# castacks/mvs_gi

Measured on AMD Instinct MI355X. Metric: stereo frames/sec/GPU (G16V, 3-cam, D=16) + inv-dist L1 vs reference, higher is better.
Workload: dtype f16x3 (split-fp16 MFMA operands: 11 + 11 significant bits, f32 accumulate/activations)

## Files before the change

### __graft_entry__.py

```python
import os
import subprocess
import sys

ROOT = os.path.dirname(os.path.abspath(__file__))
CSRC = os.path.join(ROOT, "mvs_gi_amd", "csrc")
LIB = os.path.join(ROOT, "mvs_gi_amd", "libmvsgi_hip.so")
SOURCES = ["api.cpp", "sweep.hip", "conv3d.hip", "conv3d_f16.hip", "conv3d_rs.hip", "conv3d_wino.hip", "conv3d_wino_up2.hip", "conv3d_s2rs.hip", "conv3d_up2poly.hip", "conv3d_headsplit.hip", "conv2d.hip", "resblock2d_rs.hip", "resize.hip", "softargmin.hip", "layout.hip", "grids.hip", "deform_conv2d.hip", "instnorm.hip"]


SRCHASH = LIB + ".srchash"


def _deps() -> list:
    return sorted([os.path.join(CSRC, s) for s in SOURCES] +
                  [os.path.join(CSRC, h) for h in os.listdir(CSRC) if h.endswith((".hpp", ".inc"))] +
                  [os.path.join(ROOT, "include", "mvsgi.h")])


def _source_hash(defs=()) -> str:
    import hashlib
    h = hashlib.sha256()
    for d in _deps():
        h.update(os.path.basename(d).encode() + b"\0")
        h.update(open(d, "rb").read())
    h.update(repr((sorted(defs), sorted(EXTRA_FLAGS.items()))).encode())
    return h.hexdigest()


def _needs_rebuild() -> bool:
    if not os.path.isfile(LIB) or not os.path.isfile(SRCHASH):
        return True
    return open(SRCHASH).read().strip() != _source_hash()


EXTRA_FLAGS = {
    "conv3d_rs.hip": ["-fno-slp-vectorize"],
    "conv3d_wino.hip": ["-fno-slp-vectorize"],
    "conv3d_wino_up2.hip": ["-fno-slp-vectorize"],
}


def _compile_objects(defs=(), tag="") -> list:
    from concurrent.futures import ThreadPoolExecutor
    import hashlib
    hipcc = os.environ.get("HIPCC", "/opt/rocm/bin/hipcc")
    if defs:
        tag += "_" + hashlib.md5(repr(sorted(defs)).encode()).hexdigest()[:8]
    objdir = os.path.join(ROOT, "build", "obj" + tag)
    os.makedirs(objdir, exist_ok=True)
    hdrs = [os.path.join(CSRC, h) for h in os.listdir(CSRC) if h.endswith((".hpp", ".inc"))] + \
           [os.path.join(ROOT, "include", "mvsgi.h")]
    hdr_t = max(os.path.getmtime(h) for h in hdrs)

    def one(src):
        obj = os.path.join(objdir, src + ".o")
        sp = os.path.join(CSRC, src)
        if os.path.isfile(obj) and os.path.getmtime(obj) > max(os.path.getmtime(sp), hdr_t):
            return obj
        cmd = [hipcc, "--offload-arch=gfx950", "-O3", "-std=c++17", "-fPIC", "-c", sp, "-o", obj] + list(defs) + \
            EXTRA_FLAGS.get(src, [])
        print("[build]", " ".join(cmd), flush=True)
        subprocess.run(cmd, check=True)
        return obj
    with ThreadPoolExecutor(max_workers=min(8, len(SOURCES))) as ex:
        return list(ex.map(one, SOURCES))


def _link(objs, out) -> None:
    hipcc = os.environ.get("HIPCC", "/opt/rocm/bin/hipcc")
    tmp = out + f".tmp{os.getpid()}"
    try:
        subprocess.run([hipcc, "--offload-arch=gfx950", "-fPIC", "-shared", "-o", tmp] + objs, check=True)
        os.replace(tmp, out)
    finally:
        if os.path.exists(tmp):
            os.remove(tmp)


def build(force: bool = False) -> None:
    if ROOT not in sys.path:
        sys.path.insert(0, ROOT)
    if force or _needs_rebuild():
        if force:
            import shutil
            shutil.rmtree(os.path.join(ROOT, "build", "obj"), ignore_errors=True)
        h = _source_hash()
        _link(_compile_objects(), LIB)
        with open(SRCHASH + f".tmp{os.getpid()}", "w") as f:
            f.write(h + "\n")
        os.replace(SRCHASH + f".tmp{os.getpid()}", SRCHASH)
    import mvs_gi_amd
    from mvs_gi_amd import _lib
    lib = _lib.load()
    assert lib.mvsgi_abi_version() == _lib.ABI_VERSION
    print(f"[build] {LIB} ok (ABI {lib.mvsgi_abi_version()})", flush=True)


def build_stamps(ablate: int = 0) -> str:
    out = os.path.join(ROOT, "mvs_gi_amd", f"libmvsgi_hip_stamps{ablate or ''}.so")
    _link(_compile_objects(["-DMVSGI_STAMPS", "-DMVSGI_RS_STAMPS", f"-DMVSGI_ABL={ablate}", f"-DMVSGI_RS_ABL={ablate}"],
                           tag=f"_stamps{ablate or ''}"), out)
    return out


def build_variant(defs, tag: str) -> str:
    out = os.path.join(ROOT, "mvs_gi_amd", f"libmvsgi_hip_{tag}.so")
    _link(_compile_objects(list(defs), tag="_" + tag), out)
    return out


def smoke() -> None:
    if ROOT not in sys.path:
        sys.path.insert(0, ROOT)
    import numpy as np
    import torch
    build()
    from mvs_gi_amd import hip_ops as H, synth
    from mvs_gi_amd.configs import CONFIGS, DIST_8L
    from mvs_gi_amd.pipeline import HotPath
    from oracle import mvsgi_oracle as O

    assert torch.cuda.is_available(), "smoke() needs a GPU"
    cfg = CONFIGS["G16V"].scaled(feat_hw=(16, 64), mask_hw=(64, 256), cv_hw=(8, 32), dist_cands=DIST_8L)
    inp = synth.make_inputs(cfg, seed=11, batch=1)
    w = synth.make_weights(cfg, seed=11)
    t = O.to_torch(inp)
    ref = O.hot_path(t["feats"], t["grids"], t["grid_masks"], t["masks"], O.to_torch(w), cfg.builder,
                     cfg.dist_cands, cfg.bf, cfg.interp_scale_factor, cfg.pre_interp)
    default_mode = H.get_conv_mode()
    try:
        bars = {"bf16x3": 1e-3, "f16x3": 1e-4, "f32": 1e-4}
        for mode in dict.fromkeys((default_mode, "f16x3", "bf16x3", "f32")):
            bar = bars[mode]
            H.set_conv_mode(mode)
            hp = HotPath(cfg, w, inp, device="cuda:0")
            inv, _ = hp(torch.from_numpy(inp["feats"]).to("cuda:0"))
            torch.cuda.synchronize()
            err = float((inv.cpu() - ref).abs().max() / ref.abs().max())
            print(f"[smoke] mode {mode}: inv_dist {tuple(inv.shape)} max-rel error vs oracle {err:.3e} (bar {bar:g})", flush=True)
            assert np.isfinite(err) and err < bar, (mode, err)
    finally:
        H.set_conv_mode(default_mode)


if __name__ == "__main__":
    build(force="--force" in sys.argv)
    if "--smoke" in sys.argv:
        smoke()
```

### include/mvsgi.h

```cpp
#ifndef MVSGI_H
#define MVSGI_H

#include <stddef.h>
#include <stdint.h>

#ifdef __cplusplus
extern "C" {
#endif

#define MVSGI_ABI_VERSION 5

typedef void* mvsgi_stream_t;

#define MVSGI_CONV_AUTO   0
#define MVSGI_CONV_DIRECT 1
#define MVSGI_CONV_MFMA   2
#define MVSGI_CONV_BF16X3 3
#define MVSGI_CONV_BF16X3_C16 4
#define MVSGI_CONV_BF16X3_V32 5
#define MVSGI_CONV_BF16X3_D32 6

#define MVSGI_CONV_F16 0x100

#define MVSGI_SPLIT_F16 1

int         mvsgi_abi_version(void);
const char* mvsgi_last_error(void);

#define MVSGI_SAT_SWEEP 1u
#define MVSGI_SAT_SPLIT 2u
#define MVSGI_SAT_WINO  4u
int mvsgi_saturation_flags(int clear, unsigned* flags);
int mvsgi_saturation_words(unsigned* words8);

int mvsgi_sweep_std_f32(const float* feats, const float* grids, const void* grid_masks,
                        int grid_mask_is_f32, const float* masks, float* vol,
                        int B, int N, int C, int Hi, int Wi, int Hm, int Wm,
                        int D, int Ho, int Wo, mvsgi_stream_t stream);

int mvsgi_sweep_cat_f32(const float* feats, const float* grids, float* vol,
                        int B, int N, int C, int Hi, int Wi,
                        int D, int Ho, int Wo, mvsgi_stream_t stream);

int mvsgi_sweep_std_nhwc_f32(const float* feats, const float* grids, const void* grid_masks,
                             int grid_mask_is_f32, const float* masks, float* vol,
                             int B, int N, int C, int Hi, int Wi, int Hm, int Wm,
                             int D, int Ho, int Wo, mvsgi_stream_t stream);
int mvsgi_sweep_cat_nhwc_f32(const float* feats, const float* grids, float* vol,
                             int B, int N, int C, int Hi, int Wi,
                             int D, int Ho, int Wo, mvsgi_stream_t stream);

int mvsgi_sweep_validity_u8(const float* grids, const void* grid_masks, int grid_mask_is_f32,
                            const float* masks, unsigned char* vmask,
                            int B, int N, int Hm, int Wm, int D, int Ho, int Wo, mvsgi_stream_t stream);
int mvsgi_sweep_std_nhwc_valid_f32(const float* feats, const float* grids, const unsigned char* vmask,
                                   float* vol, int B, int N, int C, int Hi, int Wi,
                                   int D, int Ho, int Wo, mvsgi_stream_t stream);
int mvsgi_sweep_std_nhwc_valid_rig_f32(const float* feats, const float* grids, const unsigned char* vmask,
                                       float* vol, int B, int N, int C, int Hi, int Wi, int D, int Ho, int Wo,
                                       mvsgi_stream_t stream);

size_t mvsgi_conv3d_packed_weight_floats(int Cout, int Cin);
int mvsgi_conv3d_pack_weights_f32(const float* w_oidhw, float* w_packed, int Cout, int Cin,
                                  mvsgi_stream_t stream);
size_t mvsgi_conv3d_packed_weight_bytes_bf16x3(int Cout, int Cin);
int mvsgi_conv3d_pack_weights_bf16x3(const float* w_oidhw, void* w_packed, int Cout, int Cin,
                                     mvsgi_stream_t stream);
int mvsgi_conv3d_pack_weights_split(const float* w_oidhw, void* w_packed, int Cout, int Cin, int layout, mvsgi_stream_t stream);
int mvsgi_conv3d_f32(const float* x, const float* w_oidhw, const float* w_packed,
                     const float* scale, const float* shift, const float* res, float* y,
                     int B, int Cin, int Din, int Hin, int Win, int Cout,
                     int stride, float neg_slope, int impl, mvsgi_stream_t stream);
const char* mvsgi_conv3d_variant_f32(int B, int Cin, int Din, int Hin, int Win, int Cout,
                                     int stride, int impl);

int mvsgi_conv3d_up2_f32(const float* x, const void* w_packed, int w_layout ,
                         const float* scale, const float* shift, const float* res, float* y,
                         int B, int Cin, int Dl, int Hl, int Wl, int Cout, float neg_slope, mvsgi_stream_t stream);
const char* mvsgi_conv3d_up2_variant_f32(int B, int Cin, int Dl, int Hl, int Wl, int Cout, int w_layout);
int mvsgi_conv3d_v32_applies(int B, int Cin, int Din, int Hin, int Win, int Cout, int stride);
int mvsgi_conv3d_d32_applies(int B, int Cin, int Din, int Hin, int Win, int Cout, int stride);
int mvsgi_conv3d_up2_d32_applies(int B, int Cin, int Dl, int Hl, int Wl, int Cout);
size_t mvsgi_conv3d_packed_weight_bytes_bf16x3_v32(int Cout, int Cin);
int mvsgi_conv3d_pack_weights_bf16x3_v32(const float* w_oidhw, void* w_packed, int Cout, int Cin, mvsgi_stream_t stream);
size_t mvsgi_conv3d_packed_weight_bytes_bf16x3_c16(int Cin);
int mvsgi_conv3d_pack_weights_bf16x3_c16(const float* w_oidhw, void* w_packed, int Cin, mvsgi_stream_t stream);

size_t mvsgi_conv2d_packed_weight_floats(int Cout, int Cin);
int mvsgi_conv2d_pack_weights_f32(const float* w_oihw, float* w_packed, int Cout, int Cin,
                                  mvsgi_stream_t stream);
size_t mvsgi_conv2d_stem_packed_weight_bytes(void);
int mvsgi_conv2d_stem_pack_weights(const float* w_oihw, void* w_packed, mvsgi_stream_t stream);
size_t mvsgi_conv2d_packed_weight_bytes_bf16x3(int Cout, int Cin);
int mvsgi_conv2d_pack_weights_bf16x3(const float* w_oihw, void* w_packed, int Cout, int Cin,
                                     mvsgi_stream_t stream);
int mvsgi_conv2d_f32(const float* x, const float* w_oihw, const void* w_packed,
                     const float* scale, const float* shift, const float* res, float* y,
                     int B, int Cin, int Hin, int Win, int Cout, int ksize, int stride,
                     float neg_slope, int impl, int in_nchw, mvsgi_stream_t stream);
const char* mvsgi_conv2d_variant_f32(int Cin, int Cout, int ksize, int stride, int impl, int in_nchw);

int mvsgi_resize_trilinear_f32(const float* x, float* y, int B, int C,
                               int Di, int Hi, int Wi, int Do, int Ho, int Wo,
                               mvsgi_stream_t stream);

int mvsgi_softargmin_f32(const float* costs, const float* inv_idx, float* inv_dist,
                         float* norm_costs, int B, int D, int H, int W, int scale,
                         mvsgi_stream_t stream);

int mvsgi_softargmin_div_f32(const float* costs, const float* inv_idx, float* inv_dist,
                             float* norm_costs, int B, int D, int H, int W, int scale,
                             float post_div, mvsgi_stream_t stream);

#define MVSGI_SA_AUTO  0
#define MVSGI_SA_PIXEL 1
#define MVSGI_SA_BAND  2
int mvsgi_softargmin_scaled_f32(const float* costs, const float* inv_idx, float* inv_dist,
                                float* norm_costs, int B, int D, int H, int W, double scale,
                                int OH, int OW, float post_div, int variant, mvsgi_stream_t stream);

int mvsgi_ncv_to_nvc_f32(const float* x, float* y, int B, int C, long long V, mvsgi_stream_t stream);
int mvsgi_nvc_to_ncv_f32(const float* x, float* y, int B, int C, long long V, mvsgi_stream_t stream);

int mvsgi_resblock2d_f32(const float* x, const void* w_packed1, const float* scale1, const float* shift1,
                         const void* w_packed2, const float* scale2, const float* shift2, float* y,
                         int N, int H, int W, float neg_slope, mvsgi_stream_t stream);

size_t mvsgi_split2d_bytes(int N, int H, int W);
int mvsgi_f32_to_split2d(const float* x, void* y_split, int N, int H, int W, mvsgi_stream_t stream);
int mvsgi_split2d_to_f32(const void* x_split, float* y, int N, int H, int W, mvsgi_stream_t stream);
size_t mvsgi_resblock2d_split_packed_weight_bytes(void);
int mvsgi_resblock2d_split_pack_weights(const float* w_oihw, const float* scale, void* w_packed, mvsgi_stream_t stream);
int mvsgi_resblock2d_split(const void* x_split, const void* w_packed1, const float* shift1,
                           const void* w_packed2, const float* shift2, void* y, int y_is_split,
                           int N, int H, int W, float neg_slope, mvsgi_stream_t stream);
int mvsgi_conv2d_s2_split(const void* x_split, const void* w_packed, const float* shift, void* y_split,
                          int N, int H, int W, float neg_slope, mvsgi_stream_t stream);
int mvsgi_conv2d_f32_out_split2d(const float* x, const float* w_oihw, const void* w_packed,
                                 const float* scale, const float* shift, const float* res, void* y_split,
                                 int B, int Cin, int Hin, int Win, int Cout, int ksize, int stride,
                                 float neg_slope, int impl, int in_nchw, mvsgi_stream_t stream);

int mvsgi_rays_panorama_f32(const float* dist, float* rays, int N, int H, int W,
                            float lat0, float lat1, float lon0, float lon1, mvsgi_stream_t stream);
int mvsgi_transform_points_f32(const float* T , const float* points, float* out,
                               int B, long long M, mvsgi_stream_t stream);
int mvsgi_grid_double_sphere_f32(const float* points, float* grid, unsigned char* mask, int B, long long M,
                                 float xi, float alpha, float fx, float fy, float cx, float cy,
                                 int calib_h, int calib_w, float w2, mvsgi_stream_t stream);
int mvsgi_grid_equirect_f32(const float* points, float* grid, int B, long long M, mvsgi_stream_t stream);

int mvsgi_deform_conv2d_pack_weights_f32(const float* w_oihw, float* w_packed, int Cout, int Cin, int Kh, int Kw,
                                         mvsgi_stream_t stream);
int mvsgi_deform_conv2d_f32(const float* x, const float* offset, int offset_per_image, const float* w_packed,
                            const float* scale, const float* shift, const float* res, float* y,
                            int N, int Cin, int H, int W, int Cout, int Kh, int Kw, int stride_h, int stride_w,
                            int pad_h, int pad_w, int dil_h, int dil_w, float neg_slope, mvsgi_stream_t stream);

int mvsgi_sweep_std_nhwc_valid_split(const float* feats, const float* grids, const unsigned char* vmask,
                                     void* vol_split, int B, int N, int C, int Hi, int Wi, int D, int Ho, int Wo,
                                     int rig_batch, mvsgi_stream_t stream);

int mvsgi_conv3d_f32_out_split(const float* x, const float* w_packed_b3, const float* scale, const float* shift,
                               const float* res, void* y_split, int B, int Cin, int Din, int Hin, int Win, int Cout,
                               int stride, float neg_slope, mvsgi_stream_t stream);
int mvsgi_conv3d_rs16_split(const void* x_split, const void* w_packed_rs, const float* scale, const float* shift, float* y,
                            int B, int D, int H, int W, float neg_slope, mvsgi_stream_t stream);
int mvsgi_conv3d_rs16_split_out_split(const void* x_split, const void* w_packed_rs, const float* scale, const float* shift,
                                      void* y_split, int B, int D, int H, int W, float neg_slope, mvsgi_stream_t stream);
size_t mvsgi_conv3d_s2rs_packed_weight_bytes(void);
int mvsgi_conv3d_s2rs_pack_weights(const float* w_oidhw, const float* scale, void* w_packed, mvsgi_stream_t stream);
int mvsgi_conv3d_s2rs(const void* x_split, const void* w_packed, const float* shift, void* y_split,
                      int B, int D, int H, int W, float neg_slope, mvsgi_stream_t stream);
size_t mvsgi_conv3d_rs_packed_weight_bytes(int Cout, int Cin);
int mvsgi_conv3d_rs_pack_weights(const float* w_oidhw, void* w_packed, int Cout, int Cin, mvsgi_stream_t stream);
size_t mvsgi_act_split_bytes(int B, int C, int D, int H, int W);
int mvsgi_act_f32_to_split(const float* x, void* y_split, int B, int C, int D, int H, int W, mvsgi_stream_t stream);
int mvsgi_act_split_to_f32(const void* x_split, float* y, int B, int C, int D, int H, int W, mvsgi_stream_t stream);
int mvsgi_conv3d_rs_split(const void* x_split, const void* w_packed_rs, const float* scale, const float* shift,
                          const void* res_split, void* y, int y_is_f32, int B, int Cin, int D, int H, int W, int Cout,
                          float neg_slope, mvsgi_stream_t stream);

int mvsgi_conv3d_up2_f32_out_split(const float* x, const void* w_packed, int w_layout, const float* scale, const float* shift,
                                   const float* res, void* y_split, int B, int Cin, int Dl, int Hl, int Wl, int Cout,
                                   float neg_slope, mvsgi_stream_t stream);
int mvsgi_conv3d_up2_poly_split(const void* x_split, const void* plan_dev, const float* scale, const float* shift, void* y_split,
                                int B, int D, int H, int W, float neg_slope, mvsgi_stream_t stream);
size_t mvsgi_conv3d_head_split_packed_weight_bytes(int Cin);
int mvsgi_conv3d_head_split_pack_weights(const float* w_oidhw, void* w_packed, int Cin, mvsgi_stream_t stream);
int mvsgi_conv3d_head_split(const void* x_split, const void* w_packed, float scale, float shift, float* y, int B, int Cin,
                            int D, int H, int W, float neg_slope, mvsgi_stream_t stream);
int mvsgi_conv3d_head_split_pack_weights_f16(const float* w_oidhw, void* w_packed, int Cin, mvsgi_stream_t stream);
int mvsgi_conv3d_head_split_f16(const void* x_split, const void* w_packed, float scale, float shift, float* y, int B, int Cin,
                            int D, int H, int W, float neg_slope, mvsgi_stream_t stream);
size_t mvsgi_conv3d_up2_poly_plan_bytes(int D, int H, int W);
int mvsgi_conv3d_up2_poly_plan(const float* w_oidhw_host, void* plan_host, int D, int H, int W);
int mvsgi_conv3d_up2_poly_f32(const void* x_split, const void* plan_dev, const float* scale, const float* shift, float* y,
                              int B, int D, int H, int W, float neg_slope, mvsgi_stream_t stream);

int mvsgi_act_f32_to_split_fmt(const float* x, void* y_split, int B, int C, int D, int H, int W, int fmt, mvsgi_stream_t stream);
int mvsgi_act_split_to_f32_fmt(const void* x_split, float* y, int B, int C, int D, int H, int W, int fmt, mvsgi_stream_t stream);
int mvsgi_sweep_std_nhwc_valid_split_fmt(const float* feats, const float* grids, const unsigned char* vmask, void* vol_split,
                                         int B, int N, int C, int Hi, int Wi, int D, int Ho, int Wo, int rig_batch, int fmt,
                                         mvsgi_stream_t stream);
int mvsgi_conv3d_f32_out_split_fmt(const float* x, const float* w_packed_b3, const float* scale, const float* shift,
                                   const float* res, void* y_split, int B, int Cin, int Din, int Hin, int Win, int Cout,
                                   int stride, float neg_slope, int fmt, mvsgi_stream_t stream);
int mvsgi_conv3d_rs_pack_weights_fmt(const float* w_oidhw, void* w_packed, int Cout, int Cin, int fmt, mvsgi_stream_t stream);
int mvsgi_conv3d_rs_split_fmt(const void* x_split, const void* w_packed_rs, const float* scale, const float* shift,
                              const void* res_split, void* y, int y_is_f32, int B, int Cin, int D, int H, int W, int Cout,
                              float neg_slope, int fmt, mvsgi_stream_t stream);
int mvsgi_conv3d_rs16_split_fmt(const void* x_split, const void* w_packed_rs, const float* scale, const float* shift, void* y,
                                int y_is_split, int B, int D, int H, int W, float neg_slope, int fmt, mvsgi_stream_t stream);
int mvsgi_conv3d_s2rs_pack_weights_fmt(const float* w_oidhw, const float* scale, void* w_packed, int fmt, mvsgi_stream_t stream);
int mvsgi_conv3d_s2rs_fmt(const void* x_split, const void* w_packed, const float* shift, void* y_split, int B, int D, int H, int W,
                          float neg_slope, float unscale, int fmt, mvsgi_stream_t stream);
int mvsgi_conv3d_s2rs_out_fmt(const void* x_split, const void* w_packed, const float* shift, void* y_split, int B, int D, int H, int W,
                              float neg_slope, float unscale, int fmt, int y_f32p, mvsgi_stream_t stream);
int mvsgi_conv3d_up2_poly_plan_fmt(const float* w_oidhw_host, void* plan_host, int D, int H, int W, int fmt);
int mvsgi_conv3d_up2_poly_fmt(const void* x_split, const void* plan_dev, const float* scale, const float* shift, void* y,
                              int y_is_split, int B, int D, int H, int W, float neg_slope, int fmt, mvsgi_stream_t stream);
int mvsgi_conv3d_up2_poly_wino_pays(int B, int D, int H, int W);

size_t mvsgi_conv3d_wino32_packed_weight_bytes(void);
int mvsgi_conv3d_wino32_applies(int Cin, int Cout, int D, int H, int W, int stride, float neg_slope);
int mvsgi_conv3d_wino32_pack_weights(const float* w_oidhw, void* w_packed, float* unscale, mvsgi_stream_t stream);
int mvsgi_conv3d_wino32_f16(const void* x_split, const void* w_packed, const float* scale, const float* shift, const void* res_split,
                            void* y, int y_is_f32, int act_f32p, int B, int D, int H, int W, float neg_slope, mvsgi_stream_t stream);

size_t mvsgi_instance_norm_ws_bytes(int B, int S, int C);
int mvsgi_instance_norm_f32(const float* x, const float* res, const float* gamma, const float* beta, float* y, float* ws,
                            int B, int S, int C, float eps, float neg_slope, mvsgi_stream_t stream);

#ifdef __cplusplus
}
#endif
#endif
```

### mvs_gi_amd/_lib.py

```python
from __future__ import annotations

import ctypes
import os
from ctypes import c_char_p, c_double, c_float, c_int, c_longlong, c_size_t, c_void_p

_HERE = os.path.dirname(os.path.abspath(__file__))
LIB_PATH = os.environ.get("MVSGI_LIB", os.path.join(_HERE, "libmvsgi_hip.so"))

ABI_VERSION = 5


class MvsgiLibraryMissing(RuntimeError):
    pass


_P = c_void_p
SIGNATURES = {
    "mvsgi_abi_version": (c_int, []),
    "mvsgi_last_error": (c_char_p, []),
    "mvsgi_saturation_flags": (c_int, [c_int, _P]),
    "mvsgi_saturation_words": (c_int, [_P]),
    "mvsgi_sweep_std_f32": (c_int, [_P, _P, _P, c_int, _P, _P] + [c_int] * 10 + [_P]),
    "mvsgi_sweep_cat_f32": (c_int, [_P, _P, _P] + [c_int] * 8 + [_P]),
    "mvsgi_sweep_std_nhwc_f32": (c_int, [_P, _P, _P, c_int, _P, _P] + [c_int] * 10 + [_P]),
    "mvsgi_sweep_cat_nhwc_f32": (c_int, [_P, _P, _P] + [c_int] * 8 + [_P]),
    "mvsgi_sweep_validity_u8": (c_int, [_P, _P, c_int, _P, _P] + [c_int] * 7 + [_P]),
    "mvsgi_sweep_std_nhwc_valid_f32": (c_int, [_P, _P, _P, _P] + [c_int] * 8 + [_P]),
    "mvsgi_sweep_std_nhwc_valid_split": (c_int, [_P, _P, _P, _P] + [c_int] * 9 + [_P]),
    "mvsgi_sweep_std_nhwc_valid_rig_f32": (c_int, [_P, _P, _P, _P] + [c_int] * 8 + [_P]),
    "mvsgi_conv3d_packed_weight_floats": (c_size_t, [c_int, c_int]),
    "mvsgi_conv3d_pack_weights_f32": (c_int, [_P, _P, c_int, c_int, _P]),
    "mvsgi_conv3d_packed_weight_bytes_bf16x3": (c_size_t, [c_int, c_int]),
    "mvsgi_conv3d_pack_weights_bf16x3": (c_int, [_P, _P, c_int, c_int, _P]),
    "mvsgi_conv3d_pack_weights_split": (c_int, [_P, _P, c_int, c_int, c_int, _P]),
    "mvsgi_conv3d_f32": (c_int, [_P] * 7 + [c_int] * 7 + [c_float, c_int, _P]),
    "mvsgi_conv3d_variant_f32": (c_char_p, [c_int] * 8),
    "mvsgi_conv3d_up2_f32": (c_int, [_P, _P, c_int] + [_P] * 4 + [c_int] * 6 + [c_float, _P]),
    "mvsgi_conv3d_up2_variant_f32": (c_char_p, [c_int] * 7),
    "mvsgi_conv3d_v32_applies": (c_int, [c_int] * 7),
    "mvsgi_conv3d_d32_applies": (c_int, [c_int] * 7),
    "mvsgi_conv3d_up2_d32_applies": (c_int, [c_int] * 6),
    "mvsgi_conv3d_packed_weight_bytes_bf16x3_v32": (c_size_t, [c_int, c_int]),
    "mvsgi_conv3d_pack_weights_bf16x3_v32": (c_int, [_P, _P, c_int, c_int, _P]),
    "mvsgi_conv3d_packed_weight_bytes_bf16x3_c16": (c_size_t, [c_int]),
    "mvsgi_conv3d_pack_weights_bf16x3_c16": (c_int, [_P, _P, c_int, _P]),
    "mvsgi_conv2d_stem_packed_weight_bytes": (c_size_t, []),
    "mvsgi_conv2d_stem_pack_weights": (c_int, [_P, _P, _P]),
    "mvsgi_conv2d_packed_weight_floats": (c_size_t, [c_int, c_int]),
    "mvsgi_conv2d_pack_weights_f32": (c_int, [_P, _P, c_int, c_int, _P]),
    "mvsgi_conv2d_packed_weight_bytes_bf16x3": (c_size_t, [c_int, c_int]),
    "mvsgi_conv2d_pack_weights_bf16x3": (c_int, [_P, _P, c_int, c_int, _P]),
    "mvsgi_conv2d_f32": (c_int, [_P] * 7 + [c_int] * 7 + [c_float, c_int, c_int, _P]),
    "mvsgi_conv2d_variant_f32": (c_char_p, [c_int] * 6),
    "mvsgi_resblock2d_f32": (c_int, [_P] * 8 + [c_int] * 3 + [c_float, _P]),
    "mvsgi_split2d_bytes": (c_size_t, [c_int] * 3),
    "mvsgi_f32_to_split2d": (c_int, [_P, _P] + [c_int] * 3 + [_P]),
    "mvsgi_split2d_to_f32": (c_int, [_P, _P] + [c_int] * 3 + [_P]),
    "mvsgi_resblock2d_split_packed_weight_bytes": (c_size_t, []),
    "mvsgi_resblock2d_split_pack_weights": (c_int, [_P, _P, _P, _P]),
    "mvsgi_resblock2d_split": (c_int, [_P] * 6 + [c_int] * 4 + [c_float, _P]),
    "mvsgi_conv2d_s2_split": (c_int, [_P] * 4 + [c_int] * 3 + [c_float, _P]),
    "mvsgi_conv2d_f32_out_split2d": (c_int, [_P] * 7 + [c_int] * 7 + [c_float, c_int, c_int, _P]),
    "mvsgi_resize_trilinear_f32": (c_int, [_P, _P] + [c_int] * 8 + [_P]),
    "mvsgi_softargmin_f32": (c_int, [_P, _P, _P, _P] + [c_int] * 5 + [_P]),
    "mvsgi_softargmin_div_f32": (c_int, [_P, _P, _P, _P] + [c_int] * 5 + [c_float, _P]),
    "mvsgi_softargmin_scaled_f32": (c_int, [_P, _P, _P, _P] + [c_int] * 4 + [c_double, c_int, c_int, c_float, c_int, _P]),
    "mvsgi_rays_panorama_f32": (c_int, [_P, _P, c_int, c_int, c_int] + [c_float] * 4 + [_P]),
    "mvsgi_transform_points_f32": (c_int, [_P, _P, _P, c_int, c_longlong, _P]),
    "mvsgi_grid_double_sphere_f32": (c_int, [_P, _P, _P, c_int, c_longlong] + [c_float] * 6 + [c_int, c_int, c_float, _P]),
    "mvsgi_grid_equirect_f32": (c_int, [_P, _P, c_int, c_longlong, _P]),
    "mvsgi_deform_conv2d_pack_weights_f32": (c_int, [_P, _P] + [c_int] * 4 + [_P]),
    "mvsgi_deform_conv2d_f32": (c_int, [_P, _P, c_int] + [_P] * 5 + [c_int] * 13 + [c_float, _P]),
    "mvsgi_act_split_bytes": (c_size_t, [c_int] * 5),
    "mvsgi_act_f32_to_split": (c_int, [_P, _P] + [c_int] * 5 + [_P]),
    "mvsgi_act_split_to_f32": (c_int, [_P, _P] + [c_int] * 5 + [_P]),
    "mvsgi_conv3d_f32_out_split": (c_int, [_P] * 6 + [c_int] * 7 + [c_float, _P]),
    "mvsgi_conv3d_rs16_split": (c_int, [_P] * 5 + [c_int] * 4 + [c_float, _P]),
    "mvsgi_conv3d_rs16_split_out_split": (c_int, [_P] * 5 + [c_int] * 4 + [c_float, _P]),
    "mvsgi_conv3d_s2rs_packed_weight_bytes": (c_size_t, []),
    "mvsgi_conv3d_s2rs_pack_weights": (c_int, [_P, _P, _P, _P]),
    "mvsgi_conv3d_s2rs": (c_int, [_P] * 4 + [c_int] * 4 + [c_float, _P]),
    "mvsgi_conv3d_rs_packed_weight_bytes": (c_size_t, [c_int, c_int]),
    "mvsgi_conv3d_rs_pack_weights": (c_int, [_P, _P, c_int, c_int, _P]),
    "mvsgi_conv3d_rs_split": (c_int, [_P] * 6 + [c_int] * 7 + [c_float, _P]),
    "mvsgi_conv3d_up2_f32_out_split": (c_int, [_P, _P, c_int] + [_P] * 4 + [c_int] * 6 + [c_float, _P]),
    "mvsgi_conv3d_up2_poly_split": (c_int, [_P] * 5 + [c_int] * 4 + [c_float, _P]),
    "mvsgi_conv3d_head_split_packed_weight_bytes": (c_size_t, [c_int]),
    "mvsgi_conv3d_head_split_pack_weights": (c_int, [_P, _P, c_int, _P]),
    "mvsgi_conv3d_head_split": (c_int, [_P, _P, c_float, c_float, _P] + [c_int] * 5 + [c_float, _P]),
    "mvsgi_conv3d_head_split_pack_weights_f16": (c_int, [_P, _P, c_int, _P]),
    "mvsgi_conv3d_head_split_f16": (c_int, [_P, _P, c_float, c_float, _P] + [c_int] * 5 + [c_float, _P]),
    "mvsgi_conv3d_up2_poly_plan_bytes": (c_size_t, [c_int] * 3),
    "mvsgi_conv3d_up2_poly_plan": (c_int, [_P, _P] + [c_int] * 3),
    "mvsgi_conv3d_up2_poly_f32": (c_int, [_P] * 5 + [c_int] * 4 + [c_float, _P]),
    "mvsgi_act_f32_to_split_fmt": (c_int, [_P, _P] + [c_int] * 6 + [_P]),
    "mvsgi_act_split_to_f32_fmt": (c_int, [_P, _P] + [c_int] * 6 + [_P]),
    "mvsgi_sweep_std_nhwc_valid_split_fmt": (c_int, [_P, _P, _P, _P] + [c_int] * 10 + [_P]),
    "mvsgi_conv3d_f32_out_split_fmt": (c_int, [_P] * 6 + [c_int] * 7 + [c_float, c_int, _P]),
    "mvsgi_conv3d_rs_pack_weights_fmt": (c_int, [_P, _P, c_int, c_int, c_int, _P]),
    "mvsgi_conv3d_rs_split_fmt": (c_int, [_P] * 6 + [c_int] * 7 + [c_float, c_int, _P]),
    "mvsgi_conv3d_rs16_split_fmt": (c_int, [_P] * 5 + [c_int] * 5 + [c_float, c_int, _P]),
    "mvsgi_conv3d_s2rs_pack_weights_fmt": (c_int, [_P, _P, _P, c_int, _P]),
    "mvsgi_conv3d_s2rs_fmt": (c_int, [_P] * 4 + [c_int] * 4 + [c_float, c_float, c_int, _P]),
    "mvsgi_conv3d_s2rs_out_fmt": (c_int, [_P] * 4 + [c_int] * 4 + [c_float, c_float, c_int, c_int, _P]),
    "mvsgi_conv3d_up2_poly_plan_fmt": (c_int, [_P, _P] + [c_int] * 4),
    "mvsgi_conv3d_wino32_packed_weight_bytes": (c_size_t, []),
    "mvsgi_conv3d_wino32_applies": (c_int, [c_int] * 6 + [c_float]),
    "mvsgi_conv3d_wino32_pack_weights": (c_int, [_P] * 4),
    "mvsgi_conv3d_wino32_f16": (c_int, [_P] * 6 + [c_int] * 6 + [c_float, _P]),
    "mvsgi_conv3d_up2_poly_fmt": (c_int, [_P] * 5 + [c_int] * 5 + [c_float, c_int, _P]),
    "mvsgi_conv3d_up2_poly_wino_pays": (c_int, [c_int] * 4),
    "mvsgi_ncv_to_nvc_f32": (c_int, [_P, _P, c_int, c_int, c_longlong, _P]),
    "mvsgi_nvc_to_ncv_f32": (c_int, [_P, _P, c_int, c_int, c_longlong, _P]),
    "mvsgi_instance_norm_ws_bytes": (c_size_t, [c_int] * 3),
    "mvsgi_instance_norm_f32": (c_int, [_P] * 6 + [c_int] * 3 + [c_float, c_float, _P]),
}

_lib = None


def load() -> ctypes.CDLL:
    global _lib
    if _lib is not None:
        return _lib
    if not os.path.isfile(LIB_PATH):
        raise MvsgiLibraryMissing(
            f"{LIB_PATH} not found: build the HIP library first (__graft_entry__.build()). "
            "mvs_gi_amd has no CPU fallback.")
    import torch
    lib = ctypes.CDLL(LIB_PATH)
    try:
        lib.mvsgi_abi_version.restype = c_int
        lib.mvsgi_abi_version.argtypes = []
        got = lib.mvsgi_abi_version()
    except AttributeError as e:
        raise MvsgiLibraryMissing(f"{LIB_PATH}: not a libmvsgi_hip ({e}); rebuild it (__graft_entry__.build())") from None
    if got != ABI_VERSION:
        raise MvsgiLibraryMissing(f"{LIB_PATH}: ABI version {got}, expected {ABI_VERSION}; rebuild it (__graft_entry__.build())")
    for name, (res, args) in SIGNATURES.items():
        try:
            fn = getattr(lib, name)
        except AttributeError:
            raise MvsgiLibraryMissing(f"{LIB_PATH}: symbol {name} missing although the ABI version matches; rebuild it "
                                      "(__graft_entry__.build())") from None
        fn.restype = res
        fn.argtypes = args
    lib.mvsgi_saturation_flags(0, None)
    _lib = lib
    return lib


def check(status: int, what: str) -> None:
    if status != 0:
        msg = load().mvsgi_last_error()
        raise RuntimeError(f"{what}: {msg.decode() if msg else 'unknown error'}")
```

### mvs_gi_amd/csrc/sweep.hip

```cpp
#include "common.hpp"

namespace {

#include "split_fmt.hpp"

struct Bilin {
    int o00, o01, o10, o11;
    float w00, w01, w10, w11;
};

#ifndef MVSGI_SWEEP_SKIP_CAM
#define MVSGI_SWEEP_SKIP_CAM 1
#endif
__device__ __forceinline__ Bilin bilin_setup(float gx, float gy, int W, int H) {
#pragma clang fp contract(off)
    Bilin t;
    const float x = ((gx + 1.0f) * (float)W - 1.0f) / 2.0f;
    const float y = ((gy + 1.0f) * (float)H - 1.0f) / 2.0f;
    const float xf = floorf(x), yf = floorf(y);
    const float x1f = xf + 1.0f, y1f = yf + 1.0f;
    t.w00 = (x1f - x) * (y1f - y);
    t.w01 = (x1f - x) * (y - yf);
    t.w10 = (x - xf) * (y1f - y);
    t.w11 = (x - xf) * (y - yf);
    const int x0 = (int)fminf(fmaxf(xf, -2.0f), (float)W + 1.0f);
    const int y0 = (int)fminf(fmaxf(yf, -2.0f), (float)H + 1.0f);
    const int x1 = x0 + 1, y1 = y0 + 1;
    const bool vx0 = (x0 >= 0) & (x0 < W), vx1 = (x1 >= 0) & (x1 < W);
    const bool vy0 = (y0 >= 0) & (y0 < H), vy1 = (y1 >= 0) & (y1 < H);
    t.o00 = (vx0 & vy0) ? y0 * W + x0 : -1;
    t.o01 = (vx0 & vy1) ? y1 * W + x0 : -1;
    t.o10 = (vx1 & vy0) ? y0 * W + x1 : -1;
    t.o11 = (vx1 & vy1) ? y1 * W + x1 : -1;
    return t;
}

__device__ __forceinline__ Bilin bilin_setup_bytes(float gx, float gy, int W, int H, int C4, int rowB) {
#pragma clang fp contract(off)
    Bilin t;
    const float x = ((gx + 1.0f) * (float)W - 1.0f) / 2.0f;
    const float y = ((gy + 1.0f) * (float)H - 1.0f) / 2.0f;
    const float xf = floorf(x), yf = floorf(y);
    const float x1f = xf + 1.0f, y1f = yf + 1.0f;
    t.w00 = (x1f - x) * (y1f - y);
    t.w01 = (x1f - x) * (y - yf);
    t.w10 = (x - xf) * (y1f - y);
    t.w11 = (x - xf) * (y - yf);
    const int x0 = (int)fminf(fmaxf(xf, -2.0f), (float)W + 1.0f);
    const int y0 = (int)fminf(fmaxf(yf, -2.0f), (float)H + 1.0f);
    const bool vx0 = (unsigned)x0 < (unsigned)W, vx1 = (unsigned)(x0 + 1) < (unsigned)W;
    const bool vy0 = (unsigned)y0 < (unsigned)H, vy1 = (unsigned)(y0 + 1) < (unsigned)H;
    const int base = __mul24(y0, rowB) + __mul24(x0, C4);
    constexpr int kOutside = (int)0x80000000;
    t.o00 = (vx0 & vy0) ? base : kOutside;
    t.o01 = (vx0 & vy1) ? base + rowB : kOutside;
    t.o10 = (vx1 & vy0) ? base + C4 : kOutside;
    t.o11 = (vx1 & vy1) ? base + rowB + C4 : kOutside;
    return t;
}

__device__ __forceinline__ float bilin_fetch(const float* __restrict__ plane, const Bilin& t) {
#pragma clang fp contract(off)
    const float i00 = t.o00 >= 0 ? plane[t.o00] : 0.0f;
    const float i01 = t.o01 >= 0 ? plane[t.o01] : 0.0f;
    const float i10 = t.o10 >= 0 ? plane[t.o10] : 0.0f;
    const float i11 = t.o11 >= 0 ? plane[t.o11] : 0.0f;
    return ((i00 * t.w00 + i01 * t.w01) + i10 * t.w10) + i11 * t.w11;
}

typedef float f32x4_t __attribute__((ext_vector_type(4)));

__device__ __forceinline__ float div_small(float x, float d, float inv) {
    const float ax = fabsf(x);
    const float q = x * inv;
    const float r = __builtin_fmaf(-d, q, x);
    float res = __builtin_fmaf(r, inv, q);
    if (ax == 0.0f) res = x;
    const bool rare = ax != 0.0f && !(ax >= 1e-30f && ax <= 1e30f);
    if (__builtin_amdgcn_ballot_w64(rare) != 0) {
        if (rare) res = x / d;
    }
    return res;
}

struct SweepDims {
    int B, N, C, Hi, Wi, Hm, Wm, D, Ho, Wo;
};

template <int NCAM, int CC>
__global__ __launch_bounds__(256) void sweep_std_kernel(const float* __restrict__ feats,
                                                        const float* __restrict__ grids,
                                                        const unsigned char* __restrict__ gm_u8,
                                                        const float* __restrict__ gm_f32,
                                                        const float* __restrict__ masks,
                                                        float* __restrict__ vol, SweepDims s) {
#pragma clang fp contract(off)
    const long long total = (long long)s.B * s.D * s.Ho * s.Wo;
    const long long idx = (long long)blockIdx.x * 256 + threadIdx.x;
    if (idx >= total) return;
    const int wo = (int)(idx % s.Wo);
    const int ho = (int)((idx / s.Wo) % s.Ho);
    const int d = (int)((idx / ((long long)s.Wo * s.Ho)) % s.D);
    const int b = (int)(idx / ((long long)s.Wo * s.Ho * s.D));

    Bilin ft[NCAM];
    float vf[NCAM];
    float n = 0.0f;
    const long long HWi = (long long)s.Hi * s.Wi;
    const long long HWm = (long long)s.Hm * s.Wm;
#pragma unroll
    for (int cam = 0; cam < NCAM; ++cam) {
        const long long g = ((((long long)(b * NCAM + cam) * s.D + d) * s.Ho + ho) * s.Wo + wo);
        const float2 gxy = *reinterpret_cast<const float2*>(grids + g * 2);
        ft[cam] = bilin_setup(gxy.x, gxy.y, s.Wi, s.Hi);
        const Bilin mt = bilin_setup(gxy.x, gxy.y, s.Wm, s.Hm);
        const float sm = bilin_fetch(masks + (long long)(b * NCAM + cam) * HWm, mt);
        const bool gmv = gm_f32 ? (gm_f32[g] != 0.0f) : (gm_u8[g] != 0);
        const bool valid = (sm > 0.0f) && gmv;
        vf[cam] = valid ? 1.0f : 0.0f;
        n = n + vf[cam];
    }
    const bool ok = n > 1.0f;
    const float cnt = ok ? n : 1.0f;

    float* out = vol + idx * s.C;
    for (int c = 0; c < s.C; c += CC) {
        float sv[NCAM][CC];
#pragma unroll
        for (int cam = 0; cam < NCAM; ++cam) {
            const float* plane = feats + ((long long)(b * NCAM + cam) * s.C + c) * HWi;
#pragma unroll
            for (int k = 0; k < CC; ++k) sv[cam][k] = bilin_fetch(plane + k * HWi, ft[cam]);
        }
        float r[CC];
#pragma unroll
        for (int k = 0; k < CC; ++k) {
            float sum = 0.0f;
#pragma unroll
            for (int cam = 0; cam < NCAM; ++cam) sum = sum + sv[cam][k] * vf[cam];
            const float avg = sum / cnt;
            float var = 0.0f;
#pragma unroll
            for (int cam = 0; cam < NCAM; ++cam) {
                const float t = vf[cam] != 0.0f ? sv[cam][k] : avg;
                const float df = t - avg;
                var = var + df * df;
            }
            var = var / cnt;
            r[k] = ok ? var : 0.0f;
        }
        if (CC == 4) {
            *reinterpret_cast<float4*>(out + c) = make_float4(r[0], r[1], r[2], r[3]);
        } else {
#pragma unroll
            for (int k = 0; k < CC; ++k) out[c + k] = r[k];
        }
    }
}

template <int CC>
__global__ __launch_bounds__(256) void sweep_cat_kernel(const float* __restrict__ feats,
                                                        const float* __restrict__ grids,
                                                        float* __restrict__ vol, SweepDims s) {
#pragma clang fp contract(off)
    const long long total = (long long)s.B * s.D * s.Ho * s.N * s.Wo;
    const long long idx = (long long)blockIdx.x * 256 + threadIdx.x;
    if (idx >= total) return;
    const int wo = (int)(idx % s.Wo);
    const int cam = (int)((idx / s.Wo) % s.N);
    const int ho = (int)((idx / ((long long)s.Wo * s.N)) % s.Ho);
    const int d = (int)((idx / ((long long)s.Wo * s.N * s.Ho)) % s.D);
    const int b = (int)(idx / ((long long)s.Wo * s.N * s.Ho * s.D));
    const long long g = ((((long long)(b * s.N + cam) * s.D + d) * s.Ho + ho) * s.Wo + wo);
    const float2 gxy = *reinterpret_cast<const float2*>(grids + g * 2);
    const Bilin ft = bilin_setup(gxy.x, gxy.y, s.Wi, s.Hi);
    const long long HWi = (long long)s.Hi * s.Wi;
    const long long vox = (((long long)b * s.D + d) * s.Ho + ho) * s.Wo + wo;
    float* out = vol + vox * ((long long)s.N * s.C) + (long long)cam * s.C;
    const float* base = feats + ((long long)(b * s.N + cam) * s.C) * HWi;
    for (int c = 0; c < s.C; c += CC) {
        float r[CC];
#pragma unroll
        for (int k = 0; k < CC; ++k) r[k] = bilin_fetch(base + (long long)(c + k) * HWi, ft);
        if (CC == 4) {
            *reinterpret_cast<float4*>(out + c) = make_float4(r[0], r[1], r[2], r[3]);
        } else {
#pragma unroll
            for (int k = 0; k < CC; ++k) out[c + k] = r[k];
        }
    }
}

__device__ __forceinline__ f32x4_t ld4(const float* p) { return *reinterpret_cast<const f32x4_t*>(p); }

__device__ __forceinline__ f32x4_t bilin_fetch4(const float* __restrict__ img, int C, const Bilin& t) {
#pragma clang fp contract(off)
    const f32x4_t z = {0.f, 0.f, 0.f, 0.f};
    const f32x4_t i00 = t.o00 >= 0 ? ld4(img + t.o00 * C) : z;
    const f32x4_t i01 = t.o01 >= 0 ? ld4(img + t.o01 * C) : z;
    const f32x4_t i10 = t.o10 >= 0 ? ld4(img + t.o10 * C) : z;
    const f32x4_t i11 = t.o11 >= 0 ? ld4(img + t.o11 * C) : z;
    return ((i00 * t.w00 + i01 * t.w01) + i10 * t.w10) + i11 * t.w11;
}

__device__ __forceinline__ f32x4_t bilin_fetch4_buf(__amdgpu_buffer_rsrc_t img, int c, int C, const Bilin& t) {
#pragma clang fp contract(off)
    const f32x4_t i00 = __builtin_bit_cast(f32x4_t, __builtin_amdgcn_raw_buffer_load_b128(img, (t.o00 * C + c) * 4, 0, 0));
    const f32x4_t i01 = __builtin_bit_cast(f32x4_t, __builtin_amdgcn_raw_buffer_load_b128(img, (t.o01 * C + c) * 4, 0, 0));
    const f32x4_t i10 = __builtin_bit_cast(f32x4_t, __builtin_amdgcn_raw_buffer_load_b128(img, (t.o10 * C + c) * 4, 0, 0));
    const f32x4_t i11 = __builtin_bit_cast(f32x4_t, __builtin_amdgcn_raw_buffer_load_b128(img, (t.o11 * C + c) * 4, 0, 0));
    return ((i00 * t.w00 + i01 * t.w01) + i10 * t.w10) + i11 * t.w11;
}

__device__ __forceinline__ float bilin_fetch_buf(__amdgpu_buffer_rsrc_t plane, const Bilin& t) {
#pragma clang fp contract(off)
    const float i00 = __builtin_bit_cast(float, __builtin_amdgcn_raw_buffer_load_b32(plane, t.o00 * 4, 0, 0));
    const float i01 = __builtin_bit_cast(float, __builtin_amdgcn_raw_buffer_load_b32(plane, t.o01 * 4, 0, 0));
    const float i10 = __builtin_bit_cast(float, __builtin_amdgcn_raw_buffer_load_b32(plane, t.o10 * 4, 0, 0));
    const float i11 = __builtin_bit_cast(float, __builtin_amdgcn_raw_buffer_load_b32(plane, t.o11 * 4, 0, 0));
    return ((i00 * t.w00 + i01 * t.w01) + i10 * t.w10) + i11 * t.w11;
}

__device__ __forceinline__ int sweep_xcd_remap(int bid, int n) {
    const int q = n >> 3, r = n & 7, x = bid & 7, i = bid >> 3;
    return (x < r ? x * (q + 1) : r * (q + 1) + (x - r) * q) + i;
}

template <int NCAM>
__global__ __launch_bounds__(256) void sweep_std_nhwc_kernel(const float* __restrict__ feats,
                                                             const float* __restrict__ grids,
                                                             const unsigned char* __restrict__ gm_u8,
                                                             const float* __restrict__ gm_f32,
                                                             const float* __restrict__ masks,
                                                             float* __restrict__ vol, SweepDims s) {
#pragma clang fp contract(off)
    static_assert(NCAM <= 4, "one camera per lane of a quad");
    const int q = threadIdx.x & 3;
    const int WT = (s.Wo + 63) >> 6;
    int L = sweep_xcd_remap((int)blockIdx.x, (int)gridDim.x);
    const int wt = L % WT;
    L /= WT;
    const int d = L % s.D;
    L /= s.D;
    const int ho = L % s.Ho;
    const int b = L / s.Ho;
    int wo = wt * 64 + (threadIdx.x >> 2);
    const bool live = wo < s.Wo;
    if (!live) wo = s.Wo - 1;
    const int HWm = s.Hm * s.Wm, HWi = s.Hi * s.Wi;

    Bilin mine = {};
    float myvalid = 0.f;
    if (q < NCAM) {
        const long long grow = (((long long)(b * NCAM + q) * s.D + d) * s.Ho + ho) * s.Wo;
        const float2 gxy = *reinterpret_cast<const float2*>(grids + (grow + wo) * 2);
        mine = bilin_setup(gxy.x, gxy.y, s.Wi, s.Hi);
        const Bilin mt = bilin_setup(gxy.x, gxy.y, s.Wm, s.Hm);
        const float sm = bilin_fetch(masks + (long long)(b * NCAM + q) * HWm, mt);
        const bool gmv = gm_f32 ? (gm_f32[grow + wo] != 0.0f) : (gm_u8[grow + wo] != 0);
        myvalid = ((sm > 0.0f) && gmv) ? 1.0f : 0.0f;
    }
    const int lane = threadIdx.x & 63, qbase = lane & ~3;
    __amdgpu_buffer_rsrc_t img[NCAM];
#pragma unroll
    for (int cam = 0; cam < NCAM; ++cam)
        img[cam] = __builtin_amdgcn_make_buffer_rsrc(
            const_cast<float*>(feats + (long long)(b * NCAM + cam) * HWi * s.C), 0, HWi * s.C * 4, 0x00020000);
    Bilin ft[NCAM];
    float vf[NCAM];
    float n = 0.0f;
#pragma unroll
    for (int cam = 0; cam < NCAM; ++cam) {
        const int src = qbase + cam;
        ft[cam].o00 = __shfl(mine.o00, src);
        ft[cam].o01 = __shfl(mine.o01, src);
        ft[cam].o10 = __shfl(mine.o10, src);
        ft[cam].o11 = __shfl(mine.o11, src);
        ft[cam].w00 = __shfl(mine.w00, src);
        ft[cam].w01 = __shfl(mine.w01, src);
        ft[cam].w10 = __shfl(mine.w10, src);
        ft[cam].w11 = __shfl(mine.w11, src);
        vf[cam] = __shfl(myvalid, src);
        n = n + vf[cam];
    }
    const bool ok = n > 1.0f;
    const float cnt = ok ? n : 1.0f;
    const float inv = 1.0f / cnt;
    float* out = vol + ((((long long)b * s.D + d) * s.Ho + ho) * s.Wo + wo) * s.C;
    for (int c = q * 4; c < s.C; c += 16) {
        f32x4_t sv[NCAM];
#pragma unroll
        for (int cam = 0; cam < NCAM; ++cam) sv[cam] = bilin_fetch4_buf(img[cam], c, s.C, ft[cam]);
        f32x4_t r;
#pragma unroll
        for (int k = 0; k < 4; ++k) {
            float sum = 0.0f;
#pragma unroll
            for (int cam = 0; cam < NCAM; ++cam) sum = sum + sv[cam][k] * vf[cam];
            const float avg = div_small(sum, cnt, inv);
            float var = 0.0f;
#pragma unroll
            for (int cam = 0; cam < NCAM; ++cam) {
                const float t = vf[cam] != 0.0f ? sv[cam][k] : avg;
                const float df = t - avg;
                var = var + df * df;
            }
            var = div_small(var, cnt, inv);
            r[k] = ok ? var : 0.0f;
        }
        if (live) *reinterpret_cast<f32x4_t*>(out + c) = r;
    }
}

__global__ __launch_bounds__(256) void sweep_validity_kernel(const float* __restrict__ grids,
                                                             const unsigned char* __restrict__ gm_u8,
                                                             const float* __restrict__ gm_f32,
                                                             const float* __restrict__ masks,
                                                             unsigned char* __restrict__ vmask, SweepDims s) {
#pragma clang fp contract(off)
    const long long HW = (long long)s.Ho * s.Wo;
    const long long total = (long long)s.B * s.D * HW;
    const long long idx = (long long)blockIdx.x * 256 + threadIdx.x;
    if (idx >= total) return;
    const long long pix = idx % HW;
    const int d = (int)((idx / HW) % s.D);
    const int b = (int)(idx / (HW * s.D));
    const long long HWm = (long long)s.Hm * s.Wm;
    unsigned bits = 0;
    for (int cam = 0; cam < s.N; ++cam) {
        const long long g = ((long long)(b * s.N + cam) * s.D + d) * HW + pix;
        const float2 gxy = *reinterpret_cast<const float2*>(grids + g * 2);
        const Bilin mt = bilin_setup(gxy.x, gxy.y, s.Wm, s.Hm);
        const float sm = bilin_fetch(masks + (long long)(b * s.N + cam) * HWm, mt);
        const bool gmv = gm_f32 ? (gm_f32[g] != 0.0f) : (gm_u8[g] != 0);
        bits |= ((sm > 0.0f) && gmv) ? (1u << cam) : 0u;
    }
    vmask[idx] = (unsigned char)bits;
}

template <int CAM>
__device__ __forceinline__ int quad_bcast_i(int v) {
    return __builtin_amdgcn_mov_dpp(v, CAM * 0x55, 0xf, 0xf, true);
}
template <int CAM>
__device__ __forceinline__ float quad_bcast_f(float v) {
    return __builtin_bit_cast(float, quad_bcast_i<CAM>(__builtin_bit_cast(int, v)));
}
template <int CAM>
__device__ __forceinline__ Bilin quad_bcast(const Bilin& m) {
    Bilin t;
    t.o00 = quad_bcast_i<CAM>(m.o00);
    t.o01 = quad_bcast_i<CAM>(m.o01);
    t.o10 = quad_bcast_i<CAM>(m.o10);
    t.o11 = quad_bcast_i<CAM>(m.o11);
    t.w00 = quad_bcast_f<CAM>(m.w00);
    t.w01 = quad_bcast_f<CAM>(m.w01);
    t.w10 = quad_bcast_f<CAM>(m.w10);
    t.w11 = quad_bcast_f<CAM>(m.w11);
    return t;
}

#ifndef MVSGI_SWEEP_NT
#define MVSGI_SWEEP_NT 0
#endif
#ifndef MVSGI_SWEEP_WAVES
#define MVSGI_SWEEP_WAVES 5
#endif
template <int NCAM, bool C16, bool F16 = false>
__global__ __launch_bounds__(256, MVSGI_SWEEP_WAVES) void sweep_std_nhwc_v_kernel(const float* __restrict__ feats,
                                                               const float* __restrict__ grids,
                                                               const unsigned char* __restrict__ vmask,
                                                               float* __restrict__ vol, SweepDims s, int dchunk,
                                                               int nd, int rig_shared, unsigned char* __restrict__ vol_split,
                                                               unsigned* __restrict__ sat) {
#pragma clang fp contract(off)
    static_assert(NCAM <= 4, "one camera per lane of a quad");
    float satm = 0.f;
    const int q = threadIdx.x & 3;
    const int WT = (s.Wo + 63) >> 6;
    int L = sweep_xcd_remap((int)blockIdx.x, (int)gridDim.x);
    const int wt = L % WT;
    L /= WT;
    const int dc = L % nd;
    L /= nd;
    const int ho = L % s.Ho;
    const int b = L / s.Ho;
    int wo = wt * 64 + (threadIdx.x >> 2);
    const bool live = wo < s.Wo;
    if (!live) wo = s.Wo - 1;
    const int d0 = dc * dchunk;
    const int d1 = d0 + dchunk < s.D ? d0 + dchunk : s.D;
    const int HWi = s.Hi * s.Wi;
    const long long HW = (long long)s.Ho * s.Wo;

    __amdgpu_buffer_rsrc_t img[NCAM];
#pragma unroll
    for (int cam = 0; cam < NCAM; ++cam)
        img[cam] = __builtin_amdgcn_make_buffer_rsrc(
            const_cast<float*>(feats + (long long)(b * NCAM + cam) * HWi * s.C), 0, HWi * s.C * 4, 0x00020000);
    const int mycam = q < NCAM ? q : NCAM - 1;
    const int br = rig_shared ? 0 : b;
    const float2* gp = reinterpret_cast<const float2*>(grids) + ((long long)(br * NCAM + mycam) * s.D + d0) * HW +
                       (long long)ho * s.Wo + wo;
    const unsigned char* vp = vmask + ((long long)br * s.D + d0) * HW + (long long)ho * s.Wo + wo;
    float* out = vol + ((((long long)b * s.D + d0) * s.Ho + ho) * s.Wo + wo) * s.C;
    const long long vstep = HW * s.C;
    unsigned char* outs = vol_split ? vol_split + ((((long long)b * (s.D + 2) + d0 + 1) * (s.Ho + 2) + ho + 1) * (s.Wo + 2) + wo + 1) * 64 +
                                          ((q & 1) * 2 + (q >> 1)) * 16
                                    : nullptr;
    const long long sstep = (long long)(s.Ho + 2) * (s.Wo + 2) * 64;
    const int C4 = C16 ? 64 : s.C * 4, rowB = s.Wi * C4;
    auto candidate = [&](const float2 gxy, const unsigned vm, float* __restrict__ o, unsigned char* __restrict__ os) {
        typedef float f32x2_t __attribute__((ext_vector_type(2)));
        const Bilin mine = bilin_setup_bytes(gxy.x, gxy.y, s.Wi, s.Hi, C4, rowB);
        Bilin ft[NCAM];
        ft[0] = quad_bcast<0>(mine);
        if (NCAM > 1) ft[NCAM > 1 ? 1 : 0] = quad_bcast<1>(mine);
        if (NCAM > 2) ft[NCAM > 2 ? 2 : 0] = quad_bcast<2>(mine);
        if (NCAM > 3) ft[NCAM > 3 ? 3 : 0] = quad_bcast<3>(mine);
        bool val[NCAM];
        f32x2_t VF[NCAM];
        float n = 0.0f;
#pragma unroll
        for (int cam = 0; cam < NCAM; ++cam) {
            val[cam] = ((vm >> cam) & 1u) != 0;
            const float vf = val[cam] ? 1.0f : 0.0f;
            VF[cam] = f32x2_t{vf, vf};
            n = n + vf;
        }
        const bool ok = n > 1.0f;
        const float cnt = ok ? n : 1.0f;
#ifndef MVSGI_SWEEP_GATHER_ALL
#pragma unroll
        for (int cam = 0; cam < NCAM; ++cam) {
            const bool need = val[cam] & ok;
            ft[cam].o00 = need ? ft[cam].o00 : (int)0x80000000;
            ft[cam].o01 = need ? ft[cam].o01 : (int)0x80000000;
            ft[cam].o10 = need ? ft[cam].o10 : (int)0x80000000;
            ft[cam].o11 = need ? ft[cam].o11 : (int)0x80000000;
        }
#endif
        const float inv = cnt == 2.0f ? 0.5f : cnt == 3.0f ? 0x1.555556p-2f : cnt == 4.0f ? 0.25f : 1.0f;
        const f32x2_t INV = {inv, inv}, NCNT = {-cnt, -cnt};
#pragma unroll 1
        for (int cb = q * 16; cb < (C16 ? 64 : C4); cb += 64) {
            f32x4_t tx[NCAM][4];
#ifdef MVSGI_SWEEP_ABL_NOGATHER
#pragma unroll
            for (int cam = 0; cam < NCAM; ++cam) { ft[cam].o00 &= 64; ft[cam].o01 &= 64; ft[cam].o10 &= 64; ft[cam].o11 &= 64; }
#endif
#pragma unroll
            for (int cam = 0; cam < NCAM; ++cam) {
#if MVSGI_SWEEP_SKIP_CAM
                if (__builtin_amdgcn_ballot_w64(val[cam] & ok) == 0) {
                    tx[cam][0] = tx[cam][1] = tx[cam][2] = tx[cam][3] = f32x4_t{0.f, 0.f, 0.f, 0.f};
                    continue;
                }
#endif
                tx[cam][0] = __builtin_bit_cast(f32x4_t, __builtin_amdgcn_raw_buffer_load_b128(img[cam], ft[cam].o00 + cb, 0, 0));
                tx[cam][1] = __builtin_bit_cast(f32x4_t, __builtin_amdgcn_raw_buffer_load_b128(img[cam], ft[cam].o01 + cb, 0, 0));
                tx[cam][2] = __builtin_bit_cast(f32x4_t, __builtin_amdgcn_raw_buffer_load_b128(img[cam], ft[cam].o10 + cb, 0, 0));
                tx[cam][3] = __builtin_bit_cast(f32x4_t, __builtin_amdgcn_raw_buffer_load_b128(img[cam], ft[cam].o11 + cb, 0, 0));
            }
            f32x2_t sv[NCAM][2];
#pragma unroll
            for (int cam = 0; cam < NCAM; ++cam) {
                const f32x2_t W00 = {ft[cam].w00, ft[cam].w00}, W01 = {ft[cam].w01, ft[cam].w01};
                const f32x2_t W10 = {ft[cam].w10, ft[cam].w10}, W11 = {ft[cam].w11, ft[cam].w11};
#pragma unroll
                for (int p = 0; p < 2; ++p) {
                    const f32x2_t i00 = {tx[cam][0][2 * p], tx[cam][0][2 * p + 1]}, i01 = {tx[cam][1][2 * p], tx[cam][1][2 * p + 1]};
                    const f32x2_t i10 = {tx[cam][2][2 * p], tx[cam][2][2 * p + 1]}, i11 = {tx[cam][3][2 * p], tx[cam][3][2 * p + 1]};
                    sv[cam][p] = ((i00 * W00 + i01 * W01) + i10 * W10) + i11 * W11;
                }
            }
            f32x2_t sum[2], var[2];
            f32x4_t r;
            float big = 0.0f;
#pragma unroll
            for (int p = 0; p < 2; ++p) {
                sum[p] = sv[0][p] * VF[0];
#pragma unroll
                for (int cam = 1; cam < NCAM; ++cam) sum[p] = sum[p] + sv[cam][p] * VF[cam];
                const f32x2_t qa = sum[p] * INV;
                const f32x2_t avg = __builtin_elementwise_fma(__builtin_elementwise_fma(NCNT, qa, sum[p]), INV, qa);
#pragma unroll
                for (int cam = 0; cam < NCAM; ++cam) {
                    const f32x2_t t = {val[cam] ? sv[cam][p].x : avg.x, val[cam] ? sv[cam][p].y : avg.y};
                    const f32x2_t df = t - avg;
                    var[p] = cam == 0 ? df * df : var[p] + df * df;
                }
                const f32x2_t qv = var[p] * INV;
                const f32x2_t v = __builtin_elementwise_fma(__builtin_elementwise_fma(NCNT, qv, var[p]), INV, qv);
                r[2 * p] = ok ? v.x : 0.0f;
                r[2 * p + 1] = ok ? v.y : 0.0f;
                big = __builtin_fmaxf(__builtin_fmaxf(big, __builtin_fmaxf(__builtin_fabsf(sum[p].x), __builtin_fabsf(sum[p].y))),
                                      __builtin_fmaxf(var[p].x, var[p].y));
            }
            if (__builtin_amdgcn_ballot_w64(big > 1e30f) != 0) {
                float dv = cnt;
                asm volatile("; exact-division path" : "+v"(dv));
#pragma unroll
                for (int k = 0; k < 4; ++k) {
                    const float sm = sum[k >> 1][k & 1];
                    const float avg = sm / dv;
                    float vr = 0.0f;
#pragma unroll
                    for (int cam = 0; cam < NCAM; ++cam) {
                        const float t = val[cam] ? sv[cam][k >> 1][k & 1] : avg;
                        const float df = t - avg;
                        vr = vr + df * df;
                    }
                    vr = vr / dv;
                    r[k] = ok ? vr : 0.0f;
                }
            }
            if (os) {
                unsigned hi[2], lo[2];
#pragma unroll
                for (int p = 0; p < 2; ++p) {
                    if constexpr (F16) {
                        const float a_ = sf_clamp<true>(r[2 * p]), b_ = sf_clamp<true>(r[2 * p + 1]);
                        satm = sf_sat_acc(satm, a_, b_);
                        const unsigned hb = sf_cvt_pk<true>(a_, b_);
                        hi[p] = hb;
                        lo[p] = sf_cvt_pk<true>(a_ - sf_widen_lo<true>(hb), b_ - sf_widen_hi<true>(hb));
                    } else {
                        typedef __bf16 b2_t __attribute__((ext_vector_type(2)));
                        const f32x2_t v = {r[2 * p], r[2 * p + 1]};
                        const unsigned hb = __builtin_bit_cast(unsigned, __builtin_convertvector(v, b2_t));
                        const f32x2_t hf = {__builtin_bit_cast(float, hb << 16), __builtin_bit_cast(float, hb & 0xffff0000u)};
                        hi[p] = hb;
                        lo[p] = __builtin_bit_cast(unsigned, __builtin_convertvector(v - hf, b2_t));
                    }
                }
                const bool odd = (q & 1) != 0;
                const unsigned r0 = (unsigned)__builtin_amdgcn_mov_dpp((int)(odd ? hi[0] : lo[0]), 0xB1, 0xf, 0xf, true);
                const unsigned r1 = (unsigned)__builtin_amdgcn_mov_dpp((int)(odd ? hi[1] : lo[1]), 0xB1, 0xf, 0xf, true);
                const uint4 piece = odd ? make_uint4(r0, r1, lo[0], lo[1]) : make_uint4(hi[0], hi[1], r0, r1);
#ifdef MVSGI_SWEEP_ABL_NOSTORE
                if (live && hi[0] == 0x12345678u) {
#else
                if (live) {
#endif
#if MVSGI_SWEEP_NT
                    {
                        typedef unsigned nt_u32x4 __attribute__((ext_vector_type(4)));
                        __builtin_nontemporal_store(nt_u32x4{piece.x, piece.y, piece.z, piece.w}, reinterpret_cast<nt_u32x4*>(os));
                    }
#else
                    *reinterpret_cast<uint4*>(os) = piece;
#endif
                }
            } else if (live) *reinterpret_cast<f32x4_t*>(reinterpret_cast<char*>(o) + cb) = r;
        }
    };
    float2 gA = *gp;
    unsigned vA = *vp;
    for (int d = d0; d < d1; d += 2) {
        const bool hasB = d + 1 < d1;
        const long long sB = hasB ? HW : 0;
        const float2 gB = gp[sB];
        const unsigned vB = vp[sB];
        candidate(gA, vA, out, outs);
        const long long sA = d + 2 < d1 ? 2 * HW : sB;
        gA = gp[sA];
        vA = vp[sA];
        if (hasB) candidate(gB, vB, out + vstep, outs ? outs + sstep : nullptr);
        gp += 2 * HW;
        vp += 2 * HW;
        out += 2 * vstep;
        if (outs) outs += 2 * sstep;
    }
    if constexpr (F16) sf_sat_report(sat, kSatSweep, satm, kF16Max);
}

__global__ __launch_bounds__(256) void sweep_cat_nhwc_kernel(const float* __restrict__ feats,
                                                             const float* __restrict__ grids,
                                                             float* __restrict__ vol, SweepDims s) {
#pragma clang fp contract(off)
    const int q = threadIdx.x & 3;
    const int WT = (s.Wo + 63) >> 6;
    int L = sweep_xcd_remap((int)blockIdx.x, (int)gridDim.x);
    const int wt = L % WT;
    L /= WT;
    const int cam = L % s.N;
    L /= s.N;
    const int d = L % s.D;
    L /= s.D;
    const int ho = L % s.Ho;
    const int b = L / s.Ho;
    const int wo = wt * 64 + (threadIdx.x >> 2);
    if (wo >= s.Wo) return;
    const long long grow = (((long long)(b * s.N + cam) * s.D + d) * s.Ho + ho) * s.Wo;
    const float2 gxy = *reinterpret_cast<const float2*>(grids + (grow + wo) * 2);
    const Bilin ft = bilin_setup(gxy.x, gxy.y, s.Wi, s.Hi);
    const int HWi = s.Hi * s.Wi;
    const long long vox = (((long long)b * s.D + d) * s.Ho + ho) * s.Wo + wo;
    float* out = vol + vox * ((long long)s.N * s.C) + (long long)cam * s.C;
    const __amdgpu_buffer_rsrc_t img = __builtin_amdgcn_make_buffer_rsrc(
        const_cast<float*>(feats + (long long)(b * s.N + cam) * HWi * s.C), 0, HWi * s.C * 4, 0x00020000);
    for (int c = q * 4; c < s.C; c += 16)
        *reinterpret_cast<f32x4_t*>(out + c) = bilin_fetch4_buf(img, c, s.C, ft);
}

int check_dims(const SweepDims& s, const char* who) {
    MVSGI_REQUIRE(s.B > 0 && s.N > 0 && s.C > 0 && s.Hi > 0 && s.Wi > 0 && s.D > 0 && s.Ho > 0 && s.Wo > 0,
                  "%s: non-positive dimension", who);
    MVSGI_REQUIRE((long long)s.Hi * s.Wi < (1ll << 31) && (long long)s.Hm * s.Wm < (1ll << 31),
                  "%s: image plane too large for 32-bit texel offsets", who);
    return 0;
}

}

extern "C" int mvsgi_sweep_std_f32(const float* feats, const float* grids, const void* grid_masks,
                                   int grid_mask_is_f32, const float* masks, float* vol, int B, int N,
                                   int C, int Hi, int Wi, int Hm, int Wm, int D, int Ho, int Wo,
                                   mvsgi_stream_t stream) {
    SweepDims s{B, N, C, Hi, Wi, Hm, Wm, D, Ho, Wo};
    if (check_dims(s, "mvsgi_sweep_std_f32")) return 1;
    MVSGI_REQUIRE(Hm > 0 && Wm > 0, "mvsgi_sweep_std_f32: non-positive mask size");
    MVSGI_REQUIRE(feats && grids && grid_masks && masks && vol, "mvsgi_sweep_std_f32: null pointer");
    MVSGI_REQUIRE(N >= 1 && N <= 6, "mvsgi_sweep_std_f32: num_cams %d not in [1, 6]", N);
    const long long total = (long long)B * D * Ho * Wo;
    const dim3 grid((unsigned)mvsgi::cdiv(total, 256)), block(256);
    const unsigned char* g8 = grid_mask_is_f32 ? nullptr : static_cast<const unsigned char*>(grid_masks);
    const float* g32 = grid_mask_is_f32 ? static_cast<const float*>(grid_masks) : nullptr;
    hipStream_t st = mvsgi::as_stream(stream);
#define LAUNCH_STD(NC)                                                                                    \
    case NC:                                                                                              \
        if (C % 4 == 0)                                                                                   \
            hipLaunchKernelGGL((sweep_std_kernel<NC, 4>), grid, block, 0, st, feats, grids, g8, g32, masks, \
                               vol, s);                                                                   \
        else                                                                                              \
            hipLaunchKernelGGL((sweep_std_kernel<NC, 1>), grid, block, 0, st, feats, grids, g8, g32, masks, \
                               vol, s);                                                                   \
        break;
    switch (N) {
        LAUNCH_STD(1)
        LAUNCH_STD(2)
        LAUNCH_STD(3)
        LAUNCH_STD(4)
        LAUNCH_STD(5)
        LAUNCH_STD(6)
    }
#undef LAUNCH_STD
    return mvsgi::check_launch("mvsgi_sweep_std_f32");
}

extern "C" int mvsgi_sweep_cat_f32(const float* feats, const float* grids, float* vol, int B, int N, int C,
                                   int Hi, int Wi, int D, int Ho, int Wo, mvsgi_stream_t stream) {
    SweepDims s{B, N, C, Hi, Wi, 1, 1, D, Ho, Wo};
    if (check_dims(s, "mvsgi_sweep_cat_f32")) return 1;
    MVSGI_REQUIRE(feats && grids && vol, "mvsgi_sweep_cat_f32: null pointer");
    const long long total = (long long)B * D * Ho * N * Wo;
    const dim3 grid((unsigned)mvsgi::cdiv(total, 256)), block(256);
    hipStream_t st = mvsgi::as_stream(stream);
    if (C % 4 == 0)
        hipLaunchKernelGGL((sweep_cat_kernel<4>), grid, block, 0, st, feats, grids, vol, s);
    else
        hipLaunchKernelGGL((sweep_cat_kernel<1>), grid, block, 0, st, feats, grids, vol, s);
    return mvsgi::check_launch("mvsgi_sweep_cat_f32");
}

extern "C" int mvsgi_sweep_std_nhwc_f32(const float* feats, const float* grids, const void* grid_masks,
                                        int grid_mask_is_f32, const float* masks, float* vol, int B, int N,
                                        int C, int Hi, int Wi, int Hm, int Wm, int D, int Ho, int Wo,
                                        mvsgi_stream_t stream) {
    SweepDims s{B, N, C, Hi, Wi, Hm, Wm, D, Ho, Wo};
    if (check_dims(s, "mvsgi_sweep_std_nhwc_f32")) return 1;
    MVSGI_REQUIRE(Hm > 0 && Wm > 0, "mvsgi_sweep_std_nhwc_f32: non-positive mask size");
    MVSGI_REQUIRE(feats && grids && grid_masks && masks && vol, "mvsgi_sweep_std_nhwc_f32: null pointer");
    MVSGI_REQUIRE(N >= 1 && N <= 4, "mvsgi_sweep_std_nhwc_f32: num_cams %d not in [1, 4]", N);
    MVSGI_REQUIRE(C % 4 == 0, "mvsgi_sweep_std_nhwc_f32: C=%d must be a multiple of 4", C);
    const long long nblk = mvsgi::cdiv(Wo, 64) * Ho * D * B;
    MVSGI_REQUIRE((long long)Hi * Wi * C < (1ll << 31) && nblk < (1ll << 31),
                  "mvsgi_sweep_std_nhwc_f32: dimensions exceed the launch geometry");
    const dim3 grid((unsigned)nblk), block(256);
    const unsigned char* g8 = grid_mask_is_f32 ? nullptr : static_cast<const unsigned char*>(grid_masks);
    const float* g32 = grid_mask_is_f32 ? static_cast<const float*>(grid_masks) : nullptr;
    hipStream_t st = mvsgi::as_stream(stream);
    switch (N) {
        case 1: hipLaunchKernelGGL((sweep_std_nhwc_kernel<1>), grid, block, 0, st, feats, grids, g8, g32, masks, vol, s); break;
        case 2: hipLaunchKernelGGL((sweep_std_nhwc_kernel<2>), grid, block, 0, st, feats, grids, g8, g32, masks, vol, s); break;
        case 3: hipLaunchKernelGGL((sweep_std_nhwc_kernel<3>), grid, block, 0, st, feats, grids, g8, g32, masks, vol, s); break;
        case 4: hipLaunchKernelGGL((sweep_std_nhwc_kernel<4>), grid, block, 0, st, feats, grids, g8, g32, masks, vol, s); break;
    }
    return mvsgi::check_launch("mvsgi_sweep_std_nhwc_f32");
}

extern "C" int mvsgi_sweep_cat_nhwc_f32(const float* feats, const float* grids, float* vol, int B, int N, int C,
                                        int Hi, int Wi, int D, int Ho, int Wo, mvsgi_stream_t stream) {
    SweepDims s{B, N, C, Hi, Wi, 1, 1, D, Ho, Wo};
    if (check_dims(s, "mvsgi_sweep_cat_nhwc_f32")) return 1;
    MVSGI_REQUIRE(feats && grids && vol, "mvsgi_sweep_cat_nhwc_f32: null pointer");
    MVSGI_REQUIRE(C % 4 == 0, "mvsgi_sweep_cat_nhwc_f32: C=%d must be a multiple of 4", C);
    const long long nblk = mvsgi::cdiv(Wo, 64) * N * Ho * D * B;
    MVSGI_REQUIRE((long long)Hi * Wi * C < (1ll << 31) && nblk < (1ll << 31),
                  "mvsgi_sweep_cat_nhwc_f32: dimensions exceed the launch geometry");
    hipLaunchKernelGGL(sweep_cat_nhwc_kernel, dim3((unsigned)nblk), dim3(256), 0, mvsgi::as_stream(stream), feats,
                       grids, vol, s);
    return mvsgi::check_launch("mvsgi_sweep_cat_nhwc_f32");
}

extern "C" int mvsgi_sweep_validity_u8(const float* grids, const void* grid_masks, int grid_mask_is_f32,
                                       const float* masks, unsigned char* vmask, int B, int N, int Hm, int Wm, int D,
                                       int Ho, int Wo, mvsgi_stream_t stream) {
    SweepDims s{B, N, 1, 1, 1, Hm, Wm, D, Ho, Wo};
    if (check_dims(s, "mvsgi_sweep_validity_u8")) return 1;
    MVSGI_REQUIRE(Hm > 0 && Wm > 0, "mvsgi_sweep_validity_u8: non-positive mask size");
    MVSGI_REQUIRE(grids && grid_masks && masks && vmask, "mvsgi_sweep_validity_u8: null pointer");
    MVSGI_REQUIRE(N >= 1 && N <= 8, "mvsgi_sweep_validity_u8: num_cams %d not in [1, 8]", N);
    const long long total = (long long)B * D * Ho * Wo;
    MVSGI_REQUIRE(mvsgi::cdiv(total, 256) < (1ll << 31), "mvsgi_sweep_validity_u8: too many voxels");
    const unsigned char* g8 = grid_mask_is_f32 ? nullptr : static_cast<const unsigned char*>(grid_masks);
    const float* g32 = grid_mask_is_f32 ? static_cast<const float*>(grid_masks) : nullptr;
    hipLaunchKernelGGL(sweep_validity_kernel, dim3((unsigned)mvsgi::cdiv(total, 256)), dim3(256), 0,
                       mvsgi::as_stream(stream), grids, g8, g32, masks, vmask, s);
    return mvsgi::check_launch("mvsgi_sweep_validity_u8");
}

namespace {
int sweep_std_nhwc_valid_impl(const float* feats, const float* grids, const unsigned char* vmask, float* vol, int B, int N, int C,
                              int Hi, int Wi, int D, int Ho, int Wo, int rig_shared, mvsgi_stream_t stream,
                              unsigned char* vol_split = nullptr, int fmt = 0) {
    MVSGI_REQUIRE(fmt == 0 || (fmt == MVSGI_SPLIT_F16 && vol_split), "mvsgi_sweep_std_nhwc_valid_split: fmt %d not in {0, MVSGI_SPLIT_F16}", fmt);
    SweepDims s{B, N, C, Hi, Wi, 1, 1, D, Ho, Wo};
    if (check_dims(s, "mvsgi_sweep_std_nhwc_valid_f32")) return 1;
    MVSGI_REQUIRE(feats && grids && vmask && (vol || vol_split), "mvsgi_sweep_std_nhwc_valid_f32: null pointer");
    MVSGI_REQUIRE(!vol_split || C == 16, "mvsgi_sweep_std_nhwc_valid_split: the split-padded output needs C == 16 (got %d)", C);
    MVSGI_REQUIRE(N >= 1 && N <= 4, "mvsgi_sweep_std_nhwc_valid_f32: num_cams %d not in [1, 4]", N);
    MVSGI_REQUIRE(C % 4 == 0, "mvsgi_sweep_std_nhwc_valid_f32: C=%d must be a multiple of 4", C);
    const long long rows = mvsgi::cdiv(Wo, 64) * Ho * B;
    long long nd = rows >= 8192 ? 2 : mvsgi::cdiv(8192, rows);
    if (nd > D) nd = D;
    const int dchunk = (int)mvsgi::cdiv(D, nd);
    nd = mvsgi::cdiv(D, dchunk);
    const long long nblk = rows * nd;
    MVSGI_REQUIRE((long long)Hi * Wi * C < (1ll << 29) && (long long)Wi * C * 4 < (1ll << 23) && nblk < (1ll << 31),
                  "mvsgi_sweep_std_nhwc_valid_f32: dimensions exceed the launch geometry (image bytes < 2^31, row bytes < 2^23)");
    hipStream_t st = mvsgi::as_stream(stream);
    MVSGI_SAT_WORDS(sat);
    const dim3 grid((unsigned)nblk), block(256);
    if (fmt) {
        switch (N) {
            case 1: hipLaunchKernelGGL((sweep_std_nhwc_v_kernel<1, true, true>), grid, block, 0, st, feats, grids, vmask, vol, s, dchunk, (int)nd, rig_shared, vol_split, sat); break;
            case 2: hipLaunchKernelGGL((sweep_std_nhwc_v_kernel<2, true, true>), grid, block, 0, st, feats, grids, vmask, vol, s, dchunk, (int)nd, rig_shared, vol_split, sat); break;
            case 3: hipLaunchKernelGGL((sweep_std_nhwc_v_kernel<3, true, true>), grid, block, 0, st, feats, grids, vmask, vol, s, dchunk, (int)nd, rig_shared, vol_split, sat); break;
            case 4: hipLaunchKernelGGL((sweep_std_nhwc_v_kernel<4, true, true>), grid, block, 0, st, feats, grids, vmask, vol, s, dchunk, (int)nd, rig_shared, vol_split, sat); break;
        }
        return mvsgi::check_launch("mvsgi_sweep_std_nhwc_valid_split");
    }
    switch (N) {
        case 1: if (C == 16) hipLaunchKernelGGL((sweep_std_nhwc_v_kernel<1, true>), grid, block, 0, st, feats, grids, vmask, vol, s, dchunk, (int)nd, rig_shared, vol_split, sat);
                else hipLaunchKernelGGL((sweep_std_nhwc_v_kernel<1, false>), grid, block, 0, st, feats, grids, vmask, vol, s, dchunk, (int)nd, rig_shared, vol_split, sat);
                break;
        case 2: if (C == 16) hipLaunchKernelGGL((sweep_std_nhwc_v_kernel<2, true>), grid, block, 0, st, feats, grids, vmask, vol, s, dchunk, (int)nd, rig_shared, vol_split, sat);
                else hipLaunchKernelGGL((sweep_std_nhwc_v_kernel<2, false>), grid, block, 0, st, feats, grids, vmask, vol, s, dchunk, (int)nd, rig_shared, vol_split, sat);
                break;
        case 3: if (C == 16) hipLaunchKernelGGL((sweep_std_nhwc_v_kernel<3, true>), grid, block, 0, st, feats, grids, vmask, vol, s, dchunk, (int)nd, rig_shared, vol_split, sat);
                else hipLaunchKernelGGL((sweep_std_nhwc_v_kernel<3, false>), grid, block, 0, st, feats, grids, vmask, vol, s, dchunk, (int)nd, rig_shared, vol_split, sat);
                break;
        case 4: if (C == 16) hipLaunchKernelGGL((sweep_std_nhwc_v_kernel<4, true>), grid, block, 0, st, feats, grids, vmask, vol, s, dchunk, (int)nd, rig_shared, vol_split, sat);
                else hipLaunchKernelGGL((sweep_std_nhwc_v_kernel<4, false>), grid, block, 0, st, feats, grids, vmask, vol, s, dchunk, (int)nd, rig_shared, vol_split, sat);
                break;
    }
    return mvsgi::check_launch("mvsgi_sweep_std_nhwc_valid_f32");
}
}

extern "C" int mvsgi_sweep_std_nhwc_valid_f32(const float* feats, const float* grids, const unsigned char* vmask,
                                              float* vol, int B, int N, int C, int Hi, int Wi, int D, int Ho, int Wo,
                                              mvsgi_stream_t stream) {
    return sweep_std_nhwc_valid_impl(feats, grids, vmask, vol, B, N, C, Hi, Wi, D, Ho, Wo, 0, stream);
}

extern "C" int mvsgi_sweep_std_nhwc_valid_split(const float* feats, const float* grids, const unsigned char* vmask,
                                                void* vol_split, int B, int N, int C, int Hi, int Wi, int D, int Ho, int Wo,
                                                int rig_batch, mvsgi_stream_t stream) {
    MVSGI_REQUIRE(rig_batch == 1 || rig_batch == B, "mvsgi_sweep_std_nhwc_valid_split: rig_batch %d not in {1, B}", rig_batch);
    return sweep_std_nhwc_valid_impl(feats, grids, vmask, nullptr, B, N, C, Hi, Wi, D, Ho, Wo, rig_batch == 1 && B > 1 ? 1 : 0, stream,
                                     static_cast<unsigned char*>(vol_split));
}
extern "C" int mvsgi_sweep_std_nhwc_valid_split_fmt(const float* feats, const float* grids, const unsigned char* vmask,
                                                    void* vol_split, int B, int N, int C, int Hi, int Wi, int D, int Ho, int Wo,
                                                    int rig_batch, int fmt, mvsgi_stream_t stream) {
    MVSGI_REQUIRE(rig_batch == 1 || rig_batch == B, "mvsgi_sweep_std_nhwc_valid_split: rig_batch %d not in {1, B}", rig_batch);
    return sweep_std_nhwc_valid_impl(feats, grids, vmask, nullptr, B, N, C, Hi, Wi, D, Ho, Wo, rig_batch == 1 && B > 1 ? 1 : 0, stream,
                                     static_cast<unsigned char*>(vol_split), fmt);
}

extern "C" int mvsgi_sweep_std_nhwc_valid_rig_f32(const float* feats, const float* grids, const unsigned char* vmask,
                                                  float* vol, int B, int N, int C, int Hi, int Wi, int D, int Ho, int Wo,
                                                  mvsgi_stream_t stream) {
    return sweep_std_nhwc_valid_impl(feats, grids, vmask, vol, B, N, C, Hi, Wi, D, Ho, Wo, 1, stream);
}
```

### mvs_gi_amd/dropin/cost_volume_builder.py

```python
from __future__ import annotations

from torch import nn, Tensor

import os
import weakref

import torch

from .. import hip_ops as H
from . import common_modules as cm
from .common_modules import NORM3D_TYPE, RELU_TYPE


_RIG_VALIDITY = weakref.WeakKeyDictionary()
_RIG_CACHE_ENV = os.environ.get("MVSGI_RIG_CACHE", "1") != "0"


class _SweepBase(nn.Module):
    cache_rig_constants = True
    __getstate__ = cm.module_getstate

    def __init__(self, num_cams: int, feat_chs: int, post_k_sz: int, norm_type: str = "batch",
                 relu_type: str = "leaky"):
        super().__init__()
        self.num_cams = num_cams
        self.feat_chs = feat_chs
        self.norm_type = NORM3D_TYPE[norm_type]
        self.relu_type = RELU_TYPE[relu_type]
        self.grid_sample_mode = "bilinear"
        self.post_vol = cm.BaseConvBlk3d(in_chs=feat_chs, out_chs=feat_chs, kernel_size=post_k_sz,
                                         activation=self.relu_type(), norm_layer=self.norm_type(feat_chs))


def _rig_hit(entry, tensors) -> bool:
    return entry is not None and all(a is b for a, b in zip(entry[0], tensors)) \
        and entry[1] == tuple(t._version for t in tensors)


def _rig_cache_usable(owner, feats, grids) -> bool:
    return owner is not None and getattr(owner, "cache_rig_constants", True) and _RIG_CACHE_ENV \
        and H.nhwc_sweep_ok(feats) and grids.is_cuda


def _owned_split_buffer(owner, attr: str, key: tuple, make):
    bufs = owner.__dict__.setdefault(attr, {})
    if key not in bufs:
        bufs[key] = make()
    return bufs[key]


def std_sweep_ndhwc(feats, grids, grid_masks, masks, owner=None, split_out: bool = False, buf_frames: int = 0):
    use_cache = _rig_cache_usable(owner, feats, grids)
    if not use_cache:
        return None if split_out else H.sweep_std(feats, grids, grid_masks, masks)
    tensors = (grids, grid_masks, masks)
    cached = _RIG_VALIDITY.get(owner)
    if not _rig_hit(cached, tensors):
        if all(t.dim() > 0 and t.shape[0] > 1 and t.stride(0) == 0 for t in tensors):
            g1, gm1, m1 = (t[:1].contiguous() for t in tensors)
        else:
            g1, gm1, m1 = grids, grid_masks, masks
        cached = (tensors, tuple(t._version for t in tensors), H.sweep_validity(g1, gm1, m1), g1 if g1 is not grids else None)
        _RIG_VALIDITY[owner] = cached
    if torch.cuda.is_current_stream_capturing():
        pins = owner.__dict__.setdefault("_mvsgi_graph_pins", [])
        if not any(p is cached for p in pins):
            pins.append(cached)
    g_use = cached[3] if cached[3] is not None else grids
    if split_out:
        B, D, Ho, Wo = feats.shape[0], grids.shape[2], grids.shape[3], grids.shape[4]
        nb = max(B, int(buf_frames))
        full = _owned_split_buffer(owner, "_mvsgi_rs_vol", (nb, D, Ho, Wo, feats.device),
                                   lambda: H.SplitAct(nb, D, Ho, Wo, 16, feats.device))
        out = full if nb == B else H.SplitAct(B, D, Ho, Wo, 16, feats.device, buf=full.buf[:B])
        return H.sweep_std_valid_split(feats, g_use, cached[2], out=out, fmt=H.mode_fmt())
    return H.sweep_std_valid(feats, g_use, cached[2])


def cat_sweep_ndhwc(feats, grids) -> Tensor:
    return H.sweep_cat(feats, grids)


_USE_RS = True
_FRONT_CHUNK = int(os.environ.get("MVSGI_FRONT_CHUNK", "16"))


def _std_front(self, feats: Tensor, grids: Tensor, grid_masks: Tensor, masks: Tensor, hand_over_split: bool):
    L = cm.lower_conv_block(self.post_vol)
    if not (_USE_RS and H.split_mode() and L.cin == 16 and L.cout == 16 and L.stride == 1 and L.inorm is None
            and 0.0 <= L.neg_slope <= 1.0 and feats.dim() == 5 and feats.shape[2] == 16 and grids.dim() == 6):
        return None
    B, D, Ho, Wo = feats.shape[0], grids.shape[2], grids.shape[3], grids.shape[4]
    if not _rig_cache_usable(self, feats, grids):
        return None
    wp_rs, sc_rs = L._rs(H.mode_fmt())
    xs = None
    if hand_over_split:
        xs = _owned_split_buffer(self, "_mvsgi_rs_x0", (B, D, Ho, Wo, feats.device), lambda: H.SplitAct(B, D, Ho, Wo, 16, feats.device))
    k = _FRONT_CHUNK
    shared = all(t.dim() > 0 and t.shape[0] > 1 and t.stride(0) == 0 for t in (grids, grid_masks, masks))
    if k > 0 and B > k and shared:
        y = None if hand_over_split else torch.empty((B, D, Ho, Wo, 16), device=feats.device, dtype=torch.float32)
        for i in range(0, B, k):
            j = min(i + k, B)
            vs = std_sweep_ndhwc(feats[i:j], grids, grid_masks, masks, owner=self, split_out=True, buf_frames=k)
            if hand_over_split:
                H.conv3d_rs16(vs, wp_rs, sc_rs, L.shift, neg_slope=L.neg_slope,
                              out_split=H.SplitAct(j - i, D, Ho, Wo, 16, feats.device, buf=xs.buf[i:j]))
            else:
                H.conv3d_rs16(vs, wp_rs, sc_rs, L.shift, neg_slope=L.neg_slope, out=y[i:j])
        if hand_over_split:
            xs.fmt = H.mode_fmt()
        return xs if hand_over_split else y
    vs = std_sweep_ndhwc(feats, grids, grid_masks, masks, owner=self, split_out=True)
    if hand_over_split:
        return H.conv3d_rs16(vs, wp_rs, sc_rs, L.shift, neg_slope=L.neg_slope, out_split=xs)
    return H.conv3d_rs16(vs, wp_rs, sc_rs, L.shift, neg_slope=L.neg_slope)


def std_forward(self, feats: Tensor, grids: Tensor, grid_masks: Tensor, masks: Tensor) -> Tensor:
    y = _std_front(self, feats, grids, grid_masks, masks, False)
    if y is not None:
        return cm._to_ncdhw_view(y)
    L = cm.lower_conv_block(self.post_vol)
    vol_raw = std_sweep_ndhwc(feats, grids, grid_masks, masks, owner=self)
    return cm._to_ncdhw_view(L.run(vol_raw))


def std_forward_split(self, feats: Tensor, grids: Tensor, grid_masks: Tensor, masks: Tensor):
    return _std_front(self, feats, grids, grid_masks, masks, True)


def cat_forward(self, feats: Tensor, grids: Tensor, grid_masks: Tensor, masks: Tensor) -> Tensor:
    vol_raw = cat_sweep_ndhwc(feats, grids)
    return cm._to_ncdhw_view(cm.lower_conv_block(self.post_vol).run(vol_raw))


class SphericalSweepStdMasked(_SweepBase):
    def sweep(self, feats: Tensor, grids: Tensor, grid_masks: Tensor, masks: Tensor) -> Tensor:
        return cm._to_ncdhw_view(std_sweep_ndhwc(feats, grids, grid_masks, masks, owner=self))

    forward = std_forward
    forward_split = std_forward_split


class SphericalSweep(_SweepBase):
    def sweep(self, feats: Tensor, grids: Tensor, masks: Tensor = None) -> Tensor:
        return cm._to_ncdhw_view(cat_sweep_ndhwc(feats, grids))

    forward = cat_forward
```

### mvs_gi_amd/hip_ops.py

```python
from __future__ import annotations

from typing import Optional

import torch

from . import _lib

import math
import os

CONV_AUTO, CONV_DIRECT, CONV_MFMA, CONV_BF16X3, CONV_BF16X3_C16, CONV_BF16X3_V32, CONV_BF16X3_D32 = 0, 1, 2, 3, 4, 5, 6
SPLIT_F16 = 1
CONV_F16 = 0x100

CONV_MODES = ("f32", "bf16x3", "f16x3")
_CONV_MODE = os.environ.get("MVSGI_CONV_MODE", "f16x3")
if _CONV_MODE not in CONV_MODES:
    raise ValueError(f"MVSGI_CONV_MODE={_CONV_MODE!r} not in {CONV_MODES}")




def set_conv_mode(mode: str) -> None:
    global _CONV_MODE
    if mode not in CONV_MODES:
        raise ValueError(f"conv mode {mode!r} not in {CONV_MODES}")
    _CONV_MODE = mode


def get_conv_mode() -> str:
    return _CONV_MODE


SAT_SWEEP, SAT_SPLIT, SAT_WINO = 1, 2, 4
_SAT_TEXT = {SAT_SWEEP: "the sweep's cost volume reached +-65504 (un-normalised features?)",
             SAT_SPLIT: "an activation written or staged in fp16 pieces reached +-65504",
             SAT_WINO: "an activation of the Winograd-form level reached its +-16376 range (or a transformed sum +-65504)"}
RANGE_CHECKS = ("raise", "warn", "off")
_RANGE_CHECK = os.environ.get("MVSGI_RANGE_CHECK", "raise")
if _RANGE_CHECK not in RANGE_CHECKS:
    raise ValueError(f"MVSGI_RANGE_CHECK={_RANGE_CHECK!r} not in {RANGE_CHECKS}")
_RANGE_WARNED = set()
_RANGE_SEEN = 0


class MvsgiRangeError(RuntimeError):
    """The fp16 split left its range: results since the last check are saturated, not the reference's."""


def set_range_check(policy: str) -> None:
    global _RANGE_CHECK
    if policy not in RANGE_CHECKS:
        raise ValueError(f"range check policy {policy!r} not in {RANGE_CHECKS}")
    _RANGE_CHECK = policy


def get_range_check() -> str:
    return _RANGE_CHECK


def saturation_flags(clear: bool = False) -> int:
    import ctypes
    out = ctypes.c_uint(0)
    if _lib.load().mvsgi_saturation_flags(1 if clear else 0, ctypes.byref(out)) != 0:
        return 0
    return int(out.value)


def saturation_words():
    import ctypes
    out = (ctypes.c_uint * 8)()
    if _lib.load().mvsgi_saturation_words(out) != 0:
        return [0] * 8
    return [int(v) for v in out]


def range_flags_seen() -> int:
    return _RANGE_SEEN


def check_range(where: str = "", sync_device=None) -> int:
    if _RANGE_CHECK == "off":
        return 0
    if sync_device is not None:
        torch.cuda.synchronize(sync_device)
    f = saturation_flags(clear=False)
    if not f:
        return 0
    words = saturation_words()
    saturation_flags(clear=True)
    global _RANGE_SEEN
    _RANGE_SEEN |= f
    what = "; ".join(t for b, t in _SAT_TEXT.items() if f & b)
    msg = (f"mvs_gi_amd{' (' + where + ')' if where else ''}: the fp16 split (MVSGI_CONV_MODE=f16x3, the default) left its range (flags 0x{f:x}, words {words[:4]}) -- {what}. "
           "Results computed since the last check are saturated, not the reference's fp32 results "
           "(dsta_mvs/model/common/common_modules.py:105-115 has no clamp). Re-run with MVSGI_CONV_MODE=bf16x3 "
           "(hip_ops.set_conv_mode('bf16x3'): fp32's range, ~8x the rounding error) or 'f32'; HotPath.precision_check(frames) measures "
           "which arithmetic a checkpoint needs. MVSGI_RANGE_CHECK=warn|off relaxes this check.")
    if _RANGE_CHECK == "raise":
        raise MvsgiRangeError(msg)
    if f not in _RANGE_WARNED:
        _RANGE_WARNED.add(f)
        import warnings
        warnings.warn(msg, RuntimeWarning, stacklevel=2)
    return f


def split_mode() -> bool:
    return _CONV_MODE in ("bf16x3", "f16x3")


def mode_fmt() -> str:
    return "f16" if _CONV_MODE == "f16x3" else "bf16"


def _fmt_code(fmt: str) -> int:
    if fmt not in ("bf16", "f16"):
        raise ValueError(f"split format {fmt!r} not in ('bf16', 'f16')")
    return SPLIT_F16 if fmt == "f16" else 0


def _pow2_unscale(amax: torch.Tensor):
    k = torch.where(amax > 0, torch.floor(torch.log2(1024.0 / amax.clamp_min(1e-37))), torch.zeros_like(amax)).clamp(-100.0, 100.0)
    return torch.exp2(k), torch.exp2(-k)


def _stream_ptr(t: torch.Tensor) -> int:
    return torch.cuda.current_stream(t.device).cuda_stream


def _dev(t: torch.Tensor, name: str, dtype=torch.float32) -> torch.Tensor:
    if not isinstance(t, torch.Tensor):
        raise TypeError(f"{name}: expected a torch.Tensor, got {type(t)}")
    if not t.is_cuda:
        raise RuntimeError(f"{name}: mvs_gi_amd runs on the GPU only (tensor is on {t.device}); "
                           "there is no CPU fallback")
    if t.dtype != dtype:
        raise TypeError(f"{name}: expected {dtype}, got {t.dtype}")
    if not t.is_contiguous():
        t = t.contiguous()
    if t.data_ptr() % 16:
        t = t.clone()
    return t


def _ptr(t: Optional[torch.Tensor]) -> Optional[int]:
    return None if t is None else t.data_ptr()


def _feats_nhwc(feats):
    if feats.dim() != 5:
        raise AssertionError(f"feats must be [B, N, C, Hi, Wi], got {tuple(feats.shape)}")
    v = feats.permute(0, 1, 3, 4, 2)
    if v.is_contiguous() and v.data_ptr() % 16 == 0 and v.is_cuda and v.dtype == torch.float32:
        return v
    lib = _lib.load()
    f = _dev(feats, "feats")
    B, N, C, Hi, Wi = f.shape
    y = torch.empty((B, N, Hi, Wi, C), device=f.device, dtype=torch.float32)
    _lib.check(lib.mvsgi_ncv_to_nvc_f32(f.data_ptr(), y.data_ptr(), B * N, C, Hi * Wi, _stream_ptr(f)),
               "mvsgi_ncv_to_nvc_f32")
    return y


def nhwc_sweep_ok(feats) -> bool:
    return feats.dim() == 5 and feats.shape[2] % 4 == 0 and feats.shape[1] <= 4


def sweep_validity(grids, grid_masks, masks) -> torch.Tensor:
    lib = _lib.load()
    grids = _dev(grids, "grids")
    masks = _dev(masks, "masks")
    gm, gm_f32 = _gm_arg(grid_masks)
    B, N, D, Ho, Wo, two = grids.shape
    if two != 2 or N > 8:
        raise AssertionError(f"grids must be [B, N<=8, D, Ho, Wo, 2], got {tuple(grids.shape)}")
    if tuple(gm.shape[:5]) != (B, N, D, Ho, Wo) or gm.numel() != B * N * D * Ho * Wo:
        raise AssertionError(f"grid_masks {tuple(gm.shape)} do not match grids {tuple(grids.shape)}")
    if masks.shape[0] != B or masks.shape[1] != N or masks.numel() != B * N * masks.shape[-2] * masks.shape[-1]:
        raise AssertionError(f"masks {tuple(masks.shape)} do not match grids {tuple(grids.shape)}")
    Hm, Wm = masks.shape[-2:]
    vmask = torch.empty((B, D, Ho, Wo), device=grids.device, dtype=torch.uint8)
    _lib.check(lib.mvsgi_sweep_validity_u8(grids.data_ptr(), gm.data_ptr(), gm_f32, masks.data_ptr(), vmask.data_ptr(),
                                           B, N, Hm, Wm, D, Ho, Wo, _stream_ptr(grids)), "mvsgi_sweep_validity_u8")
    return vmask


def sweep_std_valid(feats, grids, vmask) -> torch.Tensor:
    lib = _lib.load()
    if not nhwc_sweep_ok(feats):
        raise AssertionError(f"sweep_std_valid needs C % 4 == 0 and N <= 4, got feats {tuple(feats.shape)}")
    B, N, C, Hi, Wi = feats.shape
    f = _feats_nhwc(feats)
    grids = _dev(grids, "grids")
    vmask = _dev(vmask, "vmask", torch.uint8)
    Bg, Ng, D, Ho, Wo, two = grids.shape
    if (Ng, two) != (N, 2) or Bg not in (1, B):
        raise AssertionError(f"grids {tuple(grids.shape)} do not match feats {tuple(feats.shape)}")
    if tuple(vmask.shape) != (Bg, D, Ho, Wo):
        raise AssertionError(f"vmask {tuple(vmask.shape)} does not match grids {tuple(grids.shape)}")
    vol = torch.empty((B, D, Ho, Wo, C), device=f.device, dtype=torch.float32)
    fn = lib.mvsgi_sweep_std_nhwc_valid_rig_f32 if (Bg == 1 and B > 1) else lib.mvsgi_sweep_std_nhwc_valid_f32
    _lib.check(fn(f.data_ptr(), grids.data_ptr(), vmask.data_ptr(), vol.data_ptr(), B, N, C, Hi, Wi, D, Ho, Wo, _stream_ptr(f)),
               "mvsgi_sweep_std_nhwc_valid_f32")
    return vol


def sweep_std_valid_split(feats, grids, vmask, out: "SplitAct", fmt: str = "bf16") -> "SplitAct":
    lib = _lib.load()
    B, N, C, Hi, Wi = feats.shape
    f = _feats_nhwc(feats)
    grids = _dev(grids, "grids")
    vmask = _dev(vmask, "vmask", torch.uint8)
    Bg, Ng, D, Ho, Wo, two = grids.shape
    if (Ng, two) != (N, 2) or Bg not in (1, B) or tuple(vmask.shape) != (Bg, D, Ho, Wo) or C != 16:
        raise AssertionError(f"grids {tuple(grids.shape)} / vmask {tuple(vmask.shape)} do not match feats {tuple(feats.shape)}")
    if out.shape != (B, D, Ho, Wo, C):
        raise AssertionError(f"split output {out.shape} does not match {(B, D, Ho, Wo, C)}")
    _lib.check(lib.mvsgi_sweep_std_nhwc_valid_split_fmt(f.data_ptr(), grids.data_ptr(), vmask.data_ptr(), out.buf.data_ptr(), B, N, C, Hi,
                                                        Wi, D, Ho, Wo, Bg, _fmt_code(fmt), _stream_ptr(f)), "mvsgi_sweep_std_nhwc_valid_split")
    out.fmt = fmt
    return out


def sweep_std(feats, grids, grid_masks, masks, layout: str = "auto") -> torch.Tensor:
    lib = _lib.load()
    if layout == "auto" and nhwc_sweep_ok(feats):
        return _sweep_std_nhwc(feats, grids, grid_masks, masks)
    feats = _dev(feats, "feats")
    grids = _dev(grids, "grids")
    masks = _dev(masks, "masks")
    if grid_masks.dtype == torch.bool:
        gm = _dev(grid_masks, "grid_masks", torch.bool)
        gm_f32 = 0
    elif grid_masks.dtype == torch.uint8:
        gm = _dev(grid_masks, "grid_masks", torch.uint8)
        gm_f32 = 0
    else:
        gm = _dev(grid_masks.to(torch.float32) if grid_masks.dtype != torch.float32 else grid_masks, "grid_masks")
        gm_f32 = 1
    B, N, C, Hi, Wi = feats.shape
    Bg, Ng, D, Ho, Wo, two = grids.shape
    if (Bg, Ng, two) != (B, N, 2):
        raise AssertionError(f"grids {tuple(grids.shape)} do not match feats {tuple(feats.shape)}")
    if tuple(gm.shape[:5]) != (B, N, D, Ho, Wo) or gm.numel() != B * N * D * Ho * Wo:
        raise AssertionError(f"grid_masks {tuple(gm.shape)} do not match grids {tuple(grids.shape)}")
    if masks.shape[0] != B or masks.shape[1] != N or masks.numel() != B * N * masks.shape[-2] * masks.shape[-1]:
        raise AssertionError(f"masks {tuple(masks.shape)} do not match feats {tuple(feats.shape)}")
    Hm, Wm = masks.shape[-2:]
    vol = torch.empty((B, D, Ho, Wo, C), device=feats.device, dtype=torch.float32)
    _lib.check(lib.mvsgi_sweep_std_f32(feats.data_ptr(), grids.data_ptr(), gm.data_ptr(), gm_f32, masks.data_ptr(),
                                       vol.data_ptr(), B, N, C, Hi, Wi, Hm, Wm, D, Ho, Wo, _stream_ptr(feats)),
               "mvsgi_sweep_std_f32")
    return vol


def _gm_arg(grid_masks):
    if grid_masks.dtype == torch.bool:
        return _dev(grid_masks, "grid_masks", torch.bool), 0
    if grid_masks.dtype == torch.uint8:
        return _dev(grid_masks, "grid_masks", torch.uint8), 0
    return _dev(grid_masks.to(torch.float32) if grid_masks.dtype != torch.float32 else grid_masks, "grid_masks"), 1


def _sweep_std_nhwc(feats, grids, grid_masks, masks) -> torch.Tensor:
    lib = _lib.load()
    B, N, C, Hi, Wi = feats.shape
    f = _feats_nhwc(feats)
    grids = _dev(grids, "grids")
    masks = _dev(masks, "masks")
    gm, gm_f32 = _gm_arg(grid_masks)
    Bg, Ng, D, Ho, Wo, two = grids.shape
    if (Bg, Ng, two) != (B, N, 2):
        raise AssertionError(f"grids {tuple(grids.shape)} do not match feats {tuple(feats.shape)}")
    if tuple(gm.shape[:5]) != (B, N, D, Ho, Wo) or gm.numel() != B * N * D * Ho * Wo:
        raise AssertionError(f"grid_masks {tuple(gm.shape)} do not match grids {tuple(grids.shape)}")
    if masks.shape[0] != B or masks.shape[1] != N or masks.numel() != B * N * masks.shape[-2] * masks.shape[-1]:
        raise AssertionError(f"masks {tuple(masks.shape)} do not match feats {tuple(feats.shape)}")
    Hm, Wm = masks.shape[-2:]
    vol = torch.empty((B, D, Ho, Wo, C), device=f.device, dtype=torch.float32)
    _lib.check(lib.mvsgi_sweep_std_nhwc_f32(f.data_ptr(), grids.data_ptr(), gm.data_ptr(), gm_f32, masks.data_ptr(),
                                            vol.data_ptr(), B, N, C, Hi, Wi, Hm, Wm, D, Ho, Wo, _stream_ptr(f)),
               "mvsgi_sweep_std_nhwc_f32")
    return vol


def sweep_cat(feats, grids, layout: str = "auto") -> torch.Tensor:
    lib = _lib.load()
    if layout == "auto" and feats.dim() == 5 and feats.shape[2] % 4 == 0:
        B, N, C, Hi, Wi = feats.shape
        f = _feats_nhwc(feats)
        grids = _dev(grids, "grids")
        Bg, Ng, D, Ho, Wo, two = grids.shape
        if (Bg, Ng, two) != (B, N, 2):
            raise AssertionError(f"grids {tuple(grids.shape)} do not match feats {tuple(feats.shape)}")
        vol = torch.empty((B, D, Ho, Wo, N * C), device=f.device, dtype=torch.float32)
        _lib.check(lib.mvsgi_sweep_cat_nhwc_f32(f.data_ptr(), grids.data_ptr(), vol.data_ptr(), B, N, C, Hi, Wi, D,
                                                Ho, Wo, _stream_ptr(f)), "mvsgi_sweep_cat_nhwc_f32")
        return vol
    feats = _dev(feats, "feats")
    grids = _dev(grids, "grids")
    B, N, C, Hi, Wi = feats.shape
    Bg, Ng, D, Ho, Wo, two = grids.shape
    if (Bg, Ng, two) != (B, N, 2):
        raise AssertionError(f"grids {tuple(grids.shape)} do not match feats {tuple(feats.shape)}")
    vol = torch.empty((B, D, Ho, Wo, N * C), device=feats.device, dtype=torch.float32)
    _lib.check(lib.mvsgi_sweep_cat_f32(feats.data_ptr(), grids.data_ptr(), vol.data_ptr(), B, N, C, Hi, Wi, D, Ho, Wo,
                                       _stream_ptr(feats)), "mvsgi_sweep_cat_f32")
    return vol


def pack_conv_weights(w_oidhw: torch.Tensor) -> Optional[torch.Tensor]:
    lib = _lib.load()
    w = _dev(w_oidhw, "conv weight")
    Cout, Cin = w.shape[:2]
    if tuple(w.shape[2:]) != (3, 3, 3):
        raise NotImplementedError(f"only 3x3x3 kernels are supported, got {tuple(w.shape[2:])}")
    if Cin % 16 or not (Cout % 16 == 0 or Cout == 1):
        return None
    wp = torch.empty(lib.mvsgi_conv3d_packed_weight_floats(Cout, Cin), device=w.device, dtype=torch.float32)
    _lib.check(lib.mvsgi_conv3d_pack_weights_f32(w.data_ptr(), wp.data_ptr(), Cout, Cin, _stream_ptr(w)),
               "mvsgi_conv3d_pack_weights_f32")
    return wp


def pack_conv_weights_bf16x3(w_oidhw: torch.Tensor) -> Optional[torch.Tensor]:
    lib = _lib.load()
    w = _dev(w_oidhw, "conv weight")
    Cout, Cin = w.shape[:2]
    if tuple(w.shape[2:]) != (3, 3, 3) or Cin % 16 or Cout % 16:
        return None
    wp = torch.empty(lib.mvsgi_conv3d_packed_weight_bytes_bf16x3(Cout, Cin), device=w.device, dtype=torch.uint8)
    _lib.check(lib.mvsgi_conv3d_pack_weights_bf16x3(w.data_ptr(), wp.data_ptr(), Cout, Cin, _stream_ptr(w)),
               "mvsgi_conv3d_pack_weights_bf16x3")
    return wp


def pack_conv_weights_f16x3(w_oidhw: torch.Tensor, layout: int = CONV_BF16X3):
    lib = _lib.load()
    w = _dev(w_oidhw, "conv weight")
    Cout, Cin = w.shape[:2]
    if tuple(w.shape[2:]) != (3, 3, 3) or Cin % 16 or Cout % 16 or (layout == CONV_BF16X3_C16 and Cout != 16) or \
            (layout == CONV_BF16X3_V32 and Cout % 32) or (layout == CONV_BF16X3_D32 and Cin % 32):
        return None
    amax = w.abs().amax(dim=(1, 2, 3, 4))
    k = torch.where(amax > 0, torch.floor(torch.log2(1024.0 / amax.clamp_min(1e-37))), torch.zeros_like(amax)).clamp(-100.0, 100.0)
    ws = (w * torch.exp2(k).view(-1, 1, 1, 1, 1)).contiguous()
    n = {CONV_BF16X3: lambda: lib.mvsgi_conv3d_packed_weight_bytes_bf16x3(Cout, Cin),
         CONV_BF16X3_C16: lambda: lib.mvsgi_conv3d_packed_weight_bytes_bf16x3_c16(Cin),
         CONV_BF16X3_D32: lambda: lib.mvsgi_conv3d_packed_weight_bytes_bf16x3(Cout, Cin),
         CONV_BF16X3_V32: lambda: lib.mvsgi_conv3d_packed_weight_bytes_bf16x3_v32(Cout, Cin)}[layout]()
    wp = torch.empty(n, device=w.device, dtype=torch.uint8)
    _lib.check(lib.mvsgi_conv3d_pack_weights_split(ws.data_ptr(), wp.data_ptr(), Cout, Cin, layout | CONV_F16, _stream_ptr(w)),
               "mvsgi_conv3d_pack_weights_split")
    return wp, torch.exp2(-k).contiguous()


def conv3d_d32_applies(B, Cin, Din, Hin, Win, Cout, stride=1) -> bool:
    return bool(_lib.load().mvsgi_conv3d_d32_applies(B, Cin, Din, Hin, Win, Cout, stride))


def conv3d_up2_d32_applies(B, Cin, Dl, Hl, Wl, Cout) -> bool:
    return bool(_lib.load().mvsgi_conv3d_up2_d32_applies(B, Cin, Dl, Hl, Wl, Cout))


def pack_conv_weights_bf16x3_d32(w_oidhw: torch.Tensor) -> Optional[torch.Tensor]:
    lib = _lib.load()
    w = _dev(w_oidhw, "conv weight")
    Cout, Cin = w.shape[:2]
    if tuple(w.shape[2:]) != (3, 3, 3) or Cin % 32 or Cout % 16:
        return None
    wp = torch.empty(lib.mvsgi_conv3d_packed_weight_bytes_bf16x3(Cout, Cin), device=w.device, dtype=torch.uint8)
    _lib.check(lib.mvsgi_conv3d_pack_weights_split(w.data_ptr(), wp.data_ptr(), Cout, Cin, CONV_BF16X3_D32, _stream_ptr(w)),
               "mvsgi_conv3d_pack_weights_split")
    return wp


def conv3d_v32_applies(B, Cin, Din, Hin, Win, Cout, stride=1) -> bool:
    return bool(_lib.load().mvsgi_conv3d_v32_applies(B, Cin, Din, Hin, Win, Cout, stride))


def pack_conv_weights_bf16x3_v32(w_oidhw: torch.Tensor) -> Optional[torch.Tensor]:
    lib = _lib.load()
    w = _dev(w_oidhw, "conv weight")
    Cout, Cin = w.shape[:2]
    if tuple(w.shape[2:]) != (3, 3, 3) or Cin % 16 or Cout % 32:
        return None
    wp = torch.empty(lib.mvsgi_conv3d_packed_weight_bytes_bf16x3_v32(Cout, Cin), device=w.device, dtype=torch.uint8)
    _lib.check(lib.mvsgi_conv3d_pack_weights_bf16x3_v32(w.data_ptr(), wp.data_ptr(), Cout, Cin, _stream_ptr(w)),
               "mvsgi_conv3d_pack_weights_bf16x3_v32")
    return wp


def pack_conv_weights_bf16x3_c16(w_oidhw: torch.Tensor) -> Optional[torch.Tensor]:
    lib = _lib.load()
    w = _dev(w_oidhw, "conv weight")
    Cout, Cin = w.shape[:2]
    if tuple(w.shape[2:]) != (3, 3, 3) or Cin % 16 or Cout != 16:
        return None
    wp = torch.empty(lib.mvsgi_conv3d_packed_weight_bytes_bf16x3_c16(Cin), device=w.device, dtype=torch.uint8)
    _lib.check(lib.mvsgi_conv3d_pack_weights_bf16x3_c16(w.data_ptr(), wp.data_ptr(), Cin, _stream_ptr(w)),
               "mvsgi_conv3d_pack_weights_bf16x3_c16")
    return wp


def conv3d(x, w_oidhw, w_packed, scale, shift, res=None, stride=1, neg_slope=0.01, impl=CONV_AUTO, out=None):
    lib = _lib.load()
    x = _dev(x, "x")
    B, Din, Hin, Win, Cin = x.shape
    Cout = scale.numel()
    Do, Ho, Wo = (Din - 1) // stride + 1, (Hin - 1) // stride + 1, (Win - 1) // stride + 1
    if res is not None:
        res = _dev(res, "res")
        if tuple(res.shape) != (B, Do, Ho, Wo, Cout):
            raise AssertionError(f"residual {tuple(res.shape)} does not match output {(B, Do, Ho, Wo, Cout)}")
    y = out if out is not None else torch.empty((B, Do, Ho, Wo, Cout), device=x.device, dtype=torch.float32)
    _lib.check(lib.mvsgi_conv3d_f32(x.data_ptr(), _ptr(w_oidhw), _ptr(w_packed), scale.data_ptr(), shift.data_ptr(),
                                    _ptr(res), y.data_ptr(), B, Cin, Din, Hin, Win, Cout, stride, float(neg_slope),
                                    impl, _stream_ptr(x)), "mvsgi_conv3d_f32")
    return y


def conv3d_up2(x, w_packed_b3, scale, shift, res=None, neg_slope=0.01, out=None, w_layout=CONV_BF16X3):
    lib = _lib.load()
    x = _dev(x, "x")
    B, Dl, Hl, Wl, Cin = x.shape
    Cout = scale.numel()
    shp = (B, 2 * Dl, 2 * Hl, 2 * Wl, Cout)
    if res is not None:
        res = _dev(res, "res")
        if tuple(res.shape) != shp:
            raise AssertionError(f"residual {tuple(res.shape)} does not match output {shp}")
    y = out if out is not None else torch.empty(shp, device=x.device, dtype=torch.float32)
    _lib.check(lib.mvsgi_conv3d_up2_f32(x.data_ptr(), _ptr(w_packed_b3), w_layout, scale.data_ptr(), shift.data_ptr(), _ptr(res),
                                        y.data_ptr(), B, Cin, Dl, Hl, Wl, Cout, float(neg_slope), _stream_ptr(x)),
               "mvsgi_conv3d_up2_f32")
    return y


def conv3d_up2_out_split(x, w_packed_b3, scale, shift, out: "SplitAct", res=None, neg_slope=0.01, w_layout=CONV_BF16X3) -> "SplitAct":
    lib = _lib.load()
    x = _dev(x, "x")
    B, Dl, Hl, Wl, Cin = x.shape
    Cout = scale.numel()
    if out.shape != (B, 2 * Dl, 2 * Hl, 2 * Wl, Cout):
        raise AssertionError(f"split output {out.shape} does not match {(B, 2 * Dl, 2 * Hl, 2 * Wl, Cout)}")
    if res is not None:
        res = _dev(res, "res")
        if tuple(res.shape) != out.shape:
            raise AssertionError(f"residual {tuple(res.shape)} does not match output {out.shape}")
    _lib.check(lib.mvsgi_conv3d_up2_f32_out_split(x.data_ptr(), _ptr(w_packed_b3), w_layout, scale.data_ptr(), shift.data_ptr(), _ptr(res),
                                                  out.buf.data_ptr(), B, Cin, Dl, Hl, Wl, Cout, float(neg_slope), _stream_ptr(x)),
               "mvsgi_conv3d_up2_f32_out_split")
    out.fmt = "f16" if w_layout & CONV_F16 else "bf16"
    return out


def conv3d_up2_poly_applies(cin: int, cout: int, neg_slope: float) -> bool:
    return cin == 32 and cout == 16 and 0.0 <= neg_slope <= 1.0


def conv3d_up2_poly_plan(w_oidhw: torch.Tensor, D: int, H: int, W: int, fmt: str = "bf16"):
    lib = _lib.load()
    if tuple(w_oidhw.shape) != (16, 32, 3, 3, 3):
        raise AssertionError(f"polyphase plan needs a [16, 32, 3, 3, 3] weight, got {tuple(w_oidhw.shape)}")
    n = lib.mvsgi_conv3d_up2_poly_plan_bytes(D, H, W)
    if not n:
        raise RuntimeError("mvsgi_conv3d_up2_poly_plan_bytes: bad dims")
    wh = w_oidhw.detach().to("cpu", torch.float32).contiguous()
    unscale = None
    if fmt == "f16":
        up, un = _pow2_unscale(wh.abs().amax(dim=(1, 2, 3, 4)))
        wh = (wh * up.view(-1, 1, 1, 1, 1)).contiguous()
        unscale = un.to(w_oidhw.device)
    plan = torch.empty(n, dtype=torch.uint8)
    _lib.check(lib.mvsgi_conv3d_up2_poly_plan_fmt(wh.data_ptr(), plan.data_ptr(), D, H, W, _fmt_code(fmt)), "mvsgi_conv3d_up2_poly_plan")
    plan = plan.to(w_oidhw.device)
    return (plan, unscale) if fmt == "f16" else plan


def conv3d_up2_poly(x: "SplitAct", plan: torch.Tensor, scale, shift, neg_slope=0.01, out=None) -> torch.Tensor:
    lib = _lib.load()
    if x.C != 32 or scale.numel() != 16:
        raise AssertionError("conv3d_up2_poly is the 32 -> 16 kernel")
    shp = (x.B, 2 * x.D, 2 * x.H, 2 * x.W, 16)
    y = out if out is not None else torch.empty(shp, device=x.buf.device, dtype=torch.float32)
    if tuple(y.shape) != shp or not y.is_contiguous():
        raise AssertionError(f"output {tuple(y.shape)} does not match {shp}")
    _lib.check(lib.mvsgi_conv3d_up2_poly_fmt(x.buf.data_ptr(), plan.data_ptr(), scale.data_ptr(), shift.data_ptr(), y.data_ptr(), 0,
                                             x.B, x.D, x.H, x.W, float(neg_slope), _fmt_code(x.fmt), _stream_ptr(x.buf)),
               "mvsgi_conv3d_up2_poly_f32")
    return y


POLY_WINO = os.environ.get("MVSGI_POLY_WINO", "1") != "0"


def conv3d_up2_poly_wino_pays(B: int, D: int, Hh: int, W: int) -> bool:
    return POLY_WINO and bool(_lib.load().mvsgi_conv3d_up2_poly_wino_pays(int(B), int(D), int(Hh), int(W)))


def conv3d_up2_poly_split(x: "SplitAct", plan: torch.Tensor, scale, shift, out: "SplitAct", neg_slope=0.01, direct: bool = False,
                          wino: bool = False) -> "SplitAct":
    lib = _lib.load()
    if x.C != 32 or scale.numel() != 16 or out.shape != (x.B, 2 * x.D, 2 * x.H, 2 * x.W, 16):
        raise AssertionError(f"conv3d_up2_poly_split: input {x.shape}, output {out.shape}")
    _lib.check(lib.mvsgi_conv3d_up2_poly_fmt(x.buf.data_ptr(), plan.data_ptr(), scale.data_ptr(), shift.data_ptr(), out.buf.data_ptr(),
                                             5 if wino else (3 if (direct or not POLY_WINO) else 1),
                                             x.B, x.D, x.H, x.W, float(neg_slope), _fmt_code(x.fmt), _stream_ptr(x.buf)),
               "mvsgi_conv3d_up2_poly_split")
    out.fmt = x.fmt
    return out


def pack_head_split_weights(w_oidhw: torch.Tensor) -> Optional[torch.Tensor]:
    lib = _lib.load()
    w = _dev(w_oidhw, "conv weight")
    if w.shape[0] != 1 or tuple(w.shape[2:]) != (3, 3, 3) or w.shape[1] % 16:
        return None
    wp = torch.empty(lib.mvsgi_conv3d_head_split_packed_weight_bytes(int(w.shape[1])), device=w.device, dtype=torch.uint8)
    _lib.check(lib.mvsgi_conv3d_head_split_pack_weights(w.data_ptr(), wp.data_ptr(), int(w.shape[1]), _stream_ptr(w)),
               "mvsgi_conv3d_head_split_pack_weights")
    return wp


def pack_head_split_weights_f16(w_oidhw: torch.Tensor):
    lib = _lib.load()
    w = _dev(w_oidhw, "conv weight")
    if w.shape[0] != 1 or tuple(w.shape[2:]) != (3, 3, 3) or w.shape[1] % 16:
        return None
    amax = float(w.abs().max())
    k = 0.0 if amax == 0.0 else float(torch.floor(torch.log2(torch.tensor(1024.0 / amax))))
    ws = (w * (2.0 ** k)).contiguous()
    wp = torch.empty(lib.mvsgi_conv3d_head_split_packed_weight_bytes(int(w.shape[1])), device=w.device, dtype=torch.uint8)
    _lib.check(lib.mvsgi_conv3d_head_split_pack_weights_f16(ws.data_ptr(), wp.data_ptr(), int(w.shape[1]), _stream_ptr(w)),
               "mvsgi_conv3d_head_split_pack_weights_f16")
    return wp, 2.0 ** -k


def conv3d_head_split(x: "SplitAct", w_packed, scale: float, shift: float, neg_slope=1.0, out=None, f16: bool = False) -> torch.Tensor:
    lib = _lib.load()
    if x.fmt != ("f16" if f16 else "bf16"):
        raise AssertionError(f"conv3d_head_split(f16={f16}) on a split-padded buffer holding {x.fmt} pieces")
    y = out if out is not None else torch.empty((x.B, x.D, x.H, x.W, 1), device=x.buf.device, dtype=torch.float32)
    if tuple(y.shape) != (x.B, x.D, x.H, x.W, 1) or not y.is_contiguous():
        raise AssertionError(f"head output {tuple(y.shape)} does not match {(x.B, x.D, x.H, x.W, 1)}")
    fn = lib.mvsgi_conv3d_head_split_f16 if f16 else lib.mvsgi_conv3d_head_split
    _lib.check(fn(x.buf.data_ptr(), w_packed.data_ptr(), float(scale), float(shift), y.data_ptr(), x.B, x.C,
                  x.D, x.H, x.W, float(neg_slope), _stream_ptr(x.buf)), "mvsgi_conv3d_head_split")
    return y


def conv3d_up2_variant(B, Cin, Dl, Hl, Wl, Cout, w_layout=CONV_BF16X3) -> str:
    lib = _lib.load()
    name = lib.mvsgi_conv3d_up2_variant_f32(B, Cin, Dl, Hl, Wl, Cout, w_layout)
    if name is None:
        raise RuntimeError("mvsgi_conv3d_up2_variant_f32: " + lib.mvsgi_last_error().decode())
    return name.decode()


def conv3d_variant(B, Cin, Din, Hin, Win, Cout, stride=1, impl=CONV_AUTO) -> str:
    lib = _lib.load()
    name = lib.mvsgi_conv3d_variant_f32(B, Cin, Din, Hin, Win, Cout, stride, impl)
    if name is None:
        raise RuntimeError("mvsgi_conv3d_variant_f32: " + lib.mvsgi_last_error().decode())
    return name.decode()


class SplitAct:
    __slots__ = ("buf", "B", "D", "H", "W", "C", "fmt")

    def __init__(self, B, D, H, W, C, device, buf=None):
        self.B, self.D, self.H, self.W, self.C = int(B), int(D), int(H), int(W), int(C)
        self.fmt = "bf16"
        if buf is None:
            buf = torch.zeros((self.B, self.D + 2, self.H + 2, self.W + 2, self.C), device=device, dtype=torch.int32)
        self.buf = buf

    @property
    def shape(self):
        return (self.B, self.D, self.H, self.W, self.C)

    @property
    def device(self):
        return self.buf.device


def act_to_split(x_ndhwc: torch.Tensor, out: Optional[SplitAct] = None, fmt: str = "bf16") -> SplitAct:
    lib = _lib.load()
    x = _dev(x_ndhwc, "x")
    B, D, Hh, W, C = x.shape
    y = out if out is not None else SplitAct(B, D, Hh, W, C, x.device)
    if y.shape != (B, D, Hh, W, C):
        raise AssertionError(f"split buffer {y.shape} does not match {tuple(x.shape)}")
    _lib.check(lib.mvsgi_act_f32_to_split_fmt(x.data_ptr(), y.buf.data_ptr(), B, C, D, Hh, W, _fmt_code(fmt), _stream_ptr(x)),
               "mvsgi_act_f32_to_split")
    y.fmt = fmt
    return y


def act_from_split(x: SplitAct, out: Optional[torch.Tensor] = None) -> torch.Tensor:
    lib = _lib.load()
    y = out if out is not None else torch.empty(x.shape, device=x.buf.device, dtype=torch.float32)
    _lib.check(lib.mvsgi_act_split_to_f32_fmt(x.buf.data_ptr(), y.data_ptr(), x.B, x.C, x.D, x.H, x.W, _fmt_code(x.fmt), _stream_ptr(x.buf)),
               "mvsgi_act_split_to_f32")
    return y


def pack_conv_weights_rs(w_oidhw: torch.Tensor, fmt: str = "bf16"):
    lib = _lib.load()
    w = _dev(w_oidhw, "conv weight")
    unscale = None
    if fmt == "f16":
        up, unscale = _pow2_unscale(w.abs().amax(dim=(1, 2, 3, 4)))
        w = (w * up.view(-1, 1, 1, 1, 1)).contiguous()
    Cout, Cin = w.shape[:2]
    nbytes = lib.mvsgi_conv3d_rs_packed_weight_bytes(Cout, Cin) if tuple(w.shape[2:]) == (3, 3, 3) else 0
    if not nbytes:
        return None
    wp = torch.empty(nbytes, device=w.device, dtype=torch.uint8)
    _lib.check(lib.mvsgi_conv3d_rs_pack_weights_fmt(w.data_ptr(), wp.data_ptr(), Cout, Cin, _fmt_code(fmt), _stream_ptr(w)),
               "mvsgi_conv3d_rs_pack_weights")
    return (wp, unscale.contiguous()) if fmt == "f16" else wp


def conv3d_rs(x: SplitAct, w_packed_rs, scale, shift, res: Optional[SplitAct] = None, neg_slope=0.01,
              out=None, out_f32: bool = False):
    lib = _lib.load()
    Cout = scale.numel()
    if out_f32:
        y = out if out is not None else torch.empty((x.B, x.D, x.H, x.W, Cout), device=x.buf.device, dtype=torch.float32)
        yp = y.data_ptr()
        if tuple(y.shape) != (x.B, x.D, x.H, x.W, Cout) or not y.is_contiguous():
            raise AssertionError(f"fp32 output {tuple(y.shape)} does not match {(x.B, x.D, x.H, x.W, Cout)}")
    else:
        y = out if out is not None else SplitAct(x.B, x.D, x.H, x.W, Cout, x.buf.device)
        yp = y.buf.data_ptr()
        if y.shape != (x.B, x.D, x.H, x.W, Cout):
            raise AssertionError(f"split output {y.shape} does not match {(x.B, x.D, x.H, x.W, Cout)}")
    if res is not None and (res.shape != (x.B, x.D, x.H, x.W, Cout) or res.fmt != x.fmt):
        raise AssertionError(f"residual {res.shape} ({res.fmt}) does not match the output ({x.fmt})")
    _lib.check(lib.mvsgi_conv3d_rs_split_fmt(x.buf.data_ptr(), w_packed_rs.data_ptr(), scale.data_ptr(), shift.data_ptr(),
                                             None if res is None else res.buf.data_ptr(), yp, int(out_f32), x.B, x.C, x.D, x.H,
                                             x.W, Cout, float(neg_slope), _fmt_code(x.fmt), _stream_ptr(x.buf)), "mvsgi_conv3d_rs_split")
    if not out_f32:
        y.fmt = x.fmt
    return y


def conv3d_wino_applies(cin, cout, D, Hh, W, stride, neg_slope) -> bool:
    return bool(_lib.load().mvsgi_conv3d_wino32_applies(int(cin), int(cout), int(D), int(Hh), int(W), int(stride), float(neg_slope)))


def pack_conv_weights_wino(w_oidhw: torch.Tensor):
    lib = _lib.load()
    w = _dev(w_oidhw, "conv weight")
    if tuple(w.shape) != (32, 32, 3, 3, 3):
        return None
    wp = torch.empty(lib.mvsgi_conv3d_wino32_packed_weight_bytes(), device=w.device, dtype=torch.uint8)
    unscale = torch.empty(32, device=w.device, dtype=torch.float32)
    _lib.check(lib.mvsgi_conv3d_wino32_pack_weights(w.data_ptr(), wp.data_ptr(), unscale.data_ptr(), _stream_ptr(w)),
               "mvsgi_conv3d_wino32_pack_weights")
    return wp, unscale


F32P_MAX = 16376.0


def act_to_f32p(x_ndhwc: torch.Tensor, out: Optional[SplitAct] = None) -> SplitAct:
    x = _dev(x_ndhwc, "x")
    B, D, Hh, W, C = x.shape
    y = out if out is not None else SplitAct(B, D, Hh, W, C, x.device)
    y.buf.view(torch.float32)[:, 1:-1, 1:-1, 1:-1, :] = x.clamp(-F32P_MAX, F32P_MAX)
    y.fmt = "f32p"
    return y


def act_from_f32p(x: SplitAct) -> torch.Tensor:
    if x.fmt != "f32p":
        raise AssertionError(f"buffer holds {x.fmt} records")
    return x.buf.view(torch.float32)[:, 1:-1, 1:-1, 1:-1, :].contiguous()


def conv3d_wino(x: SplitAct, w_packed, scale, shift, res: Optional[SplitAct] = None, neg_slope=0.01, out=None, out_f32: bool = False,
                ):
    lib = _lib.load()
    if x.fmt not in ("f16", "f32p") or x.C != 32:
        raise AssertionError(f"conv3d_wino: needs a 32-channel input in the fp16 split or fp32-padded (got {x.C}, {x.fmt})")
    if out_f32:
        y = out if out is not None else torch.empty(x.shape, device=x.buf.device, dtype=torch.float32)
        if tuple(y.shape) != x.shape or not y.is_contiguous() or y.dtype != torch.float32:
            raise AssertionError(f"fp32 output {tuple(y.shape)} does not match {x.shape}")
        yp = y.data_ptr()
    else:
        y = out if out is not None else SplitAct(x.B, x.D, x.H, x.W, 32, x.buf.device)
        if y.shape != x.shape:
            raise AssertionError(f"split output {y.shape} does not match {x.shape}")
        yp = y.buf.data_ptr()
    if res is not None and (res.shape != x.shape or res.fmt != x.fmt):
        raise AssertionError(f"residual {res.shape} ({res.fmt}) does not match the input ({x.fmt})")
    if w_packed.numel() != lib.mvsgi_conv3d_wino32_packed_weight_bytes():
        raise AssertionError("conv3d_wino: packed weights of the wrong size")
    _lib.check(lib.mvsgi_conv3d_wino32_f16(x.buf.data_ptr(), w_packed.data_ptr(), scale.data_ptr(), shift.data_ptr(),
                                           None if res is None else res.buf.data_ptr(), yp, int(out_f32), int(x.fmt == "f32p"),
                                           x.B, x.D, x.H, x.W, float(neg_slope), _stream_ptr(x.buf)), "mvsgi_conv3d_wino32_f16")
    if not out_f32:
        y.fmt = x.fmt
    return y


def conv3d_out_split(x, w_packed_b3, scale, shift, out: "SplitAct", res=None, stride=1, neg_slope=0.01, fmt: str = "bf16") -> "SplitAct":
    lib = _lib.load()
    x = _dev(x, "x")
    B, Din, Hin, Win, Cin = x.shape
    Cout = scale.numel()
    Do, Ho, Wo = (Din - 1) // stride + 1, (Hin - 1) // stride + 1, (Win - 1) // stride + 1
    if out.shape != (B, Do, Ho, Wo, Cout):
        raise AssertionError(f"split output {out.shape} does not match {(B, Do, Ho, Wo, Cout)}")
    if res is not None:
        res = _dev(res, "res")
    _lib.check(lib.mvsgi_conv3d_f32_out_split_fmt(x.data_ptr(), w_packed_b3.data_ptr(), scale.data_ptr(), shift.data_ptr(), _ptr(res),
                                                  out.buf.data_ptr(), B, Cin, Din, Hin, Win, Cout, stride, float(neg_slope),
                                                  _fmt_code(fmt), _stream_ptr(x)), "mvsgi_conv3d_f32_out_split")
    out.fmt = fmt
    return out


def conv3d_rs16(x: "SplitAct", w_packed_rs, scale, shift, neg_slope=0.01, out=None, out_split: Optional["SplitAct"] = None):
    lib = _lib.load()
    if x.C != 16 or scale.numel() != 16:
        raise AssertionError("conv3d_rs16 is the 16 -> 16 kernel")
    if out_split is not None:
        if out_split.shape != x.shape or out_split.buf.data_ptr() == x.buf.data_ptr():
            raise AssertionError(f"split output {out_split.shape} must match the input {x.shape} and be another buffer")
        _lib.check(lib.mvsgi_conv3d_rs16_split_fmt(x.buf.data_ptr(), w_packed_rs.data_ptr(), scale.data_ptr(), shift.data_ptr(),
                                                   out_split.buf.data_ptr(), 1, x.B, x.D, x.H, x.W, float(neg_slope), _fmt_code(x.fmt),
                                                   _stream_ptr(x.buf)), "mvsgi_conv3d_rs16_split_out_split")
        out_split.fmt = x.fmt
        return out_split
    y = out if out is not None else torch.empty((x.B, x.D, x.H, x.W, 16), device=x.buf.device, dtype=torch.float32)
    _lib.check(lib.mvsgi_conv3d_rs16_split_fmt(x.buf.data_ptr(), w_packed_rs.data_ptr(), scale.data_ptr(), shift.data_ptr(), y.data_ptr(), 0,
                                               x.B, x.D, x.H, x.W, float(neg_slope), _fmt_code(x.fmt), _stream_ptr(x.buf)),
               "mvsgi_conv3d_rs16_split")
    return y


def conv3d_s2rs_applies(cin: int, cout: int, stride: int, neg_slope: float) -> bool:
    return cin == 16 and cout == 32 and stride == 2 and 0.0 <= neg_slope <= 1.0


def pack_conv_weights_s2rs(w_oidhw: torch.Tensor, scale: torch.Tensor, fmt: str = "bf16"):
    lib = _lib.load()
    w = _dev(w_oidhw, "w")
    scale = _dev(scale, "scale")
    if tuple(w.shape) != (32, 16, 3, 3, 3) or scale.numel() != 32:
        raise AssertionError(f"conv3d_s2rs is the 16 -> 32 channel stride-2 layer, got weights {tuple(w.shape)}")
    up = un = None
    if fmt == "f16":
        up_t, un_t = _pow2_unscale((w.abs().amax(dim=(1, 2, 3, 4)) * scale.abs()).max().reshape(1))
        up, un = float(up_t[0]), float(un_t[0])
        scale = (scale * up).contiguous()
    wp = torch.empty(lib.mvsgi_conv3d_s2rs_packed_weight_bytes(), device=w.device, dtype=torch.uint8)
    _lib.check(lib.mvsgi_conv3d_s2rs_pack_weights_fmt(w.data_ptr(), scale.data_ptr(), wp.data_ptr(), _fmt_code(fmt), _stream_ptr(w)),
               "mvsgi_conv3d_s2rs_pack_weights")
    return (wp, up, un) if fmt == "f16" else wp


def conv3d_s2rs(x: "SplitAct", w_packed, shift, out: "SplitAct", neg_slope=0.01, unscale: float = 1.0, out_f32p: bool = False) -> "SplitAct":
    lib = _lib.load()
    Do, Ho, Wo = (x.D - 1) // 2 + 1, (x.H - 1) // 2 + 1, (x.W - 1) // 2 + 1
    if x.C != 16 or out.shape != (x.B, Do, Ho, Wo, 32) or shift.numel() != 32:
        raise AssertionError(f"conv3d_s2rs: input {x.shape} -> output {out.shape}, expected {(x.B, Do, Ho, Wo, 32)}")
    _lib.check(lib.mvsgi_conv3d_s2rs_out_fmt(x.buf.data_ptr(), w_packed.data_ptr(), shift.data_ptr(), out.buf.data_ptr(), x.B, x.D, x.H, x.W,
                                             float(neg_slope), float(unscale), _fmt_code(x.fmt), int(out_f32p), _stream_ptr(x.buf)),
               "mvsgi_conv3d_s2rs")
    out.fmt = "f32p" if out_f32p else x.fmt
    return out


def conv3d_rs_applies(cin: int, cout: int, stride: int, neg_slope: float) -> bool:
    return cin == 32 and cout == 32 and stride == 1 and 0.0 <= neg_slope <= 1.0


def pack_conv2d_weights_bf16x3(w_oihw: torch.Tensor) -> Optional[torch.Tensor]:
    lib = _lib.load()
    w = _dev(w_oihw, "conv weight")
    Cout, Cin = w.shape[:2]
    if tuple(w.shape[2:]) != (3, 3) or Cin % 16 or Cout % 16:
        return None
    wp = torch.empty(lib.mvsgi_conv2d_packed_weight_bytes_bf16x3(Cout, Cin), device=w.device, dtype=torch.uint8)
    _lib.check(lib.mvsgi_conv2d_pack_weights_bf16x3(w.data_ptr(), wp.data_ptr(), Cout, Cin, _stream_ptr(w)),
               "mvsgi_conv2d_pack_weights_bf16x3")
    return wp


def pack_conv2d_stem_weights(w_oihw: torch.Tensor) -> Optional[torch.Tensor]:
    lib = _lib.load()
    w = _dev(w_oihw, "conv weight")
    if tuple(w.shape) != (16, 3, 5, 5):
        return None
    wp = torch.empty(lib.mvsgi_conv2d_stem_packed_weight_bytes(), device=w.device, dtype=torch.uint8)
    _lib.check(lib.mvsgi_conv2d_stem_pack_weights(w.data_ptr(), wp.data_ptr(), _stream_ptr(w)), "mvsgi_conv2d_stem_pack_weights")
    return wp


def pack_conv2d_weights_f32(w_oihw: torch.Tensor) -> Optional[torch.Tensor]:
    lib = _lib.load()
    w = _dev(w_oihw, "conv weight")
    Cout, Cin = w.shape[:2]
    if tuple(w.shape[2:]) != (3, 3) or Cin % 16 or Cout not in (16, 32):
        return None
    wp = torch.empty(lib.mvsgi_conv2d_packed_weight_floats(Cout, Cin), device=w.device, dtype=torch.float32)
    _lib.check(lib.mvsgi_conv2d_pack_weights_f32(w.data_ptr(), wp.data_ptr(), Cout, Cin, _stream_ptr(w)),
               "mvsgi_conv2d_pack_weights_f32")
    return wp


def conv2d(x, w_oihw, w_packed, scale, shift, res=None, stride=1, neg_slope=0.01, impl=CONV_AUTO, in_nchw=False, out_split=None):
    lib = _lib.load()
    layout = int(bool(in_nchw))
    if x.dtype == torch.uint8:
        x = _dev(x, "imgs", torch.uint8)
        B, Hin, Win, Cin = x.shape
        layout = 2
    else:
        x = _dev(x, "x")
        if in_nchw:
            B, Cin, Hin, Win = x.shape
        else:
            B, Hin, Win, Cin = x.shape
    Cout, k = scale.numel(), int(w_oihw.shape[-1])
    pad = k // 2
    Ho, Wo = (Hin + 2 * pad - k) // stride + 1, (Win + 2 * pad - k) // stride + 1
    if res is not None:
        res = _dev(res, "res")
        if tuple(res.shape) != (B, Ho, Wo, Cout):
            raise AssertionError(f"residual {tuple(res.shape)} does not match output {(B, Ho, Wo, Cout)}")
    if out_split is not None:
        _check_split2d(out_split, B, Ho, Wo, x.device)
        _lib.check(lib.mvsgi_conv2d_f32_out_split2d(x.data_ptr(), _ptr(w_oihw), _ptr(w_packed), scale.data_ptr(), shift.data_ptr(),
                                                    _ptr(res), out_split.data_ptr(), B, Cin, Hin, Win, Cout, k, stride,
                                                    float(neg_slope), impl, layout, _stream_ptr(x)), "mvsgi_conv2d_f32_out_split2d")
        return out_split
    y = torch.empty((B, Ho, Wo, Cout), device=x.device, dtype=torch.float32)
    _lib.check(lib.mvsgi_conv2d_f32(x.data_ptr(), _ptr(w_oihw), _ptr(w_packed), scale.data_ptr(), shift.data_ptr(),
                                    _ptr(res), y.data_ptr(), B, Cin, Hin, Win, Cout, k, stride, float(neg_slope), impl,
                                    layout, _stream_ptr(x)), "mvsgi_conv2d_f32")
    return y


def conv2d_variant(Cin, Cout, k=3, stride=1, impl=CONV_AUTO, in_nchw=False) -> str:
    lib = _lib.load()
    name = lib.mvsgi_conv2d_variant_f32(Cin, Cout, k, stride, impl, int(bool(in_nchw)))
    if name is None:
        raise RuntimeError("mvsgi_conv2d_variant_f32: " + lib.mvsgi_last_error().decode())
    return name.decode()


def resize_trilinear(x, size) -> torch.Tensor:
    lib = _lib.load()
    x = _dev(x, "x")
    B, Di, Hi, Wi, C = x.shape
    Do, Ho, Wo = (int(s) for s in size)
    y = torch.empty((B, Do, Ho, Wo, C), device=x.device, dtype=torch.float32)
    _lib.check(lib.mvsgi_resize_trilinear_f32(x.data_ptr(), y.data_ptr(), B, C, Di, Hi, Wi, Do, Ho, Wo,
                                              _stream_ptr(x)), "mvsgi_resize_trilinear_f32")
    return y


def instance_norm(x, res=None, gamma=None, beta=None, eps: float = 1e-5, neg_slope: float = 1.0, out=None) -> torch.Tensor:
    lib = _lib.load()
    x = _dev(x, "x")
    B, C = int(x.shape[0]), int(x.shape[-1])
    S = x.numel() // max(B * C, 1)
    if S < 2:
        raise ValueError(f"Expected more than 1 spatial element when training, got input size "
                         f"{[B, C] + list(x.shape[1:-1])}")
    if res is not None:
        res = _dev(res, "res")
        if tuple(res.shape) != tuple(x.shape):
            raise AssertionError(f"residual {tuple(res.shape)} does not match {tuple(x.shape)}")
    for t, name in ((gamma, "gamma"), (beta, "beta")):
        if t is not None and (t.numel() != C or not t.is_cuda or t.dtype != torch.float32 or not t.is_contiguous()):
            raise AssertionError(f"{name} must be a contiguous fp32 [{C}] device tensor")
    if out is None:
        out = torch.empty_like(x)
    elif out.data_ptr() != x.data_ptr():
        out = _dev(out, "out")
        if tuple(out.shape) != tuple(x.shape) or out.data_ptr() % 16:
            raise AssertionError(f"out {tuple(out.shape)} does not match {tuple(x.shape)}")
    nbytes = lib.mvsgi_instance_norm_ws_bytes(B, S, C)
    ws = torch.empty(max(int(nbytes), 16), device=x.device, dtype=torch.uint8)
    _lib.check(lib.mvsgi_instance_norm_f32(x.data_ptr(), _ptr(res), _ptr(gamma), _ptr(beta), out.data_ptr(), ws.data_ptr(),
                                           B, S, C, float(eps), float(neg_slope), _stream_ptr(x)), "mvsgi_instance_norm_f32")
    return out


SA_AUTO, SA_PIXEL, SA_BAND = 0, 1, 2


def softargmin(costs_bdhw, inv_idx, scale: float, want_norm_costs: bool, post_div: float = 1.0, variant: int = SA_AUTO):
    lib = _lib.load()
    c = _dev(costs_bdhw, "costs")
    inv_idx = _dev(inv_idx.reshape(-1), "inv_dist_idx")
    B, D, H, W = c.shape
    if inv_idx.numel() != D:
        raise AssertionError(f"{D} cost planes but {inv_idx.numel()} distance candidates")
    scale = float(scale)
    if not (math.isfinite(scale) and scale > 0):
        raise ValueError(f"softargmin: scale {scale} is not a finite positive factor")
    OH, OW = math.floor(H * scale), math.floor(W * scale)
    if OH < 1 or OW < 1:
        raise ValueError(f"softargmin: scale {scale} gives an empty {OH} x {OW} output for {H} x {W}")
    inv = torch.empty((B, 1, OH, OW), device=c.device, dtype=torch.float32)
    pr = torch.empty((B, D, OH, OW), device=c.device, dtype=torch.float32) if want_norm_costs else None
    if variant == SA_AUTO and scale in (1.0, 2.0):
        _lib.check(lib.mvsgi_softargmin_div_f32(c.data_ptr(), inv_idx.data_ptr(), inv.data_ptr(), _ptr(pr), B, D, H, W,
                                                int(scale), float(post_div), _stream_ptr(c)), "mvsgi_softargmin_div_f32")
    else:
        _lib.check(lib.mvsgi_softargmin_scaled_f32(c.data_ptr(), inv_idx.data_ptr(), inv.data_ptr(), _ptr(pr), B, D, H, W,
                                                   scale, OH, OW, float(post_div), int(variant), _stream_ptr(c)),
                   "mvsgi_softargmin_scaled_f32")
    return inv, pr


def ncdhw_to_ndhwc(x) -> torch.Tensor:
    lib = _lib.load()
    x = _dev(x, "x")
    B, C, D, H, W = x.shape
    y = torch.empty((B, D, H, W, C), device=x.device, dtype=torch.float32)
    _lib.check(lib.mvsgi_ncv_to_nvc_f32(x.data_ptr(), y.data_ptr(), B, C, D * H * W, _stream_ptr(x)),
               "mvsgi_ncv_to_nvc_f32")
    return y


def ndhwc_to_ncdhw(x) -> torch.Tensor:
    lib = _lib.load()
    x = _dev(x, "x")
    B, D, H, W, C = x.shape
    y = torch.empty((B, C, D, H, W), device=x.device, dtype=torch.float32)
    _lib.check(lib.mvsgi_nvc_to_ncv_f32(x.data_ptr(), y.data_ptr(), B, C, D * H * W, _stream_ptr(x)),
               "mvsgi_nvc_to_ncv_f32")
    return y


def as_ndhwc(vol: torch.Tensor) -> torch.Tensor:
    if vol.dim() != 5:
        raise AssertionError(f"expected a [B, C, D, H, W] volume, got {tuple(vol.shape)}")
    v = vol.permute(0, 2, 3, 4, 1)
    if v.is_contiguous():
        return v
    return ncdhw_to_ndhwc(vol.contiguous())


def pack_deform_conv2d_weights(w_oihw: torch.Tensor) -> torch.Tensor:
    lib = _lib.load()
    w = _dev(w_oihw, "deform conv weight")
    Cout, Cin, Kh, Kw = w.shape
    wp = torch.empty((Kh * Kw, Cin, Cout), device=w.device, dtype=torch.float32)
    _lib.check(lib.mvsgi_deform_conv2d_pack_weights_f32(w.data_ptr(), wp.data_ptr(), Cout, Cin, Kh, Kw, _stream_ptr(w)),
               "mvsgi_deform_conv2d_pack_weights_f32")
    return wp


def deform_conv2d(x_nhwc, offset, w_packed, scale, shift, kernel_size, stride=(1, 1), padding=(0, 0), dilation=(1, 1),
                  res=None, neg_slope=1.0) -> torch.Tensor:
    lib = _lib.load()
    x = _dev(x_nhwc, "x")
    offset = _dev(offset, "offset")
    N, Hh, W, Cin = x.shape
    Kh, Kw = kernel_size
    Cout = scale.numel()
    Ho = (Hh + 2 * padding[0] - (dilation[0] * (Kh - 1) + 1)) // stride[0] + 1
    Wo = (W + 2 * padding[1] - (dilation[1] * (Kw - 1) + 1)) // stride[1] + 1
    if offset.dim() != 4 or tuple(offset.shape[1:]) != (2 * Kh * Kw, Ho, Wo) or offset.shape[0] not in (1, N):
        raise AssertionError(f"offset {tuple(offset.shape)} does not match [1|{N}, {2 * Kh * Kw}, {Ho}, {Wo}]")
    if tuple(w_packed.shape) != (Kh * Kw, Cin, Cout):
        raise AssertionError(f"w_packed {tuple(w_packed.shape)} does not match {(Kh * Kw, Cin, Cout)}")
    if res is not None:
        res = _dev(res, "res")
        if tuple(res.shape) != (N, Ho, Wo, Cout):
            raise AssertionError(f"residual {tuple(res.shape)} does not match output {(N, Ho, Wo, Cout)}")
    y = torch.empty((N, Ho, Wo, Cout), device=x.device, dtype=torch.float32)
    _lib.check(lib.mvsgi_deform_conv2d_f32(x.data_ptr(), offset.data_ptr(), int(offset.shape[0] == N and N > 1),
                                           w_packed.data_ptr(), scale.data_ptr(), shift.data_ptr(), _ptr(res),
                                           y.data_ptr(), N, Cin, Hh, W, Cout, Kh, Kw, stride[0], stride[1], padding[0],
                                           padding[1], dilation[0], dilation[1], float(neg_slope), _stream_ptr(x)),
               "mvsgi_deform_conv2d_f32")
    return y


def split2d_buffer(N: int, H: int, W: int, device) -> torch.Tensor:
    return torch.zeros((N, H + 4, W + 4, 64), device=device, dtype=torch.uint8)


def _check_split2d(t: torch.Tensor, N: int, H: int, W: int, device) -> None:
    if t.dtype != torch.uint8 or tuple(t.shape) != (N, H + 4, W + 4, 64) or not t.is_contiguous() or t.device != device:
        raise AssertionError(f"split-padded 2-D buffer {tuple(t.shape)} {t.dtype} {t.device} does not match {(N, H + 4, W + 4, 64)} uint8 on {device}")


def f32_to_split2d(x_nhwc: torch.Tensor, out: Optional[torch.Tensor] = None) -> torch.Tensor:
    lib = _lib.load()
    x = _dev(x_nhwc, "x")
    N, Hh, W, C = x.shape
    if C != 16:
        raise AssertionError(f"the 2-D split-padded format holds 16 channels, got {tuple(x.shape)}")
    if out is None:
        out = split2d_buffer(N, Hh, W, x.device)
    _check_split2d(out, N, Hh, W, x.device)
    _lib.check(lib.mvsgi_f32_to_split2d(x.data_ptr(), out.data_ptr(), N, Hh, W, _stream_ptr(x)), "mvsgi_f32_to_split2d")
    return out


def split2d_to_f32(x_split: torch.Tensor) -> torch.Tensor:
    lib = _lib.load()
    N, Hp, Wp, _ = x_split.shape
    _check_split2d(x_split, N, Hp - 4, Wp - 4, x_split.device)
    y = torch.empty((N, Hp - 4, Wp - 4, 16), device=x_split.device, dtype=torch.float32)
    _lib.check(lib.mvsgi_split2d_to_f32(x_split.data_ptr(), y.data_ptr(), N, Hp - 4, Wp - 4, _stream_ptr(x_split)), "mvsgi_split2d_to_f32")
    return y


def pack_resblock2d_split_weights(w_oihw: torch.Tensor, scale: torch.Tensor) -> torch.Tensor:
    lib = _lib.load()
    w = _dev(w_oihw, "w")
    scale = _dev(scale, "scale")
    if tuple(w.shape) != (16, 16, 3, 3) or scale.numel() != 16:
        raise AssertionError(f"resblock2d_split is the 16 -> 16 channel 3x3 block, got weights {tuple(w.shape)}")
    wp = torch.empty(lib.mvsgi_resblock2d_split_packed_weight_bytes(), device=w.device, dtype=torch.uint8)
    _lib.check(lib.mvsgi_resblock2d_split_pack_weights(w.data_ptr(), scale.data_ptr(), wp.data_ptr(), _stream_ptr(w)),
               "mvsgi_resblock2d_split_pack_weights")
    return wp


def resblock2d_split(x_split, wp1, shift1, wp2, shift2, neg_slope=0.01, out_split=None) -> torch.Tensor:
    lib = _lib.load()
    N, Hp, Wp, _ = x_split.shape
    Hh, W = Hp - 4, Wp - 4
    _check_split2d(x_split, N, Hh, W, x_split.device)
    if shift1.numel() != 16 or shift2.numel() != 16:
        raise AssertionError("resblock2d_split is the 16-channel block")
    if out_split is not None:
        _check_split2d(out_split, N, Hh, W, x_split.device)
        y = out_split
    else:
        y = torch.empty((N, Hh, W, 16), device=x_split.device, dtype=torch.float32)
    _lib.check(lib.mvsgi_resblock2d_split(x_split.data_ptr(), wp1.data_ptr(), shift1.data_ptr(), wp2.data_ptr(), shift2.data_ptr(),
                                          y.data_ptr(), int(out_split is not None), N, Hh, W, float(neg_slope),
                                          _stream_ptr(x_split)), "mvsgi_resblock2d_split")
    return y


def conv2d_s2_split(x_split, w_packed, shift, out_split, neg_slope=0.01) -> torch.Tensor:
    lib = _lib.load()
    N, Hp, Wp, _ = x_split.shape
    Hh, W = Hp - 4, Wp - 4
    _check_split2d(x_split, N, Hh, W, x_split.device)
    _check_split2d(out_split, N, (Hh - 1) // 2 + 1, (W - 1) // 2 + 1, x_split.device)
    if shift.numel() != 16:
        raise AssertionError("conv2d_s2_split is the 16-channel layer")
    _lib.check(lib.mvsgi_conv2d_s2_split(x_split.data_ptr(), w_packed.data_ptr(), shift.data_ptr(), out_split.data_ptr(), N, Hh, W,
                                         float(neg_slope), _stream_ptr(x_split)), "mvsgi_conv2d_s2_split")
    return out_split


def resblock2d(x_nhwc, wp1, scale1, shift1, wp2, scale2, shift2, neg_slope=0.01) -> torch.Tensor:
    lib = _lib.load()
    x = _dev(x_nhwc, "x")
    N, Hh, W, C = x.shape
    if C != 16 or scale1.numel() != 16 or scale2.numel() != 16:
        raise AssertionError(f"resblock2d is the 16-channel block, got x {tuple(x.shape)}")
    y = torch.empty_like(x)
    _lib.check(lib.mvsgi_resblock2d_f32(x.data_ptr(), wp1.data_ptr(), scale1.data_ptr(), shift1.data_ptr(),
                                        wp2.data_ptr(), scale2.data_ptr(), shift2.data_ptr(), y.data_ptr(), N, Hh, W,
                                        float(neg_slope), _stream_ptr(x)), "mvsgi_resblock2d_f32")
    return y
```

Measured before the change: 6374.

## Fuse std-variance sweep with first 3D conv in warp-specialized kernel

Adds a new fused front-end kernel in which producer waves build the std cost-volume slice into an LDS double buffer, one depth plane at a time, while consumer waves run the first 3x3x3 conv with split-fp16 MFMA. The conv accumulates over a rolling window of three depth planes and writes the split output directly. This removes the round trip of the intermediate cost volume through global memory and one kernel launch. The fused path is taken only in f16 mode when a heuristic says there are enough tiles. It adds warp-specialization and barrier complexity, and occupancy is limited to one block per CU.

```diff
diff --git a/__graft_entry__.py b/__graft_entry__.py
--- a/__graft_entry__.py
+++ b/__graft_entry__.py
@@ -5,7 +5,7 @@
 ROOT = os.path.dirname(os.path.abspath(__file__))
 CSRC = os.path.join(ROOT, "mvs_gi_amd", "csrc")
 LIB = os.path.join(ROOT, "mvs_gi_amd", "libmvsgi_hip.so")
-SOURCES = ["api.cpp", "sweep.hip", "conv3d.hip", "conv3d_f16.hip", "conv3d_rs.hip", "conv3d_wino.hip", "conv3d_wino_up2.hip", "conv3d_s2rs.hip", "conv3d_up2poly.hip", "conv3d_headsplit.hip", "conv2d.hip", "resblock2d_rs.hip", "resize.hip", "softargmin.hip", "layout.hip", "grids.hip", "deform_conv2d.hip", "instnorm.hip"]
+SOURCES = ["api.cpp", "sweep.hip", "front_std16.hip", "conv3d.hip", "conv3d_f16.hip", "conv3d_rs.hip", "conv3d_wino.hip", "conv3d_wino_up2.hip", "conv3d_s2rs.hip", "conv3d_up2poly.hip", "conv3d_headsplit.hip", "conv2d.hip", "resblock2d_rs.hip", "resize.hip", "softargmin.hip", "layout.hip", "grids.hip", "deform_conv2d.hip", "instnorm.hip"]
 
 
 SRCHASH = LIB + ".srchash"
diff --git a/include/mvsgi.h b/include/mvsgi.h
--- a/include/mvsgi.h
+++ b/include/mvsgi.h
@@ -8,7 +8,7 @@
 extern "C" {
 #endif
 
-#define MVSGI_ABI_VERSION 5
+#define MVSGI_ABI_VERSION 6
 
 typedef void* mvsgi_stream_t;
 
@@ -232,6 +232,12 @@
 int mvsgi_instance_norm_f32(const float* x, const float* res, const float* gamma, const float* beta, float* y, float* ws,
                             int B, int S, int C, float eps, float neg_slope, mvsgi_stream_t stream);
 
+int mvsgi_front_std16_split_fmt(const float* feats, const float* grids, const unsigned char* vmask, const void* w_packed_rs,
+                                const float* scale, const float* shift, void* y_split, void* vol_split_debug, int B, int N,
+                                int Hi, int Wi, int D, int Ho, int Wo, int rig_batch, float neg_slope, int fmt,
+                                mvsgi_stream_t stream);
+int mvsgi_front_std16_pays(int B, int D, int Ho, int Wo);
+
 #ifdef __cplusplus
 }
 #endif
diff --git a/mvs_gi_amd/_lib.py b/mvs_gi_amd/_lib.py
--- a/mvs_gi_amd/_lib.py
+++ b/mvs_gi_amd/_lib.py
@@ -7,7 +7,7 @@
 _HERE = os.path.dirname(os.path.abspath(__file__))
 LIB_PATH = os.environ.get("MVSGI_LIB", os.path.join(_HERE, "libmvsgi_hip.so"))
 
-ABI_VERSION = 5
+ABI_VERSION = 6
 
 
 class MvsgiLibraryMissing(RuntimeError):
@@ -114,6 +114,8 @@
     "mvsgi_nvc_to_ncv_f32": (c_int, [_P, _P, c_int, c_int, c_longlong, _P]),
     "mvsgi_instance_norm_ws_bytes": (c_size_t, [c_int] * 3),
     "mvsgi_instance_norm_f32": (c_int, [_P] * 6 + [c_int] * 3 + [c_float, c_float, _P]),
+    "mvsgi_front_std16_split_fmt": (c_int, [_P] * 8 + [c_int] * 8 + [c_float, c_int, _P]),
+    "mvsgi_front_std16_pays": (c_int, [c_int] * 4),
 }
 
 _lib = None
diff --git a/mvs_gi_amd/csrc/front_std16.hip b/mvs_gi_amd/csrc/front_std16.hip
--- /dev/null
+++ b/mvs_gi_amd/csrc/front_std16.hip
@@ -0,0 +1,336 @@
+#include "common.hpp"
+
+namespace {
+
+#include "split_fmt.hpp"
+#include "sweep_candidate.hpp"
+
+typedef unsigned fs_u32x4 __attribute__((ext_vector_type(4)));
+typedef unsigned fs_u32x2 __attribute__((ext_vector_type(2)));
+
+namespace fs16 {
+constexpr int TH = 16, TW = 32, ITH = TH + 2, ITW = TW + 2;
+constexpr int PV = ITH * ITW;
+constexpr int NG = (PV + 15) / 16;
+constexpr int ROW = 40;
+constexpr int REGION = ITH * ROW * 32;
+constexpr int PLANE = 2 * REGION;
+constexpr int WBYTES = 5 * 3 * 2 * 64 * 16;
+constexpr int LDS_BYTES = WBYTES + 2 * PLANE;
+constexpr int NP = 8, NC = 8, THREADS = (NP + NC) * 64;
+constexpr int TPW = (TH * TW / 16) / NC;
+static_assert(TPW * NC * 16 == TH * TW, "tiles");
+__host__ __device__ constexpr int pair_kh(int pp, int second) { return pp < 3 ? pp : (pp == 3 ? second : (second ? -1 : 2)); }
+__host__ __device__ constexpr int pair_kw(int pp, int second) { return pp < 3 ? second : 2; }
+}
+
+#ifndef MVSGI_FRONT_ABL
+#define MVSGI_FRONT_ABL 0
+#endif
+
+struct FrontArgs {
+    const float* feats;
+    const float* grids;
+    const unsigned char* vmask;
+    const unsigned char* wp;
+    const float* scale;
+    const float* shift;
+    unsigned char* y;
+    unsigned char* dbg;
+    int B, Hi, Wi, D, Ho, Wo;
+    int rig_shared;
+    float neg_slope;
+    int tiles_h, tiles_w;
+    long long total_units;
+    unsigned* sat;
+};
+
+struct FsUnit {
+    int b, oh0, ow0;
+};
+
+#define FS_PLANE_BARRIER()                                   \
+    {                                                        \
+        asm volatile("s_waitcnt lgkmcnt(0)" ::: "memory");   \
+        __builtin_amdgcn_s_barrier();                        \
+        asm volatile("" ::: "memory");                       \
+    }
+
+template <int NCAM>
+__global__ __launch_bounds__(fs16::THREADS, 1) void front_std16_kernel(FrontArgs a) {
+    using namespace fs16;
+    extern __shared__ __attribute__((aligned(16))) unsigned char lds[];
+    const int tid = threadIdx.x, lane = tid & 63;
+    const int wave = __builtin_amdgcn_readfirstlane(tid >> 6);
+    for (int i = tid; i < WBYTES / 16; i += THREADS)
+        *reinterpret_cast<fs_u32x4*>(lds + i * 16) = *reinterpret_cast<const fs_u32x4*>(a.wp + i * 16);
+
+    const int G = (int)gridDim.x, total = (int)a.total_units;
+    int ubase = 0, ucount = total;
+    int wgs = G, wi = (int)blockIdx.x;
+    if ((G & 7) == 0) {
+        const int x = wi & 7;
+        const int q8 = total >> 3, r8 = total & 7;
+        ubase = x < r8 ? x * (q8 + 1) : r8 * (q8 + 1) + (x - r8) * q8;
+        ucount = q8 + (x < r8 ? 1 : 0);
+        wi >>= 3;
+        wgs = G >> 3;
+    }
+    const int nunits = wi < ucount ? (ucount - wi + wgs - 1) / wgs : 0;
+    const int items = nunits * a.D;
+    const int Hp = a.Ho + 2, Wp = a.Wo + 2;
+    const int HW = a.Ho * a.Wo;
+    auto unit_of = [&](const int k) {
+        unsigned t = (unsigned)(ubase + wi + k * wgs);
+        FsUnit u;
+        u.ow0 = (int)(t % (unsigned)a.tiles_w) * TW;
+        t /= (unsigned)a.tiles_w;
+        u.oh0 = (int)(t % (unsigned)a.tiles_h) * TH;
+        u.b = (int)(t / (unsigned)a.tiles_h);
+        return u;
+    };
+    __syncthreads();
+
+    if (wave < NP) {
+        const int q = lane & 3;
+        const int mycam = q < NCAM ? q : NCAM - 1;
+        const int rowB = a.Wi * 64;
+        const long long img_bytes = (long long)a.Hi * a.Wi * 64;
+        float satm = 0.f;
+        struct Gv {
+            float2 g;
+            unsigned vm;
+        };
+        const int grid_bytes = NCAM * a.D * HW * 8, vm_bytes = a.D * HW;
+        auto fetch = [&](const FsUnit u, const int d, const int g, const bool valid) {
+            const int v = g * 16 + (lane >> 2);
+            const int ih = v / ITW, iw = v - ih * ITW;
+            const int ho = u.oh0 - 1 + ih, wo = u.ow0 - 1 + iw;
+            const bool in = valid && v < PV && (unsigned)ho < (unsigned)a.Ho && (unsigned)wo < (unsigned)a.Wo;
+            const int br = a.rig_shared ? 0 : u.b;
+            const __amdgpu_buffer_rsrc_t dg = __builtin_amdgcn_make_buffer_rsrc(
+                const_cast<float*>(a.grids) + (long long)br * (grid_bytes / 4), 0, grid_bytes, 0x00020000);
+            const __amdgpu_buffer_rsrc_t dv = __builtin_amdgcn_make_buffer_rsrc(
+                const_cast<unsigned char*>(a.vmask) + (long long)br * vm_bytes, 0, vm_bytes, 0x00020000);
+            const int pix = d * HW + ho * a.Wo + wo;
+            Gv r;
+            const sf_f32x2 gw = __builtin_bit_cast(sf_f32x2, __builtin_amdgcn_raw_buffer_load_b64(dg, in ? (mycam * a.D * HW + pix) * 8 : (int)0x80000000, 0, 0));
+            r.g.x = gw.x;
+            r.g.y = gw.y;
+            r.vm = (unsigned)__builtin_amdgcn_raw_buffer_load_b8(dv, in ? pix : (int)0x80000000, 0, 0);
+            return r;
+        };
+        struct Sink {
+            unsigned char* l;
+            unsigned char* g;
+            bool to_l, to_g;
+            __device__ __forceinline__ bool split() const { return true; }
+            __device__ __forceinline__ void f32(const int, const f32x4_t) const {}
+            __device__ __forceinline__ void piece(const uint4 p) const {
+                if (to_l) *reinterpret_cast<uint4*>(l) = p;
+                if (to_g) *reinterpret_cast<uint4*>(g) = p;
+            }
+        };
+        FsUnit u = unit_of(0);
+        Gv cur = fetch(u, 0, wave, items > 0);
+        int d = 0, k = 0;
+        for (int it = 0; it <= items; ++it) {
+            if (it < items) {
+                __amdgpu_buffer_rsrc_t img[NCAM];
+#pragma unroll
+                for (int cam = 0; cam < NCAM; ++cam)
+                    img[cam] = __builtin_amdgcn_make_buffer_rsrc(
+                        const_cast<float*>(a.feats) + ((long long)u.b * NCAM + cam) * (img_bytes / 4), 0, (int)img_bytes, 0x00020000);
+                const bool more = it + 1 < items;
+                const int dn = d + 1 < a.D ? d + 1 : 0;
+                const FsUnit un = (d + 1 < a.D || !more) ? u : unit_of(k + 1);
+                unsigned char* const slot = lds + WBYTES + (int)(it & 1) * PLANE;
+                for (int g = wave; g < NG; g += NP) {
+                    asm volatile("" : "+v"(cur.g.x), "+v"(cur.g.y), "+v"(cur.vm));
+                    const Gv nxt = g + NP < NG ? fetch(u, d, g + NP, true) : fetch(un, dn, wave, more);
+                    const int v = g * 16 + (lane >> 2);
+                    const int ih = v / ITW, iw = v - ih * ITW;
+                    unsigned char* const l = slot + (q & 1) * REGION + (ih * ROW + iw) * 32 + (((q >> 1) ^ ((iw >> 3) & 1)) << 4);
+                    const int ho = u.oh0 - 1 + ih, wo = u.ow0 - 1 + iw;
+                    const bool to_g = a.dbg != nullptr && ih >= 1 && ih <= TH && iw >= 1 && iw <= TW && v < PV && ho < a.Ho && wo < a.Wo;
+                    unsigned char* const gd = a.dbg + ((((long long)u.b * (a.D + 2) + d + 1) * Hp + ho + 1) * Wp + wo + 1) * 64 + ((q & 1) * 2 + (q >> 1)) * 16;
+                    if (!(MVSGI_FRONT_ABL & 2)) sweep_candidate<NCAM, true, true>(img, q, a.Wi, a.Hi, 64, rowB, cur.g, cur.vm, satm, Sink{l, gd, v < PV, to_g});
+                    cur = nxt;
+                }
+                u = un;
+                d = dn;
+                k += dn == 0 ? 1 : 0;
+            }
+            FS_PLANE_BARRIER();
+        }
+        sf_sat_report(a.sat, kSatSweep, satm, kF16Max);
+        return;
+    }
+
+    const int cw = wave - NP;
+    const int col = lane & 15, kg = lane >> 4;
+    const int second = kg & 1, half = kg >> 1;
+    int foff[5];
+#pragma unroll
+    for (int pp = 0; pp < 5; ++pp) {
+        int kh = pair_kh(pp, second), kw = pair_kw(pp, second);
+        if (kh < 0) { kh = 2; kw = 2; }
+        const int w = col + kw;
+        foff[pp] = (kh * ROW + w) * 32 + ((half ^ ((w >> 3) & 1)) << 4);
+    }
+    const f32x4_t esc = *reinterpret_cast<const f32x4_t*>(a.scale + kg * 4), esh = *reinterpret_cast<const f32x4_t*>(a.shift + kg * 4);
+    const sf_bf16x8* const wl = reinterpret_cast<const sf_bf16x8*>(lds) + lane;
+    float satm = 0.f;
+    sf_f32x4 accA[TPW], accB[TPW], accC[TPW];
+#pragma unroll
+    for (int j = 0; j < TPW; ++j) accA[j] = accB[j] = accC[j] = sf_f32x4{0.f, 0.f, 0.f, 0.f};
+    auto epilogue = [&](const FsUnit u, const int od, const sf_f32x4 (&acc)[TPW]) {
+#pragma unroll
+        for (int j = 0; j < TPW; ++j) {
+            const int t = cw * TPW + j;
+            const int oh = u.oh0 + (t >> 1), ow = u.ow0 + (t & 1) * 16 + col;
+            sf_f32x4 f;
+#pragma unroll
+            for (int r = 0; r < 4; ++r) {
+                const float x = __builtin_fmaf(acc[j][r], esc[r], esh[r]);
+                f[r] = sf_clamp<true>(__builtin_fmaxf(x, x * a.neg_slope));
+            }
+            fs_u32x2 hi, lo;
+            sf_split4<true>(f, hi, lo, satm);
+            const fs_u32x2 s0 = __builtin_amdgcn_permlane16_swap(hi[0], lo[0], false, false);
+            const fs_u32x2 s1 = __builtin_amdgcn_permlane16_swap(hi[1], lo[1], false, false);
+            if (oh < a.Ho && ow < a.Wo) {
+                unsigned char* p = a.y + ((((long long)u.b * (a.D + 2) + od + 1) * Hp + oh + 1) * Wp + ow + 1) * 64 + (kg & 1) * 32 + (kg >> 1) * 16;
+                *reinterpret_cast<fs_u32x4*>(p) = fs_u32x4{s0[0], s1[0], s0[1], s1[1]};
+            }
+        }
+    };
+    FsUnit u = unit_of(0);
+    int d = 0, k = 0;
+    for (int it = 0; it <= items; ++it) {
+        if (it > 0 && !(MVSGI_FRONT_ABL & 1)) {
+            const unsigned char* const hi_r = lds + WBYTES + ((it - 1) & 1) * PLANE;
+            sf_bf16x8 wh[3], wlo[3], xh[2], xl[2];
+            auto ldw = [&](const int pp, const int kd) {
+                wh[kd] = wl[((pp * 3 + kd) * 2) * 64];
+                wlo[kd] = wl[((pp * 3 + kd) * 2 + 1) * 64];
+            };
+            auto ldx = [&](const int st) {
+                const int t = cw * TPW + (st & 3);
+                const int base = ((t >> 1) * ROW + (t & 1) * 16) * 32 + foff[st >> 2];
+                xh[st & 1] = *reinterpret_cast<const sf_bf16x8*>(hi_r + base);
+                xl[st & 1] = *reinterpret_cast<const sf_bf16x8*>(hi_r + REGION + base);
+            };
+#pragma unroll
+            for (int kd = 0; kd < 3; ++kd) ldw(0, kd);
+            ldx(0);
+            __builtin_amdgcn_sched_barrier(0);
+#pragma unroll
+            for (int st = 0; st < 20; ++st) {
+                const int pp = st >> 2, j = st & 3, c = st & 1;
+                if (st + 1 < 20) ldx(st + 1);
+                __builtin_amdgcn_sched_barrier(0);
+                if (j < 3 || pp == 4) {
+                    accC[j] = sf_mfma16<true>(wh[0], xh[c], accC[j]);
+                    accB[j] = sf_mfma16<true>(wh[1], xh[c], accB[j]);
+                    accA[j] = sf_mfma16<true>(wh[2], xh[c], accA[j]);
+                    accC[j] = sf_mfma16<true>(wlo[0], xh[c], accC[j]);
+                    accB[j] = sf_mfma16<true>(wlo[1], xh[c], accB[j]);
+                    accA[j] = sf_mfma16<true>(wlo[2], xh[c], accA[j]);
+                    accC[j] = sf_mfma16<true>(wh[0], xl[c], accC[j]);
+                    accB[j] = sf_mfma16<true>(wh[1], xl[c], accB[j]);
+                    accA[j] = sf_mfma16<true>(wh[2], xl[c], accA[j]);
+                } else {
+                    accC[j] = sf_mfma16<true>(wh[0], xh[c], accC[j]);
+                    accC[j] = sf_mfma16<true>(wlo[0], xh[c], accC[j]);
+                    accC[j] = sf_mfma16<true>(wh[0], xl[c], accC[j]);
+                    __builtin_amdgcn_sched_barrier(0);
+                    ldw(pp + 1, 0);
+                    __builtin_amdgcn_sched_barrier(0);
+                    accB[j] = sf_mfma16<true>(wh[1], xh[c], accB[j]);
+                    accB[j] = sf_mfma16<true>(wlo[1], xh[c], accB[j]);
+                    accB[j] = sf_mfma16<true>(wh[1], xl[c], accB[j]);
+                    __builtin_amdgcn_sched_barrier(0);
+                    ldw(pp + 1, 1);
+                    __builtin_amdgcn_sched_barrier(0);
+                    accA[j] = sf_mfma16<true>(wh[2], xh[c], accA[j]);
+                    accA[j] = sf_mfma16<true>(wlo[2], xh[c], accA[j]);
+                    accA[j] = sf_mfma16<true>(wh[2], xl[c], accA[j]);
+                    __builtin_amdgcn_sched_barrier(0);
+                    ldw(pp + 1, 2);
+                }
+                __builtin_amdgcn_sched_barrier(0);
+            }
+            if (d > 0) epilogue(u, d - 1, accA);
+#pragma unroll
+            for (int j = 0; j < TPW; ++j) {
+                accA[j] = accB[j];
+                accB[j] = accC[j];
+                accC[j] = sf_f32x4{0.f, 0.f, 0.f, 0.f};
+            }
+            if (d == a.D - 1) {
+                epilogue(u, d, accA);
+#pragma unroll
+                for (int j = 0; j < TPW; ++j) accA[j] = accB[j] = sf_f32x4{0.f, 0.f, 0.f, 0.f};
+            }
+            if (++d == a.D) {
+                d = 0;
+                u = unit_of(++k);
+            }
+        }
+        FS_PLANE_BARRIER();
+    }
+    sf_sat_report(a.sat, kSatSplit, satm, kF16Max);
+}
+
+#undef FS_PLANE_BARRIER
+
+}
+
+extern "C" int mvsgi_front_std16_pays(int B, int D, int Ho, int Wo) {
+    if (B <= 0 || D < 8 || Ho <= 0 || Wo <= 0) return 0;
+    const long long units = (long long)B * mvsgi::cdiv(Ho, fs16::TH) * mvsgi::cdiv(Wo, fs16::TW);
+    return units >= 4ll * 256 ? 1 : 0;
+}
+
+extern "C" int mvsgi_front_std16_split_fmt(const float* feats, const float* grids, const unsigned char* vmask, const void* w_packed_rs,
+                                           const float* scale, const float* shift, void* y_split, void* vol_split_debug, int B, int N,
+                                           int Hi, int Wi, int D, int Ho, int Wo, int rig_batch, float neg_slope, int fmt,
+                                           mvsgi_stream_t stream) {
+    MVSGI_REQUIRE(fmt == MVSGI_SPLIT_F16, "mvsgi_front_std16_split_fmt: fmt %d is not MVSGI_SPLIT_F16 (the fused front end exists in the fp16 split only)", fmt);
+    MVSGI_REQUIRE(feats && grids && vmask && w_packed_rs && scale && shift && y_split, "mvsgi_front_std16_split_fmt: null pointer");
+    MVSGI_REQUIRE(B > 0 && Hi > 0 && Wi > 0 && D > 0 && Ho > 0 && Wo > 0, "mvsgi_front_std16_split_fmt: non-positive dimension");
+    MVSGI_REQUIRE(N >= 1 && N <= 4, "mvsgi_front_std16_split_fmt: num_cams %d not in [1, 4]", N);
+    MVSGI_REQUIRE(rig_batch == 1 || rig_batch == B, "mvsgi_front_std16_split_fmt: rig_batch %d not in {1, B}", rig_batch);
+    MVSGI_REQUIRE(neg_slope >= 0.f && neg_slope <= 1.f, "mvsgi_front_std16_split_fmt: neg_slope %g not in [0, 1]", (double)neg_slope);
+    MVSGI_REQUIRE((long long)Hi * Wi * 16 < (1ll << 29) && (long long)Wi * 64 < (1ll << 23),
+                  "mvsgi_front_std16_split_fmt: dimensions exceed the launch geometry (image bytes < 2^31, row bytes < 2^23)");
+    MVSGI_REQUIRE((long long)N * D * Ho * Wo * 8 < (1ll << 31), "mvsgi_front_std16_split_fmt: one rig's grids exceed 32-bit offsets (N D Ho Wo 8 < 2^31)");
+    MVSGI_REQUIRE(y_split != vol_split_debug, "mvsgi_front_std16_split_fmt: the debug volume must be another buffer");
+    FrontArgs a{};
+    a.feats = feats;
+    a.grids = grids;
+    a.vmask = vmask;
+    a.wp = static_cast<const unsigned char*>(w_packed_rs);
+    a.scale = scale;
+    a.shift = shift;
+    a.y = static_cast<unsigned char*>(y_split);
+    a.dbg = static_cast<unsigned char*>(vol_split_debug);
+    a.B = B; a.Hi = Hi; a.Wi = Wi; a.D = D; a.Ho = Ho; a.Wo = Wo;
+    a.rig_shared = rig_batch == 1 && B > 1 ? 1 : 0;
+    a.neg_slope = neg_slope;
+    a.tiles_h = (int)mvsgi::cdiv(Ho, fs16::TH);
+    a.tiles_w = (int)mvsgi::cdiv(Wo, fs16::TW);
+    a.total_units = (long long)B * a.tiles_h * a.tiles_w;
+    MVSGI_REQUIRE(a.total_units < (1ll << 31), "mvsgi_front_std16_split_fmt: too many units");
+    MVSGI_SAT_WORDS(sat);
+    a.sat = sat;
+    void (*kern)(FrontArgs) = N == 1 ? front_std16_kernel<1> : N == 2 ? front_std16_kernel<2> : N == 3 ? front_std16_kernel<3> : front_std16_kernel<4>;
+    static mvsgi::PersistentGeom geo_cache[4][mvsgi::kMaxDevices] = {};
+    mvsgi::PersistentGeom geo;
+    if (mvsgi::persistent_geometry(kern, fs16::THREADS, fs16::LDS_BYTES, 1, geo_cache[N - 1], "mvsgi_front_std16_split_fmt", geo)) return 1;
+    const long long resident = (long long)geo.cus * geo.wgs_per_cu;
+    hipLaunchKernelGGL(kern, dim3((unsigned)(a.total_units <= resident ? a.total_units : resident)), dim3(fs16::THREADS), fs16::LDS_BYTES,
+                       mvsgi::as_stream(stream), a);
+    return mvsgi::check_launch("mvsgi_front_std16_split_fmt");
+}
diff --git a/mvs_gi_amd/csrc/sweep.hip b/mvs_gi_amd/csrc/sweep.hip
--- a/mvs_gi_amd/csrc/sweep.hip
+++ b/mvs_gi_amd/csrc/sweep.hip
@@ -4,14 +4,8 @@
 
 #include "split_fmt.hpp"
 
-struct Bilin {
-    int o00, o01, o10, o11;
-    float w00, w01, w10, w11;
-};
-
-#ifndef MVSGI_SWEEP_SKIP_CAM
-#define MVSGI_SWEEP_SKIP_CAM 1
-#endif
+#include "sweep_candidate.hpp"
+
 __device__ __forceinline__ Bilin bilin_setup(float gx, float gy, int W, int H) {
 #pragma clang fp contract(off)
     Bilin t;
@@ -35,30 +29,6 @@
     return t;
 }
 
-__device__ __forceinline__ Bilin bilin_setup_bytes(float gx, float gy, int W, int H, int C4, int rowB) {
-#pragma clang fp contract(off)
-    Bilin t;
-    const float x = ((gx + 1.0f) * (float)W - 1.0f) / 2.0f;
-    const float y = ((gy + 1.0f) * (float)H - 1.0f) / 2.0f;
-    const float xf = floorf(x), yf = floorf(y);
-    const float x1f = xf + 1.0f, y1f = yf + 1.0f;
-    t.w00 = (x1f - x) * (y1f - y);
-    t.w01 = (x1f - x) * (y - yf);
-    t.w10 = (x - xf) * (y1f - y);
-    t.w11 = (x - xf) * (y - yf);
-    const int x0 = (int)fminf(fmaxf(xf, -2.0f), (float)W + 1.0f);
-    const int y0 = (int)fminf(fmaxf(yf, -2.0f), (float)H + 1.0f);
-    const bool vx0 = (unsigned)x0 < (unsigned)W, vx1 = (unsigned)(x0 + 1) < (unsigned)W;
-    const bool vy0 = (unsigned)y0 < (unsigned)H, vy1 = (unsigned)(y0 + 1) < (unsigned)H;
-    const int base = __mul24(y0, rowB) + __mul24(x0, C4);
-    constexpr int kOutside = (int)0x80000000;
-    t.o00 = (vx0 & vy0) ? base : kOutside;
-    t.o01 = (vx0 & vy1) ? base + rowB : kOutside;
-    t.o10 = (vx1 & vy0) ? base + C4 : kOutside;
-    t.o11 = (vx1 & vy1) ? base + rowB + C4 : kOutside;
-    return t;
-}
-
 __device__ __forceinline__ float bilin_fetch(const float* __restrict__ plane, const Bilin& t) {
 #pragma clang fp contract(off)
     const float i00 = t.o00 >= 0 ? plane[t.o00] : 0.0f;
@@ -67,8 +37,6 @@
     const float i11 = t.o11 >= 0 ? plane[t.o11] : 0.0f;
     return ((i00 * t.w00 + i01 * t.w01) + i10 * t.w10) + i11 * t.w11;
 }
-
-typedef float f32x4_t __attribute__((ext_vector_type(4)));
 
 __device__ __forceinline__ float div_small(float x, float d, float inv) {
     const float ax = fabsf(x);
@@ -336,28 +304,6 @@
         bits |= ((sm > 0.0f) && gmv) ? (1u << cam) : 0u;
     }
     vmask[idx] = (unsigned char)bits;
-}
-
-template <int CAM>
-__device__ __forceinline__ int quad_bcast_i(int v) {
-    return __builtin_amdgcn_mov_dpp(v, CAM * 0x55, 0xf, 0xf, true);
-}
-template <int CAM>
-__device__ __forceinline__ float quad_bcast_f(float v) {
-    return __builtin_bit_cast(float, quad_bcast_i<CAM>(__builtin_bit_cast(int, v)));
-}
-template <int CAM>
-__device__ __forceinline__ Bilin quad_bcast(const Bilin& m) {
-    Bilin t;
-    t.o00 = quad_bcast_i<CAM>(m.o00);
-    t.o01 = quad_bcast_i<CAM>(m.o01);
-    t.o10 = quad_bcast_i<CAM>(m.o10);
-    t.o11 = quad_bcast_i<CAM>(m.o11);
-    t.w00 = quad_bcast_f<CAM>(m.w00);
-    t.w01 = quad_bcast_f<CAM>(m.w01);
-    t.w10 = quad_bcast_f<CAM>(m.w10);
-    t.w11 = quad_bcast_f<CAM>(m.w11);
-    return t;
 }
 
 #ifndef MVSGI_SWEEP_NT
@@ -410,150 +356,33 @@
                                     : nullptr;
     const long long sstep = (long long)(s.Ho + 2) * (s.Wo + 2) * 64;
     const int C4 = C16 ? 64 : s.C * 4, rowB = s.Wi * C4;
-    auto candidate = [&](const float2 gxy, const unsigned vm, float* __restrict__ o, unsigned char* __restrict__ os) {
-        typedef float f32x2_t __attribute__((ext_vector_type(2)));
-        const Bilin mine = bilin_setup_bytes(gxy.x, gxy.y, s.Wi, s.Hi, C4, rowB);
-        Bilin ft[NCAM];
-        ft[0] = quad_bcast<0>(mine);
-        if (NCAM > 1) ft[NCAM > 1 ? 1 : 0] = quad_bcast<1>(mine);
-        if (NCAM > 2) ft[NCAM > 2 ? 2 : 0] = quad_bcast<2>(mine);
-        if (NCAM > 3) ft[NCAM > 3 ? 3 : 0] = quad_bcast<3>(mine);
-        bool val[NCAM];
-        f32x2_t VF[NCAM];
-        float n = 0.0f;
-#pragma unroll
-        for (int cam = 0; cam < NCAM; ++cam) {
-            val[cam] = ((vm >> cam) & 1u) != 0;
-            const float vf = val[cam] ? 1.0f : 0.0f;
-            VF[cam] = f32x2_t{vf, vf};
-            n = n + vf;
-        }
-        const bool ok = n > 1.0f;
-        const float cnt = ok ? n : 1.0f;
-#ifndef MVSGI_SWEEP_GATHER_ALL
-#pragma unroll
-        for (int cam = 0; cam < NCAM; ++cam) {
-            const bool need = val[cam] & ok;
-            ft[cam].o00 = need ? ft[cam].o00 : (int)0x80000000;
-            ft[cam].o01 = need ? ft[cam].o01 : (int)0x80000000;
-            ft[cam].o10 = need ? ft[cam].o10 : (int)0x80000000;
-            ft[cam].o11 = need ? ft[cam].o11 : (int)0x80000000;
-        }
-#endif
-        const float inv = cnt == 2.0f ? 0.5f : cnt == 3.0f ? 0x1.555556p-2f : cnt == 4.0f ? 0.25f : 1.0f;
-        const f32x2_t INV = {inv, inv}, NCNT = {-cnt, -cnt};
-#pragma unroll 1
-        for (int cb = q * 16; cb < (C16 ? 64 : C4); cb += 64) {
-            f32x4_t tx[NCAM][4];
-#ifdef MVSGI_SWEEP_ABL_NOGATHER
-#pragma unroll
-            for (int cam = 0; cam < NCAM; ++cam) { ft[cam].o00 &= 64; ft[cam].o01 &= 64; ft[cam].o10 &= 64; ft[cam].o11 &= 64; }
-#endif
-#pragma unroll
-            for (int cam = 0; cam < NCAM; ++cam) {
-#if MVSGI_SWEEP_SKIP_CAM
-                if (__builtin_amdgcn_ballot_w64(val[cam] & ok) == 0) {
-                    tx[cam][0] = tx[cam][1] = tx[cam][2] = tx[cam][3] = f32x4_t{0.f, 0.f, 0.f, 0.f};
-                    continue;
-                }
-#endif
-                tx[cam][0] = __builtin_bit_cast(f32x4_t, __builtin_amdgcn_raw_buffer_load_b128(img[cam], ft[cam].o00 + cb, 0, 0));
-                tx[cam][1] = __builtin_bit_cast(f32x4_t, __builtin_amdgcn_raw_buffer_load_b128(img[cam], ft[cam].o01 + cb, 0, 0));
-                tx[cam][2] = __builtin_bit_cast(f32x4_t, __builtin_amdgcn_raw_buffer_load_b128(img[cam], ft[cam].o10 + cb, 0, 0));
-                tx[cam][3] = __builtin_bit_cast(f32x4_t, __builtin_amdgcn_raw_buffer_load_b128(img[cam], ft[cam].o11 + cb, 0, 0));
-            }
-            f32x2_t sv[NCAM][2];
-#pragma unroll
-            for (int cam = 0; cam < NCAM; ++cam) {
-                const f32x2_t W00 = {ft[cam].w00, ft[cam].w00}, W01 = {ft[cam].w01, ft[cam].w01};
-                const f32x2_t W10 = {ft[cam].w10, ft[cam].w10}, W11 = {ft[cam].w11, ft[cam].w11};
-#pragma unroll
-                for (int p = 0; p < 2; ++p) {
-                    const f32x2_t i00 = {tx[cam][0][2 * p], tx[cam][0][2 * p + 1]}, i01 = {tx[cam][1][2 * p], tx[cam][1][2 * p + 1]};
-                    const f32x2_t i10 = {tx[cam][2][2 * p], tx[cam][2][2 * p + 1]}, i11 = {tx[cam][3][2 * p], tx[cam][3][2 * p + 1]};
-                    sv[cam][p] = ((i00 * W00 + i01 * W01) + i10 * W10) + i11 * W11;
-                }
-            }
-            f32x2_t sum[2], var[2];
-            f32x4_t r;
-            float big = 0.0f;
-#pragma unroll
-            for (int p = 0; p < 2; ++p) {
-                sum[p] = sv[0][p] * VF[0];
-#pragma unroll
-                for (int cam = 1; cam < NCAM; ++cam) sum[p] = sum[p] + sv[cam][p] * VF[cam];
-                const f32x2_t qa = sum[p] * INV;
-                const f32x2_t avg = __builtin_elementwise_fma(__builtin_elementwise_fma(NCNT, qa, sum[p]), INV, qa);
-#pragma unroll
-                for (int cam = 0; cam < NCAM; ++cam) {
-                    const f32x2_t t = {val[cam] ? sv[cam][p].x : avg.x, val[cam] ? sv[cam][p].y : avg.y};
-                    const f32x2_t df = t - avg;
-                    var[p] = cam == 0 ? df * df : var[p] + df * df;
-                }
-                const f32x2_t qv = var[p] * INV;
-                const f32x2_t v = __builtin_elementwise_fma(__builtin_elementwise_fma(NCNT, qv, var[p]), INV, qv);
-                r[2 * p] = ok ? v.x : 0.0f;
-                r[2 * p + 1] = ok ? v.y : 0.0f;
-                big = __builtin_fmaxf(__builtin_fmaxf(big, __builtin_fmaxf(__builtin_fabsf(sum[p].x), __builtin_fabsf(sum[p].y))),
-                                      __builtin_fmaxf(var[p].x, var[p].y));
-            }
-            if (__builtin_amdgcn_ballot_w64(big > 1e30f) != 0) {
-                float dv = cnt;
-                asm volatile("; exact-division path" : "+v"(dv));
-#pragma unroll
-                for (int k = 0; k < 4; ++k) {
-                    const float sm = sum[k >> 1][k & 1];
-                    const float avg = sm / dv;
-                    float vr = 0.0f;
-#pragma unroll
-                    for (int cam = 0; cam < NCAM; ++cam) {
-                        const float t = val[cam] ? sv[cam][k >> 1][k & 1] : avg;
-                        const float df = t - avg;
-                        vr = vr + df * df;
-                    }
-                    vr = vr / dv;
-                    r[k] = ok ? vr : 0.0f;
-                }
-            }
-            if (os) {
-                unsigned hi[2], lo[2];
-#pragma unroll
-                for (int p = 0; p < 2; ++p) {
-                    if constexpr (F16) {
-                        const float a_ = sf_clamp<true>(r[2 * p]), b_ = sf_clamp<true>(r[2 * p + 1]);
-                        satm = sf_sat_acc(satm, a_, b_);
-                        const unsigned hb = sf_cvt_pk<true>(a_, b_);
-                        hi[p] = hb;
-                        lo[p] = sf_cvt_pk<true>(a_ - sf_widen_lo<true>(hb), b_ - sf_widen_hi<true>(hb));
-                    } else {
-                        typedef __bf16 b2_t __attribute__((ext_vector_type(2)));
-                        const f32x2_t v = {r[2 * p], r[2 * p + 1]};
-                        const unsigned hb = __builtin_bit_cast(unsigned, __builtin_convertvector(v, b2_t));
-                        const f32x2_t hf = {__builtin_bit_cast(float, hb << 16), __builtin_bit_cast(float, hb & 0xffff0000u)};
-                        hi[p] = hb;
-                        lo[p] = __builtin_bit_cast(unsigned, __builtin_convertvector(v - hf, b2_t));
-                    }
-                }
-                const bool odd = (q & 1) != 0;
-                const unsigned r0 = (unsigned)__builtin_amdgcn_mov_dpp((int)(odd ? hi[0] : lo[0]), 0xB1, 0xf, 0xf, true);
-                const unsigned r1 = (unsigned)__builtin_amdgcn_mov_dpp((int)(odd ? hi[1] : lo[1]), 0xB1, 0xf, 0xf, true);
-                const uint4 piece = odd ? make_uint4(r0, r1, lo[0], lo[1]) : make_uint4(hi[0], hi[1], r0, r1);
+    struct Sink {
+        float* __restrict__ o;
+        unsigned char* __restrict__ os;
+        bool live;
+        __device__ __forceinline__ bool split() const { return os != nullptr; }
+        __device__ __forceinline__ void f32(const int cb, const f32x4_t r) const {
+            if (live) *reinterpret_cast<f32x4_t*>(reinterpret_cast<char*>(o) + cb) = r;
+        }
+        __device__ __forceinline__ void piece(const uint4 piece) const {
 #ifdef MVSGI_SWEEP_ABL_NOSTORE
-                if (live && hi[0] == 0x12345678u) {
+            if (live && piece.x == 0x12345678u) {
 #else
-                if (live) {
+            if (live) {
 #endif
 #if MVSGI_SWEEP_NT
-                    {
-                        typedef unsigned nt_u32x4 __attribute__((ext_vector_type(4)));
-                        __builtin_nontemporal_store(nt_u32x4{piece.x, piece.y, piece.z, piece.w}, reinterpret_cast<nt_u32x4*>(os));
-                    }
+                {
+                    typedef unsigned nt_u32x4 __attribute__((ext_vector_type(4)));
+                    __builtin_nontemporal_store(nt_u32x4{piece.x, piece.y, piece.z, piece.w}, reinterpret_cast<nt_u32x4*>(os));
+                }
 #else
-                    *reinterpret_cast<uint4*>(os) = piece;
+                *reinterpret_cast<uint4*>(os) = piece;
 #endif
-                }
-            } else if (live) *reinterpret_cast<f32x4_t*>(reinterpret_cast<char*>(o) + cb) = r;
-        }
+            }
+        }
+    };
+    auto candidate = [&](const float2 gxy, const unsigned vm, float* __restrict__ o, unsigned char* __restrict__ os) {
+        sweep_candidate<NCAM, C16, F16>(img, q, s.Wi, s.Hi, C4, rowB, gxy, vm, satm, Sink{o, os, live});
     };
     float2 gA = *gp;
     unsigned vA = *vp;
diff --git a/mvs_gi_amd/csrc/sweep_candidate.hpp b/mvs_gi_amd/csrc/sweep_candidate.hpp
--- /dev/null
+++ b/mvs_gi_amd/csrc/sweep_candidate.hpp
@@ -0,0 +1,194 @@
+#pragma once
+
+struct Bilin {
+    int o00, o01, o10, o11;
+    float w00, w01, w10, w11;
+};
+
+#ifndef MVSGI_SWEEP_SKIP_CAM
+#define MVSGI_SWEEP_SKIP_CAM 1
+#endif
+
+typedef float f32x4_t __attribute__((ext_vector_type(4)));
+
+__device__ __forceinline__ Bilin bilin_setup_bytes(float gx, float gy, int W, int H, int C4, int rowB) {
+#pragma clang fp contract(off)
+    Bilin t;
+    const float x = ((gx + 1.0f) * (float)W - 1.0f) / 2.0f;
+    const float y = ((gy + 1.0f) * (float)H - 1.0f) / 2.0f;
+    const float xf = floorf(x), yf = floorf(y);
+    const float x1f = xf + 1.0f, y1f = yf + 1.0f;
+    t.w00 = (x1f - x) * (y1f - y);
+    t.w01 = (x1f - x) * (y - yf);
+    t.w10 = (x - xf) * (y1f - y);
+    t.w11 = (x - xf) * (y - yf);
+    const int x0 = (int)fminf(fmaxf(xf, -2.0f), (float)W + 1.0f);
+    const int y0 = (int)fminf(fmaxf(yf, -2.0f), (float)H + 1.0f);
+    const bool vx0 = (unsigned)x0 < (unsigned)W, vx1 = (unsigned)(x0 + 1) < (unsigned)W;
+    const bool vy0 = (unsigned)y0 < (unsigned)H, vy1 = (unsigned)(y0 + 1) < (unsigned)H;
+    const int base = __mul24(y0, rowB) + __mul24(x0, C4);
+    constexpr int kOutside = (int)0x80000000;
+    t.o00 = (vx0 & vy0) ? base : kOutside;
+    t.o01 = (vx0 & vy1) ? base + rowB : kOutside;
+    t.o10 = (vx1 & vy0) ? base + C4 : kOutside;
+    t.o11 = (vx1 & vy1) ? base + rowB + C4 : kOutside;
+    return t;
+}
+
+template <int CAM>
+__device__ __forceinline__ int quad_bcast_i(int v) {
+    return __builtin_amdgcn_mov_dpp(v, CAM * 0x55, 0xf, 0xf, true);
+}
+template <int CAM>
+__device__ __forceinline__ float quad_bcast_f(float v) {
+    return __builtin_bit_cast(float, quad_bcast_i<CAM>(__builtin_bit_cast(int, v)));
+}
+template <int CAM>
+__device__ __forceinline__ Bilin quad_bcast(const Bilin& m) {
+    Bilin t;
+    t.o00 = quad_bcast_i<CAM>(m.o00);
+    t.o01 = quad_bcast_i<CAM>(m.o01);
+    t.o10 = quad_bcast_i<CAM>(m.o10);
+    t.o11 = quad_bcast_i<CAM>(m.o11);
+    t.w00 = quad_bcast_f<CAM>(m.w00);
+    t.w01 = quad_bcast_f<CAM>(m.w01);
+    t.w10 = quad_bcast_f<CAM>(m.w10);
+    t.w11 = quad_bcast_f<CAM>(m.w11);
+    return t;
+}
+
+template <int NCAM, bool C16, bool F16, class Sink>
+__device__ __forceinline__ void sweep_candidate(const __amdgpu_buffer_rsrc_t (&img)[NCAM], const int q, const int Wi, const int Hi,
+                                                const int C4, const int rowB, const float2 gxy, const unsigned vm, float& satm,
+                                                const Sink& sink) {
+#pragma clang fp contract(off)
+    typedef float f32x2_t __attribute__((ext_vector_type(2)));
+    const Bilin mine = bilin_setup_bytes(gxy.x, gxy.y, Wi, Hi, C4, rowB);
+    Bilin ft[NCAM];
+    ft[0] = quad_bcast<0>(mine);
+    if (NCAM > 1) ft[NCAM > 1 ? 1 : 0] = quad_bcast<1>(mine);
+    if (NCAM > 2) ft[NCAM > 2 ? 2 : 0] = quad_bcast<2>(mine);
+    if (NCAM > 3) ft[NCAM > 3 ? 3 : 0] = quad_bcast<3>(mine);
+    bool val[NCAM];
+    f32x2_t VF[NCAM];
+    float n = 0.0f;
+#pragma unroll
+    for (int cam = 0; cam < NCAM; ++cam) {
+        val[cam] = ((vm >> cam) & 1u) != 0;
+        const float vf = val[cam] ? 1.0f : 0.0f;
+        VF[cam] = f32x2_t{vf, vf};
+        n = n + vf;
+    }
+    const bool ok = n > 1.0f;
+    const float cnt = ok ? n : 1.0f;
+#ifndef MVSGI_SWEEP_GATHER_ALL
+#pragma unroll
+    for (int cam = 0; cam < NCAM; ++cam) {
+        const bool need = val[cam] & ok;
+        ft[cam].o00 = need ? ft[cam].o00 : (int)0x80000000;
+        ft[cam].o01 = need ? ft[cam].o01 : (int)0x80000000;
+        ft[cam].o10 = need ? ft[cam].o10 : (int)0x80000000;
+        ft[cam].o11 = need ? ft[cam].o11 : (int)0x80000000;
+    }
+#endif
+    const float inv = cnt == 2.0f ? 0.5f : cnt == 3.0f ? 0x1.555556p-2f : cnt == 4.0f ? 0.25f : 1.0f;
+    const f32x2_t INV = {inv, inv}, NCNT = {-cnt, -cnt};
+#pragma unroll 1
+    for (int cb = q * 16; cb < (C16 ? 64 : C4); cb += 64) {
+        f32x4_t tx[NCAM][4];
+#ifdef MVSGI_SWEEP_ABL_NOGATHER
+#pragma unroll
+        for (int cam = 0; cam < NCAM; ++cam) { ft[cam].o00 &= 64; ft[cam].o01 &= 64; ft[cam].o10 &= 64; ft[cam].o11 &= 64; }
+#endif
+#pragma unroll
+        for (int cam = 0; cam < NCAM; ++cam) {
+#if MVSGI_SWEEP_SKIP_CAM
+            if (__builtin_amdgcn_ballot_w64(val[cam] & ok) == 0) {
+                tx[cam][0] = tx[cam][1] = tx[cam][2] = tx[cam][3] = f32x4_t{0.f, 0.f, 0.f, 0.f};
+                continue;
+            }
+#endif
+            tx[cam][0] = __builtin_bit_cast(f32x4_t, __builtin_amdgcn_raw_buffer_load_b128(img[cam], ft[cam].o00 + cb, 0, 0));
+            tx[cam][1] = __builtin_bit_cast(f32x4_t, __builtin_amdgcn_raw_buffer_load_b128(img[cam], ft[cam].o01 + cb, 0, 0));
+            tx[cam][2] = __builtin_bit_cast(f32x4_t, __builtin_amdgcn_raw_buffer_load_b128(img[cam], ft[cam].o10 + cb, 0, 0));
+            tx[cam][3] = __builtin_bit_cast(f32x4_t, __builtin_amdgcn_raw_buffer_load_b128(img[cam], ft[cam].o11 + cb, 0, 0));
+        }
+        f32x2_t sv[NCAM][2];
+#pragma unroll
+        for (int cam = 0; cam < NCAM; ++cam) {
+            const f32x2_t W00 = {ft[cam].w00, ft[cam].w00}, W01 = {ft[cam].w01, ft[cam].w01};
+            const f32x2_t W10 = {ft[cam].w10, ft[cam].w10}, W11 = {ft[cam].w11, ft[cam].w11};
+#pragma unroll
+            for (int p = 0; p < 2; ++p) {
+                const f32x2_t i00 = {tx[cam][0][2 * p], tx[cam][0][2 * p + 1]}, i01 = {tx[cam][1][2 * p], tx[cam][1][2 * p + 1]};
+                const f32x2_t i10 = {tx[cam][2][2 * p], tx[cam][2][2 * p + 1]}, i11 = {tx[cam][3][2 * p], tx[cam][3][2 * p + 1]};
+                sv[cam][p] = ((i00 * W00 + i01 * W01) + i10 * W10) + i11 * W11;
+            }
+        }
+        f32x2_t sum[2], var[2];
+        f32x4_t r;
+        float big = 0.0f;
+#pragma unroll
+        for (int p = 0; p < 2; ++p) {
+            sum[p] = sv[0][p] * VF[0];
+#pragma unroll
+            for (int cam = 1; cam < NCAM; ++cam) sum[p] = sum[p] + sv[cam][p] * VF[cam];
+            const f32x2_t qa = sum[p] * INV;
+            const f32x2_t avg = __builtin_elementwise_fma(__builtin_elementwise_fma(NCNT, qa, sum[p]), INV, qa);
+#pragma unroll
+            for (int cam = 0; cam < NCAM; ++cam) {
+                const f32x2_t t = {val[cam] ? sv[cam][p].x : avg.x, val[cam] ? sv[cam][p].y : avg.y};
+                const f32x2_t df = t - avg;
+                var[p] = cam == 0 ? df * df : var[p] + df * df;
+            }
+            const f32x2_t qv = var[p] * INV;
+            const f32x2_t v = __builtin_elementwise_fma(__builtin_elementwise_fma(NCNT, qv, var[p]), INV, qv);
+            r[2 * p] = ok ? v.x : 0.0f;
+            r[2 * p + 1] = ok ? v.y : 0.0f;
+            big = __builtin_fmaxf(__builtin_fmaxf(big, __builtin_fmaxf(__builtin_fabsf(sum[p].x), __builtin_fabsf(sum[p].y))),
+                                  __builtin_fmaxf(var[p].x, var[p].y));
+        }
+        if (__builtin_amdgcn_ballot_w64(big > 1e30f) != 0) {
+            float dv = cnt;
+            asm volatile("; exact-division path" : "+v"(dv));
+#pragma unroll
+            for (int k = 0; k < 4; ++k) {
+                const float sm = sum[k >> 1][k & 1];
+                const float avg = sm / dv;
+                float vr = 0.0f;
+#pragma unroll
+                for (int cam = 0; cam < NCAM; ++cam) {
+                    const float t = val[cam] ? sv[cam][k >> 1][k & 1] : avg;
+                    const float df = t - avg;
+                    vr = vr + df * df;
+                }
+                vr = vr / dv;
+                r[k] = ok ? vr : 0.0f;
+            }
+        }
+        if (sink.split()) {
+            unsigned hi[2], lo[2];
+#pragma unroll
+            for (int p = 0; p < 2; ++p) {
+                if constexpr (F16) {
+                    const float a_ = sf_clamp<true>(r[2 * p]), b_ = sf_clamp<true>(r[2 * p + 1]);
+                    satm = sf_sat_acc(satm, a_, b_);
+                    const unsigned hb = sf_cvt_pk<true>(a_, b_);
+                    hi[p] = hb;
+                    lo[p] = sf_cvt_pk<true>(a_ - sf_widen_lo<true>(hb), b_ - sf_widen_hi<true>(hb));
+                } else {
+                    typedef __bf16 b2_t __attribute__((ext_vector_type(2)));
+                    const f32x2_t v = {r[2 * p], r[2 * p + 1]};
+                    const unsigned hb = __builtin_bit_cast(unsigned, __builtin_convertvector(v, b2_t));
+                    const f32x2_t hf = {__builtin_bit_cast(float, hb << 16), __builtin_bit_cast(float, hb & 0xffff0000u)};
+                    hi[p] = hb;
+                    lo[p] = __builtin_bit_cast(unsigned, __builtin_convertvector(v - hf, b2_t));
+                }
+            }
+            const bool odd = (q & 1) != 0;
+            const unsigned r0 = (unsigned)__builtin_amdgcn_mov_dpp((int)(odd ? hi[0] : lo[0]), 0xB1, 0xf, 0xf, true);
+            const unsigned r1 = (unsigned)__builtin_amdgcn_mov_dpp((int)(odd ? hi[1] : lo[1]), 0xB1, 0xf, 0xf, true);
+            sink.piece(odd ? make_uint4(r0, r1, lo[0], lo[1]) : make_uint4(hi[0], hi[1], r0, r1));
+        } else sink.f32(cb, r);
+    }
+}
diff --git a/mvs_gi_amd/dropin/cost_volume_builder.py b/mvs_gi_amd/dropin/cost_volume_builder.py
--- a/mvs_gi_amd/dropin/cost_volume_builder.py
+++ b/mvs_gi_amd/dropin/cost_volume_builder.py
@@ -49,10 +49,7 @@
     return bufs[key]
 
 
-def std_sweep_ndhwc(feats, grids, grid_masks, masks, owner=None, split_out: bool = False, buf_frames: int = 0):
-    use_cache = _rig_cache_usable(owner, feats, grids)
-    if not use_cache:
-        return None if split_out else H.sweep_std(feats, grids, grid_masks, masks)
+def _rig_constants(owner, grids, grid_masks, masks):
     tensors = (grids, grid_masks, masks)
     cached = _RIG_VALIDITY.get(owner)
     if not _rig_hit(cached, tensors):
@@ -66,15 +63,22 @@
         pins = owner.__dict__.setdefault("_mvsgi_graph_pins", [])
         if not any(p is cached for p in pins):
             pins.append(cached)
-    g_use = cached[3] if cached[3] is not None else grids
+    return (cached[3] if cached[3] is not None else grids), cached[2]
+
+
+def std_sweep_ndhwc(feats, grids, grid_masks, masks, owner=None, split_out: bool = False, buf_frames: int = 0):
+    use_cache = _rig_cache_usable(owner, feats, grids)
+    if not use_cache:
+        return None if split_out else H.sweep_std(feats, grids, grid_masks, masks)
+    g_use, vmask = _rig_constants(owner, grids, grid_masks, masks)
     if split_out:
         B, D, Ho, Wo = feats.shape[0], grids.shape[2], grids.shape[3], grids.shape[4]
         nb = max(B, int(buf_frames))
         full = _owned_split_buffer(owner, "_mvsgi_rs_vol", (nb, D, Ho, Wo, feats.device),
                                    lambda: H.SplitAct(nb, D, Ho, Wo, 16, feats.device))
         out = full if nb == B else H.SplitAct(B, D, Ho, Wo, 16, feats.device, buf=full.buf[:B])
-        return H.sweep_std_valid_split(feats, g_use, cached[2], out=out, fmt=H.mode_fmt())
-    return H.sweep_std_valid(feats, g_use, cached[2])
+        return H.sweep_std_valid_split(feats, g_use, vmask, out=out, fmt=H.mode_fmt())
+    return H.sweep_std_valid(feats, g_use, vmask)
 
 
 def cat_sweep_ndhwc(feats, grids) -> Tensor:
@@ -83,6 +87,7 @@
 
 _USE_RS = True
 _FRONT_CHUNK = int(os.environ.get("MVSGI_FRONT_CHUNK", "16"))
+_FUSED_FRONT = {"0": False, "force": "force"}.get(os.environ.get("MVSGI_FUSED_FRONT", "1"), True)
 
 
 def _std_front(self, feats: Tensor, grids: Tensor, grid_masks: Tensor, masks: Tensor, hand_over_split: bool):
@@ -97,6 +102,9 @@
     xs = None
     if hand_over_split:
         xs = _owned_split_buffer(self, "_mvsgi_rs_x0", (B, D, Ho, Wo, feats.device), lambda: H.SplitAct(B, D, Ho, Wo, 16, feats.device))
+    if hand_over_split and _FUSED_FRONT and H.mode_fmt() == "f16" and (_FUSED_FRONT == "force" or H.front_std16_pays(B, D, Ho, Wo)):
+        g_use, vmask = _rig_constants(self, grids, grid_masks, masks)
+        return H.front_std16(feats, g_use, vmask, wp_rs, sc_rs, L.shift, out=xs, neg_slope=L.neg_slope, fmt="f16", force=True)
     k = _FRONT_CHUNK
     shared = all(t.dim() > 0 and t.shape[0] > 1 and t.stride(0) == 0 for t in (grids, grid_masks, masks))
     if k > 0 and B > k and shared:
diff --git a/mvs_gi_amd/hip_ops.py b/mvs_gi_amd/hip_ops.py
--- a/mvs_gi_amd/hip_ops.py
+++ b/mvs_gi_amd/hip_ops.py
@@ -220,6 +220,34 @@
     _lib.check(lib.mvsgi_sweep_std_nhwc_valid_split_fmt(f.data_ptr(), grids.data_ptr(), vmask.data_ptr(), out.buf.data_ptr(), B, N, C, Hi,
                                                         Wi, D, Ho, Wo, Bg, _fmt_code(fmt), _stream_ptr(f)), "mvsgi_sweep_std_nhwc_valid_split")
     out.fmt = fmt
+    return out
+
+
+def front_std16_pays(B: int, D: int, Ho: int, Wo: int) -> bool:
+    return bool(_lib.load().mvsgi_front_std16_pays(int(B), int(D), int(Ho), int(Wo)))
+
+
+def front_std16(feats, grids, vmask, w_packed_rs, scale, shift, out: "SplitAct", neg_slope=0.01, fmt: str = "f16",
+                vol_debug: Optional["SplitAct"] = None, force: bool = False) -> "SplitAct":
+    lib = _lib.load()
+    B, N, C, Hi, Wi = feats.shape
+    f = _feats_nhwc(feats)
+    grids = _dev(grids, "grids")
+    vmask = _dev(vmask, "vmask", torch.uint8)
+    Bg, Ng, D, Ho, Wo, two = grids.shape
+    if (Ng, two) != (N, 2) or Bg not in (1, B) or tuple(vmask.shape) != (Bg, D, Ho, Wo) or C != 16 or scale.numel() != 16:
+        raise AssertionError(f"grids {tuple(grids.shape)} / vmask {tuple(vmask.shape)} do not match feats {tuple(feats.shape)} (C == 16)")
+    if out.shape != (B, D, Ho, Wo, C) or (vol_debug is not None and vol_debug.shape != out.shape):
+        raise AssertionError(f"split output {out.shape} does not match {(B, D, Ho, Wo, C)}")
+    if not (force or front_std16_pays(B, D, Ho, Wo)):
+        raise RuntimeError(f"front_std16: {B} frames of {(D, Ho, Wo)} are below front_std16_pays(); use the two launches (or force=True)")
+    _lib.check(lib.mvsgi_front_std16_split_fmt(f.data_ptr(), grids.data_ptr(), vmask.data_ptr(), w_packed_rs.data_ptr(), scale.data_ptr(),
+                                               shift.data_ptr(), out.buf.data_ptr(), None if vol_debug is None else vol_debug.buf.data_ptr(),
+                                               B, N, Hi, Wi, D, Ho, Wo, Bg, float(neg_slope), _fmt_code(fmt), _stream_ptr(f)),
+               "mvsgi_front_std16_split_fmt")
+    out.fmt = fmt
+    if vol_debug is not None:
+        vol_debug.fmt = fmt
     return out
 
 
```

New measurement: 6256. 0.982x the previous value.
